# bryanboateng/animating-gaussian-splats

Hardware: AMD Instinct MI355X
Metric: Msplats/sec fwd+bwd @1080p (1M gauss) (higher is better)
Workload: dtype f32; 1 GPU; C3: 1000000 Gaussians, SH3, 1920x1080, 27-camera rig, 5 view(s)/GPU/step, fwd+bwd; gaussians=1000000, image=1920x1080, sh_degree=3, parallelism=camera-dp1, streams_per_gpu=3, submission=one host thread per stream, means2D=one fresh zero leaf per render (shared.py:38-41)

## Files before the change

animating-gaussian-splats_amd/csrc/gsr_api.hip:

```cpp
#include <hip/hip_runtime.h>

#include <atomic>
#include <cstdarg>
#include <cstdio>
#include <cstdlib>
#include <cmath>
#include <cstring>
#include <chrono>
#include <condition_variable>
#include <thread>
#include <map>
#include <memory>
#include <unordered_map>
#include <mutex>
#include <string>
#include <vector>

#include "../../include/gsr.h"
#include "gsr_common.h"
#include "gsr_internal.h"
#include "gsr_host.h"

using namespace gsr;

// ... 21 lines not shown
}

int gsr::fail(int code, const char *fmt, ...) {
    char buf[512];
    va_list ap;
    va_start(ap, fmt);
    vsnprintf(buf, sizeof(buf), fmt, ap);
    va_end(ap);
    g_err = buf;
    return code;
}

gsr::Phase::Phase(hipStream_t s_, const char *n, bool on) : s(s_), name(n) {
    if (!on || !g_prof_on) return;
    std::lock_guard<std::mutex> lk(g_prof_mu);
    if (!g_prof_sel.empty() && g_prof_sel.find("," + std::string(n) + ",") == std::string::npos) return;
    a = ev_get(); b = ev_get();
    if (a) (void)hipEventRecord(a, s);
}
gsr::Phase::~Phase() {
    if (!a || !b) return;
    (void)hipEventRecord(b, s);
    std::lock_guard<std::mutex> lk(g_prof_mu);
    g_prof.push_back({name, a, b});
}

gsr::HostPhase::HostPhase(const char *n) : name(n), t0(hclock::now()), on(g_prof_on) {}
gsr::HostPhase::~HostPhase() {
    if (!on) return;
    const double ms = std::chrono::duration<double, std::milli>(hclock::now() - t0).count();
    std::lock_guard<std::mutex> lk(g_prof_mu);
    g_host_ms[name] += ms;
    g_host_n[name] += 1;
}

namespace {

std::vector<hipEvent_t> g_gw_evpool;
struct GradEvent {
    hipEvent_t ev = nullptr;
    ~GradEvent() { if (ev) g_gw_evpool.push_back(ev); }
};
struct GradWriter { hipStream_t s = nullptr; std::shared_ptr<GradEvent> ev; };
std::mutex g_gw_mu;
std::unordered_map<const void *, GradWriter> g_gw;
constexpr size_t kGradPruneAt = 1024;

hipError_t no_launch() { return hipSuccess; }

template <typename Launch>
hipError_t ordered_grad_write(const void *const *keys, int nkeys, hipStream_t s, Launch launch) {
    std::lock_guard<std::mutex> lk(g_gw_mu);
    const GradEvent *waited[16];
    int nw = 0;
    for (int k = 0; k < nkeys; ++k) {
        if (!keys[k]) continue;
        auto it = g_gw.find(keys[k]);
        if (it == g_gw.end() || it->second.s == s) continue;
        const GradEvent *e = it->second.ev.get();
        bool seen = false;
        for (int j = 0; j < nw; ++j) seen = seen || waited[j] == e;
        if (seen) continue;
        const hipError_t r = hipStreamWaitEvent(s, e->ev, 0);
        if (r != hipSuccess) return r;
        if (nw < 16) waited[nw++] = e;
    }
    auto ev = std::make_shared<GradEvent>();
    hipError_t r = hipSuccess;
    if (!g_gw_evpool.empty()) { ev->ev = g_gw_evpool.back(); g_gw_evpool.pop_back(); }
    else r = hipEventCreateWithFlags(&ev->ev, hipEventDisableTiming);
    if (r != hipSuccess) { ev->ev = nullptr; return r; }
    r = launch();
    if (r != hipSuccess) return r;
    r = hipEventRecord(ev->ev, s);
    if (r != hipSuccess) return r;
    for (int k = 0; k < nkeys; ++k)
        if (keys[k]) g_gw[keys[k]] = GradWriter{s, ev};
    if (g_gw.size() > kGradPruneAt) {
        for (auto it = g_gw.begin(); it != g_gw.end();)
            it = hipEventQuery(it->second.ev->ev) == hipSuccess ? g_gw.erase(it) : std::next(it);
    }
    return hipSuccess;
}

struct HostWord { uint32_t *h = nullptr; uint32_t *d = nullptr; };
HostWord pinned_word() {
    thread_local HostWord w;
    if (!w.h) {
        uint32_t *h = nullptr;
        if (hipHostMalloc((void **)&h, 4 * kHostWords, hipHostMallocMapped | hipHostMallocCoherent) != hipSuccess) return w;
        uint32_t *d = nullptr;
        if (hipHostGetDevicePointer((void **)&d, h, 0) != hipSuccess) { (void)hipHostFree(h); return w; }
        w.h = h; w.d = d;
    }
    return w;
}

constexpr uint32_t kNoValue = 0xFFFFFFFFu;

int check_common(const gsr_camera *cam, const gsr_gaussians *g, bool need_opacity) {
    if (!cam || !g) return fail(GSR_ERR_ARG, "null camera or gaussians");
    if (g->P < 0) return fail(GSR_ERR_ARG, "P must be >= 0");
    if (cam->image_width <= 0 || cam->image_height <= 0)
        return fail(GSR_ERR_ARG, "image size must be positive (got %dx%d)", cam->image_width, cam->image_height);
    const int gx = div_up(cam->image_width, kTileW), gy = div_up(cam->image_height, kTileH);
    if (gx > 65535 || gy > 65535) return fail(GSR_ERR_UNSUPPORTED, "tile grid too large");
    if (g->activations & ~(GSR_ACT_SIGMOID_OPACITY | GSR_ACT_EXP_SCALES | GSR_ACT_NORMALIZE_ROTATIONS))
        return fail(GSR_ERR_ARG, "unknown activation bits 0x%x", g->activations);
    if (g->P == 0) return GSR_OK;
    if (!g->means3D || (need_opacity && !g->opacities))
        return fail(GSR_ERR_ARG, "means3D and opacities are required");
    if ((g->shs == nullptr) == (g->colors_precomp == nullptr))
        return fail(GSR_ERR_ARG, "Please provide excatly one of either SHs or precomputed colors!");
    const bool sr = g->scales && g->rotations;
    if (sr == (g->cov3D_precomp != nullptr) || ((g->scales != nullptr) != (g->rotations != nullptr)))
        return fail(GSR_ERR_ARG, "Please provide exactly one of either scale/rotation pair or precomputed 3D covariance!");
    if (g->shs && (g->sh_coeffs <= 0 || (g->sh_degree + 1) * (g->sh_degree + 1) > g->sh_coeffs || g->sh_degree > 3 || g->sh_degree < 0))
        return fail(GSR_ERR_ARG, "invalid SH configuration: degree %d with %d coefficients", g->sh_degree, g->sh_coeffs);
    if (!cam->viewmatrix || !cam->projmatrix || !cam->bg || (g->shs && !cam->campos))
        return fail(GSR_ERR_ARG, "camera matrices / bg / campos missing");
    return GSR_OK;
}

std::atomic<int> g_exact{[] {
    const char *e = getenv("GSR_EXACT_THRESHOLDS");
    return (e && e[0] == '0') ? 0 : 1;
}()};

void fill_common(ViewIn &v, const gsr_camera *cam, const gsr_gaussians *g) {
    memset(&v, 0, sizeof(v));
    v.P = g->P; v.D = g->sh_degree; v.M = g->shs ? g->sh_coeffs : 0;
    v.W = cam->image_width; v.H = cam->image_height;
    v.gx = div_up(v.W, kTileW); v.gy = div_up(v.H, kTileH);
    v.scale_modifier = g->scale_modifier;
    v.act = g->activations;
    v.tan_fovx = cam->tan_fovx; v.tan_fovy = cam->tan_fovy;
    v.focal_y = v.H / (2.0f * v.tan_fovy);
    v.focal_x = v.W / (2.0f * v.tan_fovx);
    v.means3D = g->means3D; v.scales = g->scales; v.rotations = g->rotations; v.opacities = g->opacities;
    v.shs = g->shs; v.colors_precomp = g->colors_precomp; v.cov3D_precomp = g->cov3D_precomp;
    v.viewmatrix = cam->viewmatrix; v.projmatrix = cam->projmatrix; v.campos = cam->campos; v.bg = cam->bg;
    const bool vz = !cam->viewmatrix_stride[0] && !cam->viewmatrix_stride[1];
    const bool pz = !cam->projmatrix_stride[0] && !cam->projmatrix_stride[1];
    v.cs.v0 = vz ? 4 : cam->viewmatrix_stride[0]; v.cs.v1 = vz ? 1 : cam->viewmatrix_stride[1];
    v.cs.p0 = pz ? 4 : cam->projmatrix_stride[0]; v.cs.p1 = pz ? 1 : cam->projmatrix_stride[1];
    v.cs.c0 = cam->campos_stride ? cam->campos_stride : 1;
}

template <typename A>
void carve_saved(A &a, char *geom, char *img) {
    const GeomLayout G(a.v.P);
    a.rec = (float4 *)(geom + G.rec); a.rect = (uint2 *)(geom + G.rect);
    a.goff = (uint32_t *)(geom + G.goff); a.clampm = (uint8_t *)(geom + G.clampm);
    const ImageLayout L(a.v.W, a.v.H, a.v.P);
    a.ranges = (uint2 *)(img + L.ranges); a.pix_end = (float4 *)(img + L.pix_end);
    a.n_contrib = (uint32_t *)(img + L.n_contrib); a.tile_maxc = (uint32_t *)(img + L.tile_maxc);
    a.tile_flag = (uint32_t *)(img + L.tile_flag); a.near_rec = (float4 *)(img + L.near_rec);
    a.seg_off = (uint32_t *)(img + L.seg_off); a.meta = (uint32_t *)(img + L.meta);
    a.items_ws = (uint32_t *)(img + L.items_ws);
}
void carve_forward(FwdArgs &a, char *geom, char *img) {
    carve_saved(a, geom, img);
    const GeomLayout G(a.v.P);
    a.depth = (float *)(geom + G.depth); a.tiles = (uint32_t *)(geom + G.tiles);
    const ImageLayout L(a.v.W, a.v.H, a.v.P);
    a.tile_order_f = (uint32_t *)(img + L.tile_order_f); a.sort_lists = (uint32_t *)(img + L.sort_lists);
    a.tile_count = (uint32_t *)(img + L.tile_count); a.tile_cursor = (uint32_t *)(img + L.tile_cursor);
    a.block_sums = (uint32_t *)(img + L.block_sums); a.block_off = (uint32_t *)(img + L.block_off);
    a.chunk_off = (uint32_t *)(img + L.chunk_off); a.scan_ws = (uint32_t *)(img + L.scan_ws);
    a.tile_rank = (uint32_t *)(img + L.tile_rank); a.tsat_list = (uint32_t *)(img + L.tsat_list);
}
template <typename A>
void carve_binning(A &a, char *bin, const BinningLayout &L) {
    a.point_list = (uint32_t *)(bin + L.point_list); a.slot_emit = (uint32_t *)(bin + L.slot_emit);
    a.seg_state = (float4 *)(bin + L.seg_state);
}

struct BinRegions {
    BinningLayout arrays;
    size_t items, tmp, total;
    BinRegions(int K, int P, int T, bool with_items, bool with_merge) : arrays(K, P) {
        items = arrays.total;
        tmp = items + (with_items ? bwd_items_bytes(K, T) : 0);
        total = tmp + (with_merge ? sizeof(uint4) * (size_t)K : 0);
    }
};

int enqueue_post_scan(FwdArgs a, char *bin, int layout, uint32_t n_mid, uint32_t n_vlong, uint32_t max_n,
                      bool prepare_backward, int T, hipStream_t s, const uint32_t *spec_ok, bool phases) {
    const BinRegions R(layout, a.v.P, T, prepare_backward, n_vlong != 0);
    carve_binning(a, bin, R.arrays);
    a.pairs = (uint4 *)(bin + R.arrays.pairs);
    a.spec_ok = spec_ok;
    uint4 *tmp = n_vlong ? (uint4 *)(bin + R.tmp) : nullptr;
    uint2 *items = (uint2 *)(bin + R.items);
    { Phase ph(s, "bin_emit", phases); HIP_TRY(launch_bin_emit(a, spec_ok ? 0 : layout, s)); }
    { Phase ph(s, "tile_sort", phases); HIP_TRY(launch_tile_sort(a, n_mid, n_vlong, max_n, tmp, s)); }
    { Phase ph(s, "render_fwd", phases); HIP_TRY(launch_render_fwd(a, s)); }
    if (prepare_backward) {
        Phase ph(s, "bwd_items", phases);
        HIP_TRY(launch_bwd_items_raw(layout, T, a.v.P, a.ranges, a.tile_maxc, a.tile_flag, items, a.items_ws, s, spec_ok));
    }
    return GSR_OK;
}

enum class KWait { published, stream_error, drained };
KWait wait_published(const uint32_t *word, hipStream_t s, hipError_t *err) {
    auto last = hclock::now();
    while (__atomic_load_n(word, __ATOMIC_ACQUIRE) == kNoValue) {
        __builtin_ia32_pause();
        if (hclock::now() - last > std::chrono::microseconds(500)) {
            last = hclock::now();
            const hipError_t q = hipStreamQuery(s);
            if (q == hipErrorNotReady) continue;
            *err = q;
            if (q != hipSuccess) return KWait::stream_error;
            return __atomic_load_n(word, __ATOMIC_ACQUIRE) == kNoValue ? KWait::drained : KWait::published;
        }
    }
    return KWait::published;
}

}

extern "C" {

const char *gsr_last_error(void) { return g_err.c_str(); }

int gsr_set_exact_thresholds(int on) { return g_exact.exchange(on ? 1 : 0); }
int gsr_abi_version(void) { return GSR_ABI_VERSION; }

size_t gsr_geom_bytes(int P) { return GeomLayout(P < 0 ? 0 : P).total; }
size_t gsr_image_bytes(int W, int H, int P) { return ImageLayout(W, H, P < 0 ? 0 : P).total; }
size_t gsr_binning_bytes(int K, int P) { return BinningLayout(K, P).total; }
size_t gsr_backward_items_bytes(int K, int W, int H) {
    return bwd_items_bytes(K < 0 ? 0 : K, div_up(W < 0 ? 0 : W, kTileW) * div_up(H < 0 ? 0 : H, kTileH));
}
size_t gsr_sums_bytes(int P) { return align256(sizeof(float) * (kPartial * (size_t)(P < 0 ? 0 : P) + 1)); }
size_t gsr_scratch_bytes(int K, int W, int H) {
    return ScratchLayout(K, div_up(W < 0 ? 0 : W, kTileW) * div_up(H < 0 ? 0 : H, kTileH)).total;
}

void *gsr_prealloc_alloc(void *ctx, int which, size_t bytes) {
    gsr_prealloc *pa = (gsr_prealloc *)ctx;
    if (!pa) return nullptr;
    if (which >= 0 && which < 5 && pa->ptr[which] && pa->bytes[which] >= bytes && !(pa->used & (1 << which))) {
        pa->used |= 1 << which;
        return pa->ptr[which];
    }
    return pa->fallback ? pa->fallback(pa->fallback_ctx, which, bytes) : nullptr;
}

int gsr_buffer_offsets(int P, int W, int H, int K, size_t *out, int max_out) {
    const GeomLayout g(P);
    const ImageLayout im(W, H, P);
    const BinningLayout b(K, P);
    const size_t v[16] = {g.depth, g.rec, g.rect, g.tiles, g.goff,
                          im.ranges, im.pix_end, im.n_contrib, im.tile_maxc,
                          b.pairs, b.point_list, b.slot_emit, im.seg_off, b.seg_state, im.tile_flag,
                          im.items_ws + sizeof(uint32_t) * kTSatCtr};
    int n = 0;
    for (; n < 16 && n < max_out; ++n) out[n] = v[n];
    return n;
}

}

namespace {
struct SpecKey {
    int dev, P, W, H;
    bool operator==(const SpecKey &o) const { return dev == o.dev && P == o.P && W == o.W && H == o.H; }
};
struct SpecKeyHash {
    size_t operator()(const SpecKey &k) const {
        return ((size_t)k.dev * 1000003u) ^ ((size_t)k.P * 2654435761u) ^ ((size_t)k.W << 20) ^ (size_t)k.H;
    }
};
constexpr int kSpecWindow = 16;
constexpr size_t kSpecKeys = 64;
struct SpecStat {
    uint32_t recent[kSpecWindow] = {};
    uint32_t recent_mid[kSpecWindow] = {};
    int n = 0;
    bool long_lists = false;
    uint64_t used = 0;
    uint32_t window_max() const {
        uint32_t m = 0;
        for (int k = 0; k < std::min(n, kSpecWindow); ++k) m = std::max(m, recent[k]);
        return m;
    }
};
std::mutex g_spec_mu;
std::unordered_map<SpecKey, SpecStat, SpecKeyHash> g_spec;
uint64_t g_spec_clock = 0;
int g_spec_hits = 0, g_spec_misses = 0, g_async_calls = 0;

uint32_t spec_capacity(const SpecKey &key, uint32_t *sort_blocks = nullptr) {
    std::lock_guard<std::mutex> lk(g_spec_mu);
    auto it = g_spec.find(key);
    if (it == g_spec.end() || it->second.long_lists) return 0;
    it->second.used = ++g_spec_clock;
    const uint32_t mk = it->second.window_max();
    if (sort_blocks) {
        uint32_t mm = 0;
        for (int k = 0; k < std::min(it->second.n, kSpecWindow); ++k) mm = std::max(mm, it->second.recent_mid[k]);
        *sort_blocks = std::min<uint32_t>((uint32_t)kSpecSortBlocks, mm + mm / 4 + 16);
    }
    const uint64_t c = (uint64_t)mk + mk / 4 + 65536;
    return (uint32_t)std::min<uint64_t>((c + 4095) & ~uint64_t(4095), 0x7FFFFFFFu);
}
void spec_record(const SpecKey &key, uint32_t K, bool long_lists, int outcome, uint32_t n_mid) {
    std::lock_guard<std::mutex> lk(g_spec_mu);
    if (!g_spec.count(key) && g_spec.size() >= kSpecKeys) {
        auto lru = g_spec.begin();
        for (auto it = g_spec.begin(); it != g_spec.end(); ++it)
            if (it->second.used < lru->second.used) lru = it;
        g_spec.erase(lru);
    }
    SpecStat &st = g_spec[key];
    st.recent[st.n % kSpecWindow] = K;
    st.recent_mid[st.n % kSpecWindow] = n_mid;
    ++st.n;
    st.long_lists = long_lists;
    st.used = ++g_spec_clock;
    if (outcome > 0) ++g_spec_hits;
    if (outcome < 0) ++g_spec_misses;
}

constexpr int kAsyncSlots = 4096;
constexpr int kSlotWords = 16;
constexpr int kGateWord = 4, kGateErrWord = 5;
constexpr uint64_t kGateTimeoutTicks = 500000000ull;
std::atomic<uint64_t> g_gate_timeout{kGateTimeoutTicks};
std::atomic<int> g_hold_next_redo_ms{0};

struct AsyncFwd {
    uint64_t id = 0;
    int dev = 0, slot = -1, T = 0;
    hipStream_t s = nullptr;
    uint32_t seq = 0, cap = 0;
    bool prep = false, released = false, err_reported = false;
    SpecKey key{0, 0, 0, 0};
    FwdArgs a;
    void *spec_bin = nullptr;
    hipEvent_t ev_scan = nullptr;
    int state = 0;
    uint32_t K = 0;
    int layout = 0;
    void *bin = nullptr;
    void *own = nullptr;
    std::string err;
};

std::mutex g_as_mu;
std::condition_variable g_as_wake;
std::condition_variable g_as_done;
std::unordered_map<uint64_t, std::shared_ptr<AsyncFwd>> g_as;
uint64_t g_as_next_id = 1;
uint32_t g_as_seq = 0;
uint32_t *g_slot_h = nullptr, *g_slot_d = nullptr;
std::vector<uint8_t> g_slot_busy;
std::vector<hipEvent_t> g_as_evpool;
int g_slot_next = 0;
std::string g_async_err;
bool g_resolver_started = false, g_resolver_stop = false;
std::thread g_resolver;

uint32_t *slot_h(int k) { return g_slot_h + (size_t)k * kSlotWords; }
uint32_t *slot_d(int k) { return g_slot_d + (size_t)k * kSlotWords; }

void resolver_main();

std::map<int, hipStream_t> g_resolver_streams;
hipStream_t resolver_stream(int dev) {
    hipStream_t &h = g_resolver_streams[dev];
    if (h) return h;
    int lo = 0, hi = 0;
    if (hipDeviceGetStreamPriorityRange(&lo, &hi) != hipSuccess) hi = 0;
    if (hipStreamCreateWithPriority(&h, hipStreamNonBlocking, hi) != hipSuccess) h = nullptr;
    return h;
}

bool async_init() {
    if (!g_slot_h) {
        uint32_t *h = nullptr;
        const size_t bytes = sizeof(uint32_t) * ((size_t)kAsyncSlots * kSlotWords + 16);
        if (hipHostMalloc((void **)&h, bytes, hipHostMallocMapped | hipHostMallocCoherent | hipHostMallocPortable) != hipSuccess)
            return false;
        uint32_t *d = nullptr;
        if (hipHostGetDevicePointer((void **)&d, h, 0) != hipSuccess) { (void)hipHostFree(h); return false; }
        memset(h, 0, bytes);
        g_slot_h = h; g_slot_d = d;
        g_slot_busy.assign(kAsyncSlots, 0);
    }
    if (!g_resolver_started) {
        g_resolver_stop = false;
        g_resolver = std::thread(resolver_main);
        g_resolver_started = true;
    }
    return true;
}

int slot_acquire() {
    for (int k = 0; k < kAsyncSlots; ++k) {
        const int j = (g_slot_next + k) % kAsyncSlots;
        if (!g_slot_busy[j]) {
            g_slot_busy[j] = 1;
            g_slot_next = (j + 1) % kAsyncSlots;
            return j;
        }
    }
    return -1;
// ... 586 lines not shown
```

animating-gaussian-splats_amd/csrc/gsr_backward.hip:

```cpp
#include "gsr_common.h"
#include "gsr_internal.h"

#include <algorithm>

namespace gsr {

#ifdef GSR_TRACE
__device__ uint64_t *g_trace_bwd;
#endif

constexpr uint32_t kItemStartCost = 64;

constexpr int kItemsBlock = 256;
struct ItemBucket {
    uint32_t shift;
    __device__ explicit ItemBucket(int ks) {
        const uint32_t mx = (4u << ks) + kItemStartCost;
        shift = mx >= (uint32_t)kOrderBuckets ? 32 - __builtin_clz(mx / kOrderBuckets) : 0;
    }
    __device__ uint32_t operator()(uint32_t cost) const {
        return (uint32_t)kOrderBuckets - 1u - min(cost >> shift, (uint32_t)kOrderBuckets - 1u);
    }
};
template <typename F>
// ... 76 lines not shown
            items[base + atomicAdd(&items[0].y, 1u)] = make_uint2((uint32_t)t, code);
        });
    }
    const uint32_t n = ex ? 0u : rg.y - rg.x;
    for_tile_items(n, mq, ks, bk, [&](uint32_t, uint32_t b) { atomicAdd(&s_cur[b], 1u); });
    lds_barrier();
    for (int b = threadIdx.x; b < kOrderBuckets; b += blockDim.x) {
        const uint32_t h = s_cur[b];
        if (h) s_cur[b] = atomicAdd(&ws[kOrderBuckets + b], h);
    }
    lds_barrier();
    for_tile_items(n, mq, ks, bk, [&](uint32_t code, uint32_t b) {
        items[1 + atomicAdd(&s_cur[b], 1u)] = make_uint2((uint32_t)t, code);
    });
}

struct __attribute__((packed, aligned(4))) F3 { float x, y, z; };
__device__ inline void rec_store(float4 *part, uint32_t em, float r0, float r1, float r2, float r3, float r4,
                                 float r5, float r6, float r7, float r8) {
    F3 *d = reinterpret_cast<F3 *>(reinterpret_cast<float *>(part) + (size_t)kRecF * em);
    d[0] = F3{r0, r1, r2};
    d[1] = F3{r3, r4, r5};
    d[2] = F3{r6, r7, r8};
}

#define GSR_BWD_ATTR __attribute__((amdgpu_waves_per_eu(EXACT ? 4 : 7, 8)))
constexpr int kBwdWaves = 4;
#ifndef GSR_EXACT_BWD_BLOCKS
#define GSR_EXACT_BWD_BLOCKS 256
#endif
constexpr int kExactBwdBlocks = GSR_EXACT_BWD_BLOCKS;

__device__ inline void row_halves3(float &X, float &Y, float &Z) {
    asm("s_nop 1\n\t"
        "v_add_f32_dpp %0, %0, %0 row_ror:8 row_mask:0xf bank_mask:0xf bound_ctrl:1\n\t"
        "v_add_f32_dpp %1, %1, %1 row_ror:8 row_mask:0xf bank_mask:0xf bound_ctrl:1\n\t"
        "v_add_f32_dpp %2, %2, %2 row_ror:8 row_mask:0xf bank_mask:0xf bound_ctrl:1\n\t"
        "v_add_f32_dpp %0, %0, %0 row_ror:4 row_mask:0xf bank_mask:0xf bound_ctrl:1\n\t"
        "v_add_f32_dpp %1, %1, %1 row_ror:4 row_mask:0xf bank_mask:0xf bound_ctrl:1\n\t"
        "v_add_f32_dpp %2, %2, %2 row_ror:4 row_mask:0xf bank_mask:0xf bound_ctrl:1\n\t"
        "v_add_f32_dpp %0, %0, %0 row_ror:2 row_mask:0xf bank_mask:0xf bound_ctrl:1\n\t"
        "v_add_f32_dpp %1, %1, %1 row_ror:2 row_mask:0xf bank_mask:0xf bound_ctrl:1\n\t"
        "v_add_f32_dpp %2, %2, %2 row_ror:2 row_mask:0xf bank_mask:0xf bound_ctrl:1"
        : "+v"(X), "+v"(Y), "+v"(Z));
}
struct RowW { bool r0, r2; };
__device__ inline RowW row_weights(int row) { return RowW{row == 0, row == 2}; }
struct PairSums { float X, Y, Z; };
__device__ inline PairSums pair_sums(float S0, float S1, float S4, float cs0, float cs1, float cs2, float dx,
                                     const RowW &w) {
    const float pA = fold32(S0, S1), pB = fold32(S4, cs0), pC = fold32(cs1, cs2);
    const float rA = fold16(pA, pB);
    const float rC = fold16(0.f, pC);
    const float wx = w.r0 ? dx : 1.f;
    const float wy = w.r0 ? dx * dx : (w.r2 ? dx : 0.f);
    PairSums r{rA * wx, fmaf(rA, wy, rC), rA};
    row_halves3(r.X, r.Y, r.Z);
    return r;
}

struct PixState { float T, AR; f2v d01; float d2, fy; int lrel; };
struct LaneSums { float S0; f2v S14, c01; float c2; };

constexpr int kNearNone = 0, kNearLook = 1, kNearEval = 2;
struct NearRecs { const float4 *r; uint32_t n; int start; };
template <bool CLAMP, int NEAR>
__device__ __forceinline__ void eval_quarter(PixState &ps, LaneSums &s, bool &any, const PairX &x, float4 a,
                                             float C2, float o, float4 c, int j, int k, float pfx,
                                             const float4 *__restrict__ rec, const uint32_t *__restrict__ pl,
                                             const NearRecs &nrs) {
    const float dy = a.y - ps.fy;
    float p2 = pair_power(x, C2, dy);
    float G = __builtin_amdgcn_exp2f(p2);
    float alpha = CLAMP ? fminf(0.99f, o * G) : o * G;
    const bool live = j < ps.lrel;
    if constexpr (NEAR == kNearEval) {
        const bool nr = live && p2 <= 0.0f && near_threshold(alpha);
        if (nr) {
            const ExactBlend e = exact_blend(a.x, a.y, rec[(size_t)kRecF4 * pl[j] + 3], o, pfx, ps.fy);
            p2 = e.power; G = e.G; alpha = e.alpha;
        }
    } else if constexpr (NEAR == kNearLook) {
        const bool nr = live && p2 <= 0.0f && near_threshold(alpha);
        if (nr) {
            const uint32_t key = ((uint32_t)(nrs.start + j) << 8) | (uint32_t)((threadIdx.x & 63) + 64 * k);
            for (uint32_t i = 0; i < nrs.n; ++i) {
                const float4 r = nrs.r[i];
                const bool hit = __float_as_uint(r.x) == key;
                p2 = hit ? r.y : p2;
                G = hit ? r.z : G;
                alpha = hit ? r.w : alpha;
            }
        }
    }
    const bool ok = live && p2 <= 0.0f && alpha >= 1.0f / 255.0f;
    any = any || ok;
    const float al = ok ? alpha : 0.f;
    ps.T = ps.T * __builtin_amdgcn_rcpf(1.f - al);
    const float cd = fmaf(c.z, ps.d2, fmaf(c.y, ps.d01.y, c.x * ps.d01.x));
    const float diff = cd - ps.AR;
    ps.AR = fmaf(al, diff, ps.AR);
    const float w = al * ps.T;
    float gd;
    if constexpr (CLAMP) {
        const float tg = ps.T * diff;
        gd = ok ? (o * G) * tg : 0.f;
    } else {
        gd = w * diff;
    }
    const float u = gd * dy;
    s.S0 += gd;
    s.S14 = fma2(f2(gd, u), f2(dy, dy), s.S14);
    s.c01 = fma2(f2(w, w), ps.d01, s.c01);
    s.c2 = fmaf(w, ps.d2, s.c2);
}

template <bool CLAMP, int NEAR>
__device__ __forceinline__ void walk_batch(PixState (&ps)[4], uint64_t m, const float4 *s_a, float pfx,
                                           const RowW &rw, float *o_row, const float4 *__restrict__ rec,
                                           const uint32_t *__restrict__ pl, const NearRecs &nrs) {
    constexpr int kStage = 64 * kBwdWaves;
    while (m) {
        const int j = 63 - __builtin_clzll(m);
        m &= ~(1ull << j);
        const float4 a = s_a[j], b = s_a[kStage + j], c = s_a[2 * kStage + j];
        const uint32_t qm = __builtin_amdgcn_readfirstlane(__float_as_uint(c.w));
        const PairX x = pair_x(a, pfx);
        LaneSums s{-0.f, f2(-0.f, -0.f), f2(-0.f, -0.f), -0.f};
        bool any = false;
#pragma unroll
        for (int k = 0; k < 4; ++k) {
            if (!(qm & (1u << k))) continue;
            eval_quarter<CLAMP, NEAR>(ps[k], s, any, x, a, b.x, b.y, c, j, k, pfx, rec, pl, nrs);
        }
        if (__builtin_amdgcn_ballot_w64(any)) {
            const PairSums sm = pair_sums(s.S0, s.S14.x, s.S14.y, s.c01.x, s.c01.y, s.c2, x.dx, rw);
            if ((threadIdx.x & 14) == 0) {
                float *o = o_row + j * kPartial;
                lds_add(o, sm.X);
                lds_add(o + 4, sm.Y);
                if ((threadIdx.x & 63) < 2) lds_add(o + 8, sm.Z);
            }
        }
    }
}

template <bool EXACT>
__device__ __forceinline__ void bwd_item(
    uint2 it, uint32_t item, int W, int H, int gx, const uint2 *__restrict__ ranges,
    const uint32_t *__restrict__ point_list,
    const float4 *__restrict__ rec, const float *__restrict__ bg, const float4 *__restrict__ pix_end,
    const uint32_t *__restrict__ n_contrib, const uint32_t *__restrict__ tile_maxc,
    const uint32_t *__restrict__ seg_off, const float4 *__restrict__ seg_state,
    const uint32_t *__restrict__ slot_emit, const float *__restrict__ dL_dpixels,
    float4 *__restrict__ part, int ks, const uint32_t *__restrict__ tile_flag,
    const float4 *__restrict__ near_rec, float4 *s_a, float *s_out) {
    constexpr int kStage = 64 * kBwdWaves;
#ifdef GSR_TRACE
    const uint64_t t_start = __builtin_amdgcn_s_memrealtime();
#endif
    const int tile = (int)it.x;
    const uint32_t seg = it.y;
    const uint2 rg = ranges[tile];
    const int n = (int)(rg.y - rg.x);
    const int tx = tile % gx, ty = tile / gx;
    const int lane = threadIdx.x & 63;
    const int px = tx * kTileW + (lane & 15);
    const int py0 = ty * kTileH + (lane >> 4);
    const float pfx = (float)px;
    const float tx0 = (float)(tx * kTileW), ty0 = (float)(ty * kTileH);
    const float tx1 = tx0 + (kTileW - 1);
    const uint4 mq = reinterpret_cast<const uint4 *>(tile_maxc)[tile];
    const int maxc = min((int)max(max(mq.x, mq.y), max(mq.z, mq.w)), n);
    if (seg & kZeroItem) {
        const int z0 = maxc + (int)kZeroChunk * (int)((seg & ~kZeroItem) + 1);
        for (int p = z0 + lane; p < min(n, z0 + (int)kZeroChunk); p += 64) {
            rec_store(part, slot_emit[rg.x + p], 0.f, 0.f, 0.f, 0.f, 0.f, 0.f, 0.f, 0.f, 0.f);
        }
        return;
    }
    const int s0 = (int)seg << ks, s1f = s0 + (1 << ks);
    const int s1 = min(s1f, maxc);
    if (s1f >= maxc) {
        for (int p = maxc + lane; p < min(n, maxc + (int)kZeroChunk); p += 64) {
            rec_store(part, slot_emit[rg.x + p], 0.f, 0.f, 0.f, 0.f, 0.f, 0.f, 0.f, 0.f, 0.f);
        }
    }
    const float half_w = (float)(0.5 * W), half_h = (float)(0.5 * H);
    const float bg0 = bg[0], bg1 = bg[1], bg2 = bg[2];
    PixState ps[4];
    const uint32_t qmax[4] = {mq.x, mq.y, mq.z, mq.w};
    const bool has_bound = s1f < n;
    const size_t bidx = has_bound ? ((size_t)seg_off[tile] + seg) * kTilePix : 0;
#pragma unroll
    for (int k = 0; k < 4; ++k) {
        const int py = py0 + 4 * k;
        ps[k].fy = (float)py;
        const bool inside = px < W && py < H;
        const int pid = py * W + px;
        const float4 pe = inside ? pix_end[pid] : make_float4(0.f, 0.f, 0.f, 0.f);
        ps[k].lrel = (inside ? (int)n_contrib[pid] : 0) - s1;
        ps[k].d01 = f2(inside ? dL_dpixels[pid] : 0.f, inside ? dL_dpixels[H * W + pid] : 0.f);
        ps[k].d2 = inside ? dL_dpixels[2 * H * W + pid] : 0.f;
        float bd = 0;
        bd += bg0 * ps[k].d01.x; bd += bg1 * ps[k].d01.y; bd += bg2 * ps[k].d2;
        if (has_bound && qmax[k] >= (uint32_t)s1f) {
            const float4 st = seg_state[bidx + 64 * k + lane];
            ps[k].T = st.w;
            const float behind = ps[k].d01.x * (pe.x - st.x) + ps[k].d01.y * (pe.y - st.y) + ps[k].d2 * (pe.z - st.z);
            ps[k].AR = st.w > 0.f ? (behind + pe.w * bd) / st.w : bd;
        } else {
            ps[k].T = pe.w;
            ps[k].AR = bd;
        }
    }
    const RowW rw = row_weights(lane >> 4);
    float *o_row = s_out + (lane >> 4);
    NearRecs nrs{near_rec + (size_t)kNearCap * tile, EXACT ? 0u : tile_flag[tile], 0};
    uint32_t g_n = 0, em_n = 0;
    auto fetch = [&](int e) {
        const int st = e - 64 > s0 ? e - 64 : s0;
        if (lane < e - st) {
            g_n = point_list[rg.x + st + lane];
            em_n = slot_emit[rg.x + st + lane];
        }
    };
    if (s1 > s0) fetch(s1);
    for (int end = s1; end > s0; end -= 64) {
        const int start = end - 64 > s0 ? end - 64 : s0;
        const int cnt = end - start;
        float4 a = make_float4(0.f, 0.f, 0.f, 0.f), b = a, c = a, cj = a;
        float2 tl = make_float2(0.f, 0.f);
        if (lane < cnt) {
            const float4 *r = rec + (size_t)kRecF4 * g_n;
            a = r[0]; b = r[1]; c = r[2]; cj = r[3];
            tl = make_float2(cj.z, __uint_as_float(em_n));
        }
        if (end - 64 > s0) fetch(end - 64);
#pragma unroll
        for (int q = 0; q < kPartial; ++q) s_out[lane * kPartial + q] = 0.f;
#pragma unroll
        for (int k = 0; k < 4; ++k) ps[k].lrel += cnt;
        uint32_t qmask = 0;
        if (lane < cnt) {
            const uint32_t p = (uint32_t)(start + lane);
            s_a[lane] = a;
            s_a[kStage + lane] = make_float4(b.x, b.y, cj.x, cj.y);
#pragma unroll
            for (int k = 0; k < 4; ++k)
                if (p < qmax[k] &&
                    !tile_cull(a.x, a.y, -2.f * a.z, -a.w, -2.f * b.x, b.y, b.w, tx0, ty0 + 4 * k, tx1, ty0 + 4 * k + 3))
                    qmask |= 1u << k;
            if (qmask && b.y > 0.99f) qmask |= 16u;
            s_a[2 * kStage + lane] = make_float4(c.x, c.y, c.z, __uint_as_float(qmask));
        }
        uint64_t m = __ballot(qmask != 0);
        wave_lds_sync();
        const uint32_t *pl = point_list + rg.x + start;
        const bool clamp = __builtin_amdgcn_ballot_w64(qmask & 16u) != 0;
        if constexpr (EXACT) {
            if (clamp) walk_batch<true, kNearEval>(ps, m, s_a, pfx, rw, o_row, rec, pl, nrs);
            else walk_batch<false, kNearEval>(ps, m, s_a, pfx, rw, o_row, rec, pl, nrs);
        } else {
            nrs.start = start;
            if (nrs.n) {
                if (clamp) walk_batch<true, kNearLook>(ps, m, s_a, pfx, rw, o_row, rec, pl, nrs);
                else walk_batch<false, kNearLook>(ps, m, s_a, pfx, rw, o_row, rec, pl, nrs);
            } else {
                if (clamp) walk_batch<true, kNearNone>(ps, m, s_a, pfx, rw, o_row, rec, pl, nrs);
                else walk_batch<false, kNearNone>(ps, m, s_a, pfx, rw, o_row, rec, pl, nrs);
            }
        }
        wave_lds_sync();
        if (lane < cnt) {
            const float *s2 = s_out + lane * kPartial;
            float sm[kPartial];
#pragma unroll
            for (int q = 0; q < kPartial; ++q) sm[q] = s2[q];
            const float4 bj = s_a[kStage + lane];
            const float o = bj.y;
            const uint32_t em = __float_as_uint(tl.y);
            rec_store(part, em,
                      (-bj.z * sm[0] - bj.w * sm[2]) * half_w,
                      (-bj.w * sm[0] - tl.x * sm[2]) * half_h,
                      -0.5f * sm[4],
                      -0.5f * sm[6],
                      -0.5f * sm[1],
                      sm[8] != 0.f ? sm[8] / o : 0.f,
                      sm[3], sm[5], sm[7]);
        }
    }
#ifdef GSR_TRACE
    trace_wave(g_trace_bwd, item, t_start, 0);
#endif
}


template <bool EXACT>
__global__ __launch_bounds__(64 * kBwdWaves) GSR_BWD_ATTR void k_render_bwd(
    int W, int H, int gx, const uint2 *__restrict__ items, const uint2 *__restrict__ ranges,
    const uint32_t *__restrict__ point_list,
    const float4 *__restrict__ rec, const float *__restrict__ bg, const float4 *__restrict__ pix_end,
    const uint32_t *__restrict__ n_contrib, const uint32_t *__restrict__ tile_maxc,
    const uint32_t *__restrict__ seg_off, const float4 *__restrict__ seg_state,
    const uint32_t *__restrict__ slot_emit, const float *__restrict__ dL_dpixels,
    float4 *__restrict__ part, int ks, const uint32_t *__restrict__ spec_ok,
    const uint32_t *__restrict__ tile_flag, const float4 *__restrict__ near_rec) {
    constexpr int kStage = 64 * kBwdWaves;
    __shared__ float4 s_stage[3 * kStage];
    __shared__ float s_out_all[64 * kPartial * kBwdWaves];
    if (spec_ok && *spec_ok == 0u) return;
    const uint32_t wv = __builtin_amdgcn_readfirstlane(threadIdx.x >> 6);
    float4 *s_a = s_stage + 64 * wv;
    float *s_out = s_out_all + 64 * kPartial * wv;
    const uint2 hd = items[0];
    if constexpr (EXACT) {
        for (uint32_t i = blockIdx.x * kBwdWaves + wv; i < hd.y; i += gridDim.x * kBwdWaves)
            bwd_item<true>(items[1 + hd.x + i], hd.x + i, W, H, gx, ranges, point_list, rec, bg, pix_end, n_contrib, tile_maxc, seg_off, seg_state, slot_emit, dL_dpixels, part, ks, tile_flag, near_rec, s_a, s_out);
    } else {
        const uint32_t item = blockIdx.x * kBwdWaves + wv;
        if (item >= hd.x) return;
        bwd_item<false>(items[1 + item], item, W, H, gx, ranges, point_list, rec, bg, pix_end, n_contrib, tile_maxc, seg_off, seg_state, slot_emit, dL_dpixels, part, ks, tile_flag, near_rec, s_a, s_out);
    }
}

__device__ inline void gput(float *p, size_t idx, float v, bool acc) { p[idx] = acc ? p[idx] + v : v; }
template <int N>
__device__ inline void old_load(const float *p, size_t base, bool acc, float (&o)[N]) {
#pragma unroll
    for (int k = 0; k < N; ++k) o[k] = acc ? p[base + k] : 0.f;
}
__device__ inline void gput_old(float *p, size_t idx, float v, bool acc, float old) { p[idx] = acc ? old + v : v; }

__device__ inline float3 unit_vec_bwd(float3 v, float3 g) {
    const float n2 = v.x * v.x + v.y * v.y + v.z * v.z;
    const float inv_n3 = 1.0f / sqrtf(n2 * n2 * n2);
    return make_float3(((+n2 - v.x * v.x) * g.x - v.y * v.x * g.y - v.z * v.x * g.z) * inv_n3,
                       (-v.x * v.y * g.x + (n2 - v.y * v.y) * g.y - v.z * v.y * g.z) * inv_n3,
                       (-v.x * v.z * g.x - v.y * v.z * g.y + (n2 - v.z * v.z) * g.z) * inv_n3);
}

template <typename ShPtr>
__device__ inline float3 sh_dir_grad(int deg, float x, float y, float z, ShPtr sh, const float (&dRGB)[3]) {
    const float xx = x * x, yy = y * y, zz = z * z, xy = x * y, yz = y * z, xz = x * z;
    float dx[3] = {0, 0, 0}, dy[3] = {0, 0, 0}, dz[3] = {0, 0, 0};
#define SH(i, c) sh[(i) * 3 + (c)]
    if (deg > 0) {
#pragma unroll
        for (int c = 0; c < 3; ++c) {
            dx[c] = -GSR_SH_C1 * SH(3, c); dy[c] = -GSR_SH_C1 * SH(1, c); dz[c] = GSR_SH_C1 * SH(2, c);
        }
        if (deg > 1) {
#pragma unroll
            for (int c = 0; c < 3; ++c) {
                dx[c] += kSH_C2[0] * y * SH(4, c) + kSH_C2[2] * 2.f * -x * SH(6, c) + kSH_C2[3] * z * SH(7, c) +
                         kSH_C2[4] * 2.f * x * SH(8, c);
                dy[c] += kSH_C2[0] * x * SH(4, c) + kSH_C2[1] * z * SH(5, c) + kSH_C2[2] * 2.f * -y * SH(6, c) +
                         kSH_C2[4] * 2.f * -y * SH(8, c);
                dz[c] += kSH_C2[1] * y * SH(5, c) + kSH_C2[2] * 2.f * 2.f * z * SH(6, c) + kSH_C2[3] * x * SH(7, c);
            }
            if (deg > 2) {
#pragma unroll
                for (int c = 0; c < 3; ++c) {
                    dx[c] += (kSH_C3[0] * SH(9, c) * 3.f * 2.f * xy + kSH_C3[1] * SH(10, c) * yz +
                              kSH_C3[2] * SH(11, c) * -2.f * xy + kSH_C3[3] * SH(12, c) * -3.f * 2.f * xz +
                              kSH_C3[4] * SH(13, c) * (-3.f * xx + 4.f * zz - yy) +
                              kSH_C3[5] * SH(14, c) * 2.f * xz + kSH_C3[6] * SH(15, c) * 3.f * (xx - yy));
                    dy[c] += (kSH_C3[0] * SH(9, c) * 3.f * (xx - yy) + kSH_C3[1] * SH(10, c) * xz +
                              kSH_C3[2] * SH(11, c) * (-3.f * yy + 4.f * zz - xx) +
                              kSH_C3[3] * SH(12, c) * -3.f * 2.f * yz + kSH_C3[4] * SH(13, c) * -2.f * xy +
                              kSH_C3[5] * SH(14, c) * -2.f * yz + kSH_C3[6] * SH(15, c) * -3.f * 2.f * xy);
                    dz[c] += (kSH_C3[1] * SH(10, c) * xy + kSH_C3[2] * SH(11, c) * 4.f * 2.f * yz +
                              kSH_C3[3] * SH(12, c) * 3.f * (2.f * zz - xx - yy) +
                              kSH_C3[4] * SH(13, c) * 4.f * 2.f * xz + kSH_C3[5] * SH(14, c) * (xx - yy));
                }
            }
        }
    }
#undef SH
    return make_float3(dx[0] * dRGB[0] + dx[1] * dRGB[1] + dx[2] * dRGB[2],
                       dy[0] * dRGB[0] + dy[1] * dRGB[1] + dy[2] * dRGB[2],
                       dz[0] * dRGB[0] + dz[1] * dRGB[1] + dz[2] * dRGB[2]);
}

__device__ inline void sh_basis16(float x, float y, float z, float (&basis)[16]) {
    const float xx = x * x, yy = y * y, zz = z * z, xy = x * y, yz = y * z, xz = x * z;
    basis[0] = GSR_SH_C0;
    basis[1] = -GSR_SH_C1 * y; basis[2] = GSR_SH_C1 * z; basis[3] = -GSR_SH_C1 * x;
    basis[4] = kSH_C2[0] * xy; basis[5] = kSH_C2[1] * yz; basis[6] = kSH_C2[2] * (2.f * zz - xx - yy);
    basis[7] = kSH_C2[3] * xz; basis[8] = kSH_C2[4] * (xx - yy);
    basis[9] = kSH_C3[0] * y * (3.f * xx - yy);
    basis[10] = kSH_C3[1] * xy * z;
    basis[11] = kSH_C3[2] * y * (4.f * zz - xx - yy);
    basis[12] = kSH_C3[3] * z * (2.f * zz - 3.f * xx - 3.f * yy);
    basis[13] = kSH_C3[4] * x * (4.f * zz - xx - yy);
    basis[14] = kSH_C3[5] * z * (xx - yy);
    basis[15] = kSH_C3[6] * x * (xx - 3.f * yy);
}

template <typename ShPtr, typename OutPtr>
__device__ inline float3 sh_backward(int deg, int M, float3 mean, float3 campos, ShPtr sh,
                                     const bool *clamped, float3 dL_dcolor, OutPtr dL_dsh, bool acc = false) {
    const float3 d0 = make_float3(mean.x - campos.x, mean.y - campos.y, mean.z - campos.z);
    const float len = sqrtf(d0.x * d0.x + d0.y * d0.y + d0.z * d0.z);
    const float x = d0.x / len, y = d0.y / len, z = d0.z / len;
    const float dRGB[3] = {dL_dcolor.x * (clamped[0] ? 0.f : 1.f), dL_dcolor.y * (clamped[1] ? 0.f : 1.f),
                           dL_dcolor.z * (clamped[2] ? 0.f : 1.f)};
    const float3 dL_ddir = sh_dir_grad(deg, x, y, z, sh, dRGB);
    float basis[16];
    sh_basis16(x, y, z, basis);
    const int active = (deg + 1) * (deg + 1);
    if (dL_dsh) {
#pragma unroll
        for (int i = 0; i < 16; ++i) {
            if (i < M) {
#pragma unroll
                for (int c = 0; c < 3; ++c) {
                    const float v = i < active ? basis[i] * dRGB[c] : 0.f;
                    dL_dsh[i * 3 + c] = acc ? dL_dsh[i * 3 + c] + v : v;
                }
            }
        }
        for (int i = 16; i < M; ++i)
            for (int c = 0; c < 3; ++c) dL_dsh[i * 3 + c] = acc ? dL_dsh[i * 3 + c] : 0.f;
    }
    return unit_vec_bwd(d0, dL_ddir);
}

__device__ inline void cov3d_backward(float3 s3, float mod, float4 q, const float *dc, float3 &dscale,
                                      float4 &drot) {
    const float r = q.x, x = q.y, y = q.z, z = q.w;
    const m3 R = rot_from_quat(q);
    const float s[3] = {mod * s3.x, mod * s3.y, mod * s3.z};
    m3 S = {{0, 0, 0, 0, 0, 0, 0, 0, 0}};
    GM(S, 0, 0) = s[0]; GM(S, 1, 1) = s[1]; GM(S, 2, 2) = s[2];
    const m3 M = m3_mul(S, R);
    const m3 dSig = {{dc[0], 0.5f * dc[1], 0.5f * dc[2], 0.5f * dc[1], dc[3], 0.5f * dc[4], 0.5f * dc[2],
                      0.5f * dc[4], dc[5]}};
    m3 M2;
#pragma unroll
    for (int k = 0; k < 9; ++k) M2.m[k] = 2.0f * M.m[k];
    const m3 dM = m3_mul(M2, dSig);
    const m3 Rt = m3_T(R);
    m3 dMt = m3_T(dM);
    float ds[3];
#pragma unroll
    for (int i = 0; i < 3; ++i)
        ds[i] = GM(Rt, i, 0) * GM(dMt, i, 0) + GM(Rt, i, 1) * GM(dMt, i, 1) + GM(Rt, i, 2) * GM(dMt, i, 2);
    dscale = make_float3(ds[0], ds[1], ds[2]);
#pragma unroll
    for (int i = 0; i < 3; ++i)
#pragma unroll
        for (int rr = 0; rr < 3; ++rr) GM(dMt, i, rr) *= s[i];
#define G(c, rr) GM(dMt, c, rr)
    drot.x = 2 * z * (G(0, 1) - G(1, 0)) + 2 * y * (G(2, 0) - G(0, 2)) + 2 * x * (G(1, 2) - G(2, 1));
    drot.y = 2 * y * (G(1, 0) + G(0, 1)) + 2 * z * (G(2, 0) + G(0, 2)) + 2 * r * (G(1, 2) - G(2, 1)) -
             4 * x * (G(2, 2) + G(1, 1));
    drot.z = 2 * x * (G(1, 0) + G(0, 1)) + 2 * r * (G(2, 0) - G(0, 2)) + 2 * z * (G(1, 2) + G(2, 1)) -
             4 * y * (G(2, 2) + G(0, 0));
    drot.w = 2 * r * (G(0, 1) - G(1, 0)) + 2 * x * (G(2, 0) + G(0, 2)) + 2 * y * (G(1, 2) + G(2, 1)) -
             4 * z * (G(1, 1) + G(0, 0));
#undef G
}

template <int MC> constexpr int kRecChunk = 3 * 256 * 16 <= 64 * sh_row_stride(MC) * 4 ? 256 : 128;
template <int MC> constexpr int kRecStageF4 = 3 * kRecChunk<MC>;
__host__ __device__ constexpr int rec_chunk_f4(int C) { return (kRecF * C + 3 + 3) / 4; }
__device__ inline void add_chunk_records(const float *sf, uint32_t cb, uint32_t lo, uint32_t hi,
                                         float (&acc)[kPartial]) {
    for (uint32_t e = lo; e < hi; ++e) {
        const float *p = sf + kRecF * (e - cb);
#pragma unroll
        for (int k = 0; k < kPartial; ++k) acc[k] += p[k];
    }
}
// ... 440 lines not shown
        vis = true;
        gop += acc[5]; gc0 += acc[6]; gc1 += acc[7]; gc2 += acc[8];
        float vm[16], pj[16];
        load_mat16(V.viewmatrix, V.cs.v0, V.cs.v1, vm);
        load_mat16(V.projmatrix, V.cs.p0, V.cs.p1, pj);
        float dcov[6], dm0, dm1, dm2;
        view_chain(mean, c3, vm, pj, V.tan_fovx, V.tan_fovy, V.focal_x, V.focal_y, acc, dcov, dm0, dm1, dm2);
#pragma unroll
        for (int k = 0; k < 6; ++k) gcov[k] += dcov[k];
        if constexpr (MC > 0) {
            const float3 cp = load_campos(V.campos, V.cs.c0);
            bool cl[3];
            clamp_from_mask(V.clampm[i], cl);
            const float3 d0 = make_float3(mean.x - cp.x, mean.y - cp.y, mean.z - cp.z);
            const float len = sqrtf(d0.x * d0.x + d0.y * d0.y + d0.z * d0.z);
            const float x = d0.x / len, y = d0.y / len, z = d0.z / len;
            const float dRGB[3] = {acc[6] * (cl[0] ? 0.f : 1.f), acc[7] * (cl[1] ? 0.f : 1.f),
                                   acc[8] * (cl[2] ? 0.f : 1.f)};
            const float3 d = unit_vec_bwd(d0, sh_dir_grad(a.D, x, y, z, s_row, dRGB));
            dm0 += d.x; dm1 += d.y; dm2 += d.z;
        }
        gm0 += dm0; gm1 += dm1; gm2 += dm2;
    }
    if (live) {
        const int accm = a.accm;
        const bool ac = accm & GSR_GRAD_COLORS, ao = accm & GSR_GRAD_OPACITY, a3 = accm & GSR_GRAD_MEANS3D,
                   acv = accm & GSR_GRAD_COV3D, asc = accm & GSR_GRAD_SCALES, ar = accm & GSR_GRAD_ROTATIONS;
        if (!vis) {
#pragma unroll
            for (int k = 0; k < 3; ++k) {
                if (a.dL_dmeans3D && !a3) a.dL_dmeans3D[3 * i + k] = 0.f;
                if (a.dL_dcolors && !ac) a.dL_dcolors[3 * i + k] = 0.f;
                if (a.dL_dscales && !asc) a.dL_dscales[3 * i + k] = 0.f;
            }
            if (a.dL_dopacity && !ao) a.dL_dopacity[i] = 0.f;
            if (a.dL_dcov3D && !acv) {
#pragma unroll
                for (int k = 0; k < 6; ++k) a.dL_dcov3D[6 * i + k] = 0.f;
            }
            if (a.dL_drot && !ar) {
#pragma unroll
                for (int k = 0; k < 4; ++k) a.dL_drot[4 * i + k] = 0.f;
            }
        } else {
            float oo[1], oc[3], o3[3];
            old_load(a.dL_dopacity, (size_t)i, a.dL_dopacity && ao, oo);
            old_load(a.dL_dcolors, 3 * (size_t)i, a.dL_dcolors && ac, oc);
            old_load(a.dL_dmeans3D, 3 * (size_t)i, a.dL_dmeans3D && a3, o3);
            if (!a.dL_dopacity) {
            } else if (a.act & GSR_ACT_SIGMOID_OPACITY) {
                gput_old(a.dL_dopacity, i, gop * ((1.f - o_act) * o_act), ao, oo[0]);
            } else {
                gput_old(a.dL_dopacity, i, gop, ao, oo[0]);
            }
            if (a.dL_dcolors) {
                gput_old(a.dL_dcolors, 3 * i, gc0, ac, oc[0]); gput_old(a.dL_dcolors, 3 * i + 1, gc1, ac, oc[1]);
                gput_old(a.dL_dcolors, 3 * i + 2, gc2, ac, oc[2]);
            }
            if (a.dL_dmeans3D) {
                gput_old(a.dL_dmeans3D, 3 * i, gm0, a3, o3[0]); gput_old(a.dL_dmeans3D, 3 * i + 1, gm1, a3, o3[1]);
                gput_old(a.dL_dmeans3D, 3 * i + 2, gm2, a3, o3[2]);
            }
            if (a.dL_dcov3D) {
#pragma unroll
                for (int k = 0; k < 6; ++k) gput(a.dL_dcov3D, 6 * i + k, gcov[k], acv);
            }
            const bool has_sr = a.scales && !a.cov3D_precomp;
            if (has_sr) {
                float os[3], orr[4];
                old_load(a.dL_dscales, 3 * (size_t)i, a.dL_dscales && asc, os);
                old_load(a.dL_drot, 4 * (size_t)i, a.dL_drot && ar, orr);
                float3 ds; float4 dr;
                cov3d_backward(s3, a.scale_modifier, q, gcov, ds, dr);
                if (a.act & GSR_ACT_EXP_SCALES) { ds.x *= s3.x; ds.y *= s3.y; ds.z *= s3.z; }
                if (a.act & GSR_ACT_NORMALIZE_ROTATIONS) dr = act_normalize_bwd(q, qn, dr);
                if (a.dL_dscales) {
                    gput_old(a.dL_dscales, 3 * i, ds.x, asc, os[0]); gput_old(a.dL_dscales, 3 * i + 1, ds.y, asc, os[1]);
                    gput_old(a.dL_dscales, 3 * i + 2, ds.z, asc, os[2]);
                }
                if (a.dL_drot) {
                    gput_old(a.dL_drot, 4 * i, dr.x, ar, orr[0]); gput_old(a.dL_drot, 4 * i + 1, dr.y, ar, orr[1]);
                    gput_old(a.dL_drot, 4 * i + 2, dr.z, ar, orr[2]); gput_old(a.dL_drot, 4 * i + 3, dr.w, ar, orr[3]);
                }
            } else {
                if (a.dL_dscales && !asc) { a.dL_dscales[3 * i] = 0.f; a.dL_dscales[3 * i + 1] = 0.f; a.dL_dscales[3 * i + 2] = 0.f; }
                if (a.dL_drot && !ar) { a.dL_drot[4 * i] = 0.f; a.dL_drot[4 * i + 1] = 0.f; a.dL_drot[4 * i + 2] = 0.f; a.dL_drot[4 * i + 3] = 0.f; }
            }
        }
    }
    if constexpr (MC > 0) {
        if (!a.dL_dsh) return;
        if (live) {
#pragma unroll
            for (int k = 0; k < RL; ++k) s_row[k] = 0.f;
            const MultiView &V0 = a.v[vid(0)];
            int rv_n = V0.radii[i];
            uint8_t cm_n = V0.clampm[i];
            float g_n[3] = {V0.sums[(size_t)6 * P + i], V0.sums[(size_t)7 * P + i], V0.sums[(size_t)8 * P + i]};
            for (int t = 0; t < a.nv; ++t) {
                const MultiView &V = a.v[vid(t)];
                const int rv = rv_n;
                const uint8_t cm = cm_n;
                const float g[3] = {g_n[0], g_n[1], g_n[2]};
                if (t + 1 < a.nv) {
                    const MultiView &Vn = a.v[vid(t + 1)];
                    rv_n = Vn.radii[i];
                    cm_n = Vn.clampm[i];
#pragma unroll
                    for (int c = 0; c < 3; ++c) g_n[c] = Vn.sums[(size_t)(6 + c) * P + i];
                }
                if (!(rv > 0)) continue;
                const float3 cp = load_campos(V.campos, V.cs.c0);
                bool cl[3];
                clamp_from_mask(cm, cl);
                const float3 d0 = make_float3(mean.x - cp.x, mean.y - cp.y, mean.z - cp.z);
                const float len = sqrtf(d0.x * d0.x + d0.y * d0.y + d0.z * d0.z);
                const float x = d0.x / len, y = d0.y / len, z = d0.z / len;
                const float dRGB[3] = {g[0] * (cl[0] ? 0.f : 1.f), g[1] * (cl[1] ? 0.f : 1.f), g[2] * (cl[2] ? 0.f : 1.f)};
                float basis[16];
                sh_basis16(x, y, z, basis);
#pragma unroll
                for (int k = 0; k < MC; ++k)
                    if (k < active) {
#pragma unroll
                        for (int c = 0; c < 3; ++c) s_row[3 * k + c] += basis[k] * dRGB[c];
                    }
            }
        }
        __syncthreads();
        if (a.accm & GSR_GRAD_SH) sh_rows_from_lds<MC, true>(s_sh, nrow, a.dL_dsh + (size_t)i0 * RL);
        else sh_rows_from_lds<MC, false>(s_sh, nrow, a.dL_dsh + (size_t)i0 * RL);
    }
}


hipError_t launch_bwd_items_raw(int K, int T, int P, const uint2 *ranges, const uint32_t *tile_maxc,
                                const uint32_t *tile_flag, uint2 *items, uint32_t *ws, hipStream_t s,
                                const uint32_t *spec_ok) {
    if (K == 0) return hipSuccess;
    const int nb = div_up(T, kItemsBlock);
    k_items_count<<<nb, kItemsBlock, 0, s>>>(T, ranges, tile_maxc, tile_flag, items, ws, spec_ok, seg_log2(P));
    k_items_emit<<<nb, kItemsBlock, 0, s>>>(T, ranges, tile_maxc, tile_flag, items, ws, spec_ok, seg_log2(P));
    return hipGetLastError();
}
hipError_t launch_bwd_items(const BwdArgs &a, hipStream_t s) {
    return launch_bwd_items_raw(a.K, a.v.gx * a.v.gy, a.v.P, a.ranges, a.tile_maxc, a.tile_flag, a.items, a.items_ws, s);
}

hipError_t launch_render_bwd(const BwdArgs &a, hipStream_t s) {
    if (a.K == 0) return hipSuccess;
    const int ks = seg_log2(a.v.P);
    k_render_bwd<false><<<div_up((int)a.max_items, kBwdWaves), 64 * kBwdWaves, 0, s>>>(
        a.v.W, a.v.H, a.v.gx, a.items, a.ranges, a.point_list, a.rec, a.v.bg, a.pix_end, a.n_contrib, a.tile_maxc, a.seg_off,
        a.seg_state, a.slot_emit, a.dL_dcolor, a.part, ks, a.spec_ok, a.tile_flag, a.near_rec);
    k_render_bwd<true><<<std::min(div_up((int)a.max_items, kBwdWaves), kExactBwdBlocks), 64 * kBwdWaves, 0, s>>>(
        a.v.W, a.v.H, a.v.gx, a.items, a.ranges, a.point_list, a.rec, a.v.bg, a.pix_end, a.n_contrib, a.tile_maxc, a.seg_off,
        a.seg_state, a.slot_emit, a.dL_dcolor, a.part, ks, a.spec_ok, a.tile_flag, a.near_rec);
    return hipGetLastError();
}

template <int MC>
static void gauss_bwd_mc(const BwdArgs &a, hipStream_t s) {
    constexpr size_t lds = std::max(sizeof(float) * kShBlock * (MC ? sh_row_stride(MC) : 0),
                                    sizeof(float4) * kRecStageF4<MC> * (kShBlock / 64));
    k_gauss_bwd<MC><<<div_up(a.v.P, kShBlock), kShBlock, lds, s>>>(
        a.v.P, a.v.D, a.v.M, a.v.W, a.v.H, a.v.scale_modifier, a.v.tan_fovx, a.v.tan_fovy, a.v.focal_x, a.v.focal_y,
        a.v.means3D, a.v.scales, a.v.rotations, a.v.shs, a.v.cov3D_precomp, a.v.viewmatrix, a.v.projmatrix, a.v.campos, a.v.cs,
        a.radii, a.goff, a.part, a.dL_dmeans2D, a.dL_dcolors, a.dL_dopacity,
        a.dL_dmeans3D, a.dL_dcov3D, a.dL_dsh, a.dL_dscales, a.dL_drot, a.v.act, a.rec, a.accm, a.clampm);
}

hipError_t launch_gauss_bwd(const BwdArgs &a, hipStream_t s) {
    if (a.v.P == 0) return hipSuccess;
    switch (a.v.shs ? a.v.M : 0) {
        case 16: gauss_bwd_mc<16>(a, s); break;
        case 9: gauss_bwd_mc<9>(a, s); break;
        case 4: gauss_bwd_mc<4>(a, s); break;
        case 1: gauss_bwd_mc<1>(a, s); break;
        default: gauss_bwd_mc<0>(a, s); break;
    }
    return hipGetLastError();
}

template <int MC>
static void gauss_bwd_multi_mc(const MultiArgs &a, hipStream_t s) {
    k_gauss_bwd_multi<MC><<<div_up(a.P, kShBlock), kShBlock, multi_lds_bytes<MC>(), s>>>(a);
}

hipError_t launch_sum_records(int P, const uint32_t *goff, const float4 *part, float *sums, hipStream_t s,
                              const uint32_t *spec_ok, const float *viewmatrix, const float *projmatrix,
                              const float *campos, CamStrides cs, int W, int H) {
    if (P == 0) return hipSuccess;
    k_sum_records<<<div_up(P, 256), 256, 0, s>>>(P, goff, part, sums, spec_ok, viewmatrix, projmatrix, campos, cs,
                                                 W, H);
    return hipGetLastError();
}

hipError_t launch_gauss_bwd_multi(const MultiArgs &a, hipStream_t s) {
    if (a.P == 0 || a.nv == 0) return hipSuccess;
    switch (a.shs ? a.M : 0) {
        case 16: gauss_bwd_multi_mc<16>(a, s); break;
        case 9: gauss_bwd_multi_mc<9>(a, s); break;
        case 4: gauss_bwd_multi_mc<4>(a, s); break;
        case 1: gauss_bwd_multi_mc<1>(a, s); break;
        default: gauss_bwd_multi_mc<0>(a, s); break;
    }
    return hipGetLastError();
}

}

#ifdef GSR_TRACE
extern "C" int gsr_debug_trace_bwd(void *buf) {
    return hipMemcpyToSymbol(HIP_SYMBOL(gsr::g_trace_bwd), &buf, sizeof(buf)) == hipSuccess ? 0 : 2;
}
#endif
```

animating-gaussian-splats_amd/csrc/gsr_common.h:

```cpp
#pragma once
#include <hip/hip_runtime.h>
#include <stdint.h>

#include "../../include/gsr.h"

namespace gsr {

constexpr int kTileW = 16;
constexpr int kTileH = 16;
constexpr int kTilePix = kTileW * kTileH;
constexpr int kPartial = 9;
constexpr int kRecF = kPartial;
constexpr int kSortCap = 4096;
__host__ __device__ inline uint64_t pair_key(uint4 r) { return ((uint64_t)r.y << 32) | r.x; }
#ifndef GSR_FWD_SORT_CAP
#define GSR_FWD_SORT_CAP 1024
#endif
constexpr int kFwdSortCap = GSR_FWD_SORT_CAP;
constexpr int kHostWords = 4;

__host__ __device__ inline int div_up(int a, int b) { return (a + b - 1) / b; }
__host__ __device__ inline size_t align256(size_t x) { return (x + 255) & ~size_t(255); }

constexpr int kRecF4 = 4;
struct GeomLayout {
    size_t depth, rec, rect, tiles, goff, clampm, total;
    __host__ __device__ GeomLayout(int P) {
        size_t o = 0;
        depth = o;    o = align256(o + sizeof(float) * P);
        rec = o;      o = align256(o + sizeof(float4) * kRecF4 * (size_t)P);
        rect = o;     o = align256(o + sizeof(uint2) * P);
        tiles = o;    o = align256(o + sizeof(uint32_t) * P);
        goff = o;     o = align256(o + sizeof(uint32_t) * (P + 1));
        clampm = o;   o = align256(o + (size_t)P);
        total = o;
    }
};

constexpr int kBinThreads = 1024;
constexpr int kMaxLdsTiles = 16384;
struct BinGrid {
    int CH, NB;
    __host__ __device__ BinGrid(int P) {
        int c = div_up(P, 512);
        c = div_up(c, 256) * 256;
        CH = c < 1024 ? 1024 : c;
        NB = P > 0 ? div_up(P, CH) : 0;
    }
};

constexpr int kSeg = 256;
static_assert(kSeg >= 64 && (kSeg & (kSeg - 1)) == 0, "kSeg: a power of two, >= the forward's 64-entry batch");
constexpr int kSegLog2Max = __builtin_ctz(kSeg), kSegLog2Min = 6;
__host__ __device__ inline int seg_log2(int P) {
    int ks = kSegLog2Max;
    while (ks > kSegLog2Min && ((4 * (size_t)(P > 0 ? P : 0)) >> ks) < 8192) --ks;
    return ks;
}
__host__ __device__ inline uint32_t seg_bounds(uint32_t n, int ks) { return n > 0 ? (n - 1) >> ks : 0; }

__host__ __device__ inline uint32_t bwd_item_count(uint32_t n, uint4 mq, int ks) {
    const uint32_t maxc = min(max(max(mq.x, mq.y), max(mq.z, mq.w)), n);
    return n == 0 ? 0u : max(1u, (maxc + (1u << ks) - 1) >> ks);
}
__host__ __device__ inline uint32_t bwd_item_cost(uint32_t j, uint4 mq, int ks) {
    const uint32_t s0 = j << ks, s1 = s0 + (1u << ks);
    const uint32_t a = mq.x > s0 ? min(mq.x, s1) - s0 : 0u, b = mq.y > s0 ? min(mq.y, s1) - s0 : 0u;
    const uint32_t c = mq.z > s0 ? min(mq.z, s1) - s0 : 0u, d = mq.w > s0 ? min(mq.w, s1) - s0 : 0u;
    return a + b + c + d;
}
constexpr uint32_t kZeroChunk = 1024;
constexpr uint32_t kZeroItem = 0x80000000u;
__host__ __device__ inline uint32_t bwd_zero_items(uint32_t n, uint4 mq) {
    const uint32_t maxc = min(max(max(mq.x, mq.y), max(mq.z, mq.w)), n);
    return n - maxc > kZeroChunk ? (n - maxc - 1) / kZeroChunk : 0u;
}
__host__ __device__ inline size_t max_bwd_items(int K, int T) {
    const size_t k = (size_t)(K > 0 ? K : 0);
    return (k >> kSegLog2Min) + k / kZeroChunk + (k < (size_t)T ? k : (size_t)T) + 1;
}

constexpr int kOrderBuckets = 2048;
constexpr int kItemsWsWords = 2 * kOrderBuckets + 64;
constexpr int kTSatCtr = 2 * kOrderBuckets + 8;
__host__ __device__ constexpr uint32_t tsat_capacity(int npix) { return (uint32_t)(npix / 8 + 64); }

constexpr uint64_t kScanAgg = 1ull << 62, kScanInc = 2ull << 62;
constexpr int kScanBlocksMax = 512;
constexpr int kScanCtr = 16;
constexpr int kScanWsWords = 2 * kScanBlocksMax + kScanCtr + kOrderBuckets;
__host__ __device__ inline uint32_t lpt_bucket(uint32_t c) {
    uint32_t b = c;
    if (c >= 1024u) {
        const uint32_t e = 31u - (uint32_t)__builtin_clz(c);
        b = 1024u + ((e - 10u) << 5) + ((c >> (e - 5u)) & 31u);
    }
    return (uint32_t)kOrderBuckets - 1u - b;
}

constexpr uint32_t kNearCap = 16;
struct ImageLayout {
    size_t ranges, pix_end, n_contrib, tile_maxc, tile_order_f, seg_off, sort_lists,
        tile_count, tile_cursor, block_sums, block_off, meta, items_ws, scan_ws, tile_rank, tile_flag, tsat_list,
        near_rec, chunk_off, total;
    __host__ __device__ ImageLayout(int W, int H, int P) {
        const int T = div_up(W, kTileW) * div_up(H, kTileH);
        const int N = W * H;
        const int NB = BinGrid(P).NB;
        size_t o = 0;
        ranges = o;      o = align256(o + sizeof(uint2) * T);
        pix_end = o;     o = align256(o + sizeof(float4) * N);
        n_contrib = o;   o = align256(o + sizeof(uint32_t) * N);
        tile_maxc = o;   o = align256(o + sizeof(uint32_t) * 4 * T);
        tile_order_f = o; o = align256(o + sizeof(uint32_t) * T);
        seg_off = o;     o = align256(o + sizeof(uint32_t) * (T + 1));
        sort_lists = o;  o = align256(o + sizeof(uint32_t) * T);
        tile_count = o;  o = align256(o + sizeof(uint32_t) * T);
        tile_cursor = o; o = align256(o + sizeof(uint32_t) * T);
        block_sums = o;  o = align256(o + sizeof(uint32_t) * (NB + 1));
        block_off = o;   o = align256(o + sizeof(uint32_t) * (NB + 1));
        meta = o;        o = align256(o + sizeof(uint32_t) * 16);
        items_ws = o;    o = align256(o + sizeof(uint32_t) * kItemsWsWords);
        scan_ws = o;     o = align256(o + sizeof(uint32_t) * kScanWsWords);
        tile_rank = o;   o = align256(o + sizeof(uint32_t) * T);
        tile_flag = o;   o = align256(o + sizeof(uint32_t) * T);
        tsat_list = o;   o = align256(o + 32 * (size_t)tsat_capacity(N));
        near_rec = o;    o = align256(o + sizeof(float4) * kNearCap * T);
        chunk_off = o;   o = align256(o + (T <= kMaxLdsTiles ? sizeof(uint32_t) * (size_t)NB * T : 0));
        total = o;
    }
};

struct BinningLayout {
    size_t pairs, point_list, slot_emit, seg_state, total;
    __host__ __device__ BinningLayout(int K, int P) {
        size_t o = 0;
        pairs = o;      o = align256(o + sizeof(uint4) * (K > 0 ? K : 1));
        point_list = o; o = align256(o + sizeof(uint32_t) * (K > 0 ? K : 1));
        slot_emit = o;  o = align256(o + sizeof(uint32_t) * (K > 0 ? K : 1));
        seg_state = o;  o = align256(o + sizeof(float4) * kTilePix * (size_t)(((size_t)(K > 0 ? K : 0) >> seg_log2(P)) + 1));
        total = o;
    }
};

__host__ __device__ inline size_t bwd_items_bytes(int K, int T) { return align256(sizeof(uint2) * (max_bwd_items(K, T) + 1)); }

struct ScratchLayout {
    size_t part, items, total;
    __host__ __device__ ScratchLayout(int K, int T) {
        const size_t k = size_t(K > 0 ? K : 1);
        size_t o = 0;
        part = o;  o = align256(o + sizeof(float) * kRecF * k + 16);
        items = o; o += bwd_items_bytes(K, T);
        total = o;
    }
};

constexpr int kShBlock = 128;
__host__ __device__ constexpr int sh_row_stride(int MC) { return (3 * MC) | 1; }

template <int MC, int INFL = 16>
__device__ inline void sh_rows_to_lds(const float *__restrict__ src, int nrow, float *s) {
    constexpr int RL = 3 * MC, RS = sh_row_stride(MC);
    constexpr int IT = (kShBlock * RL / 4 + kShBlock - 1) / kShBlock;
    constexpr int B = IT < INFL ? IT : INFL;
    const int n = nrow * RL;
    if ((reinterpret_cast<uintptr_t>(src) & 15) == 0) {
        const int n4 = n >> 2;
        const float4 *s4 = reinterpret_cast<const float4 *>(src);
#pragma unroll
        for (int i0 = 0; i0 < IT; i0 += B) {
            float4 v[B];
#pragma unroll
            for (int it = 0; it < B; ++it) {
                const int q = threadIdx.x + (i0 + it) * kShBlock;
                if (i0 + it < IT && q < n4) v[it] = s4[q];
            }
#pragma unroll
            for (int it = 0; it < B; ++it) {
                const int q = threadIdx.x + (i0 + it) * kShBlock;
                if (i0 + it < IT && q < n4) {
                    const float f[4] = {v[it].x, v[it].y, v[it].z, v[it].w};
#pragma unroll
                    for (int j = 0; j < 4; ++j) {
                        const int e = 4 * q + j, r = e / RL;
                        s[r * RS + (e - r * RL)] = f[j];
                    }
                }
            }
        }
        for (int e = 4 * n4 + (int)threadIdx.x; e < n; e += kShBlock) {
            const int r = e / RL;
            s[r * RS + (e - r * RL)] = src[e];
        }
    } else {
        for (int e = threadIdx.x; e < n; e += kShBlock) {
            const int r = e / RL;
            s[r * RS + (e - r * RL)] = src[e];
        }
    }
}

template <int MC, bool ACC = false>
__device__ inline void sh_rows_from_lds(const float *s, int nrow, float *__restrict__ dst) {
    constexpr int RL = 3 * MC, RS = sh_row_stride(MC);
    const int n = nrow * RL;
    if ((reinterpret_cast<uintptr_t>(dst) & 15) == 0) {
        const int n4 = n >> 2;
        float4 *d4 = reinterpret_cast<float4 *>(dst);
        constexpr int IT = (kShBlock * RL / 4 + kShBlock - 1) / kShBlock;
        float4 o[IT];
        if (ACC) {
#pragma unroll
            for (int it = 0; it < IT; ++it) {
                const int q = threadIdx.x + it * kShBlock;
                o[it] = d4[q < n4 ? q : 0];
            }
        }
#pragma unroll
        for (int it = 0; it < IT; ++it) {
            const int q = threadIdx.x + it * kShBlock;
            if (q >= n4) break;
            float f[4];
#pragma unroll
            for (int j = 0; j < 4; ++j) {
                const int e = 4 * q + j, r = e / RL;
                f[j] = s[r * RS + (e - r * RL)];
            }
            float4 v = make_float4(f[0], f[1], f[2], f[3]);
            if (ACC) v = make_float4(o[it].x + v.x, o[it].y + v.y, o[it].z + v.z, o[it].w + v.w);
            d4[q] = v;
        }
        for (int e = 4 * n4 + (int)threadIdx.x; e < n; e += kShBlock) {
            const int r = e / RL;
            const float v = s[r * RS + (e - r * RL)];
            dst[e] = ACC ? dst[e] + v : v;
        }
    } else {
        for (int e = threadIdx.x; e < n; e += kShBlock) {
            const int r = e / RL;
            const float v = s[r * RS + (e - r * RL)];
            dst[e] = ACC ? dst[e] + v : v;
        }
    }
}

#define GSR_SH_C0 0.28209479177387814f
#define GSR_SH_C1 0.4886025119029199f
__device__ __constant__ const float kSH_C2[5] = {1.0925484305920792f, -1.0925484305920792f,
                                                 0.31539156525252005f, -1.0925484305920792f,
                                                 0.5462742152960396f};
__device__ __constant__ const float kSH_C3[7] = {-0.5900435899266435f, 2.890611442640554f,
                                                 -0.4570457994644658f, 0.3731763325901154f,
                                                 -0.4570457994644658f, 1.445305721320277f,
                                                 -0.5900435899266435f};

struct m3 { float m[9]; };
#define GM(A, c, r) ((A).m[(c) * 3 + (r)])

__device__ inline m3 m3_mul(const m3 &a, const m3 &b) {
    m3 o;
#pragma unroll
    for (int c = 0; c < 3; ++c)
#pragma unroll
        for (int r = 0; r < 3; ++r)
            o.m[c * 3 + r] = a.m[0 * 3 + r] * b.m[c * 3 + 0] + a.m[1 * 3 + r] * b.m[c * 3 + 1] +
                             a.m[2 * 3 + r] * b.m[c * 3 + 2];
    return o;
}
__device__ inline m3 m3_T(const m3 &a) {
    m3 o;
#pragma unroll
    for (int c = 0; c < 3; ++c)
#pragma unroll
        for (int r = 0; r < 3; ++r) o.m[c * 3 + r] = a.m[r * 3 + c];
    return o;
}

__device__ inline float ndc2pix(float v, int S) { return (float)(((v + 1.0) * S - 1.0) * 0.5); }

__device__ inline void get_rect(float px, float py, int max_radius, int gx, int gy, int &x0, int &y0,
                                int &x1, int &y1) {
    x0 = min(gx, max(0, (int)((px - max_radius) / kTileW)));
    y0 = min(gy, max(0, (int)((py - max_radius) / kTileH)));
    x1 = min(gx, max(0, (int)((px + max_radius + kTileW - 1) / kTileW)));
    y1 = min(gy, max(0, (int)((py + max_radius + kTileH - 1) / kTileH)));
}

__device__ inline float3 xform4x3(float3 p, const float *m) {
    return make_float3(m[0] * p.x + m[4] * p.y + m[8] * p.z + m[12],
                       m[1] * p.x + m[5] * p.y + m[9] * p.z + m[13],
                       m[2] * p.x + m[6] * p.y + m[10] * p.z + m[14]);
// ... 287 lines not shown
```

animating-gaussian-splats_amd/csrc/gsr_forward.hip:

```cpp
#include "gsr_common.h"
#include "gsr_internal.h"

#include <algorithm>
#include <type_traits>

namespace gsr {

#ifdef GSR_TRACE
__device__ uint64_t *g_trace_fwd;
#ifdef GSR_TRACE
__device__ inline uint64_t trace_fwd_work(uint64_t batches, uint64_t walk, uint64_t evals) {
    return (batches << 40) | ((walk < 0xFFFFFull ? walk : 0xFFFFFull) << 20) | (evals < 0xFFFFFull ? evals : 0xFFFFFull);
}
#endif
__device__ uint64_t *g_trace_emit;
#define GSR_EMIT_STAMP(k)                                                                        \
    do {                                                                                         \
        if (g_trace_emit && threadIdx.x == 0)                                                    \
            g_trace_emit[4 * blockIdx.x + (k)] = __builtin_amdgcn_s_memrealtime();               \
    } while (0)
#else
#define GSR_EMIT_STAMP(k) do {} while (0)
#endif

// ... 207 lines not shown
            const uint32_t ws_ = lane <= first ? (uint32_t)(w >> 32) & 0x3FFFFFFFu : 0u;
            ex_c += (uint32_t)__builtin_amdgcn_readlane((int)wave_incl_scan_u32(wc), 63);
            ex_s += (uint32_t)__builtin_amdgcn_readlane((int)wave_incl_scan_u32(ws_), 63);
            if (inc) break;
        }
        if (lane == 0 && blk > 0)
            __hip_atomic_store(&look[blk], kScanInc | ((uint64_t)(ex_s + agg_s) << 32) | (ex_c + agg_c),
                               __ATOMIC_RELAXED, __HIP_MEMORY_SCOPE_AGENT);
        const int tl = blk * kColW + lane;
        const uint32_t bkt = lpt_bucket(cnt);
        const bool mine = lane < kColW && tl < T;
        const uint32_t local = mine ? atomicAdd(&s_lpt[bkt], 1u) : 0u;
        wave_lds_sync();
        if (mine && local == 0) s_lpt[bkt] = atomicAdd(&lpt[bkt], s_lpt[bkt]);
        wave_lds_sync();
        if (mine) tile_rank[tl] = s_lpt[bkt] + local;
        if (mine) {
            const uint32_t ex = ex_c + ic - cnt;
            ranges[tl] = cnt ? make_uint2(ex, ex + cnt) : make_uint2(0, 0);
            tile_cursor[tl] = ex;
            seg_off[tl] = ex_s + is - sb;
            if (cnt > (uint32_t)kSortCap) {
                sort_lists[T - 1 - atomicAdd(&ctr[3], 1u)] = (uint32_t)tl;
                atomicMax(&ctr[4], cnt);
            } else if (cnt > (uint32_t)kFwdSortCap) {
                sort_lists[atomicAdd(&ctr[2], 1u)] = (uint32_t)tl;
            }
        }
    }
    drain_vmem();
    __builtin_amdgcn_fence(__ATOMIC_RELEASE, "workgroup");
    __syncthreads();
    if (threadIdx.x == 0) s_last = atomicAdd(&ctr[1], 1u) == gridDim.x - 1 ? 1u : 0u;
    __syncthreads();
    if (!s_last) return;
    const uint64_t fin = __hip_atomic_load(&look[gridDim.x - 1], __ATOMIC_RELAXED, __HIP_MEMORY_SCOPE_AGENT);
    const uint32_t K = (uint32_t)fin, n_seg = (uint32_t)(fin >> 32) & 0x3FFFFFFFu;
    {
        constexpr int kPer = kOrderBuckets / (kColW * kColG);
        uint32_t h[kPer], hs = 0;
#pragma unroll
        for (int i = 0; i < kPer; ++i) {
            h[i] = __hip_atomic_load(&lpt[threadIdx.x * kPer + i], __ATOMIC_RELAXED, __HIP_MEMORY_SCOPE_AGENT);
            hs += h[i];
        }
        uint32_t tt;
        uint32_t e = block_excl_scan_u32(hs, s_red, &tt);
#pragma unroll
        for (int i = 0; i < kPer; ++i) {
            lpt[threadIdx.x * kPer + i] = e;
            e += h[i];
        }
    }
    {
        const uint32_t bs = (int)threadIdx.x < NB ? block_sums[threadIdx.x] : 0u;
        uint32_t btot;
        const uint32_t bex = block_excl_scan_u32(bs, s_red, &btot);
        if ((int)threadIdx.x < NB) block_off[threadIdx.x] = bex;
    }
    if (threadIdx.x == 0) {
        const uint32_t n_mid = __hip_atomic_load(&ctr[2], __ATOMIC_RELAXED, __HIP_MEMORY_SCOPE_AGENT);
        const uint32_t n_long = __hip_atomic_load(&ctr[3], __ATOMIC_RELAXED, __HIP_MEMORY_SCOPE_AGENT);
        const uint32_t max_long = __hip_atomic_load(&ctr[4], __ATOMIC_RELAXED, __HIP_MEMORY_SCOPE_AGENT);
        seg_off[T] = n_seg;
        meta[0] = K;
        meta[1] = (cap && K <= cap && n_long == 0u) ? 1u : 0u;
        meta[2] = n_mid;
        if (host_words) {
            __hip_atomic_store(host_words + 1, n_mid, __ATOMIC_RELAXED, __HIP_MEMORY_SCOPE_SYSTEM);
            __hip_atomic_store(host_words + 2, n_long, __ATOMIC_RELAXED, __HIP_MEMORY_SCOPE_SYSTEM);
            __hip_atomic_store(host_words + 3, max_long, __ATOMIC_RELAXED, __HIP_MEMORY_SCOPE_SYSTEM);
            __hip_atomic_store(host_words, K, __ATOMIC_RELEASE, __HIP_MEMORY_SCOPE_SYSTEM);
        }
    }
}

__global__ __launch_bounds__(1024) void k_bin_scan(int T, int NB, const uint32_t *__restrict__ tile_count,
                                                   uint2 *__restrict__ ranges,
                                                   uint32_t *__restrict__ tile_cursor,
                                                   const uint32_t *__restrict__ block_sums,
                                                   uint32_t *__restrict__ block_off,
                                                   uint32_t *__restrict__ meta,
                                                   uint32_t *host_words,
                                                   uint32_t *__restrict__ tile_order,
                                                   uint32_t *__restrict__ sort_lists,
                                                   uint32_t *__restrict__ seg_off, uint32_t cap, int ks) {
    __shared__ uint32_t s_red[16];
    __shared__ uint32_t s_hist[kOrderBuckets];
    __shared__ uint32_t s_cls[3];
    if (threadIdx.x < 3) s_cls[threadIdx.x] = 0;
    uint32_t carry = 0;
    for (int base = 0; base < T; base += blockDim.x) {
        const int t = base + threadIdx.x;
        const uint32_t c = t < T ? tile_count[t] : 0;
        uint32_t tot;
        const uint32_t ex = block_excl_scan_u32(c, s_red, &tot) + carry;
        if (t < T) {
            ranges[t] = c ? make_uint2(ex, ex + c) : make_uint2(0, 0);
            tile_cursor[t] = ex;
        }
        carry += tot;
    }
    uint32_t carry3 = 0;
    for (int base = 0; base < T; base += blockDim.x) {
        const int t = base + threadIdx.x;
        const uint32_t nb = t < T ? seg_bounds(tile_count[t], ks) : 0;
        uint32_t tot;
        const uint32_t ex = block_excl_scan_u32(nb, s_red, &tot) + carry3;
        if (t < T) seg_off[t] = ex;
        carry3 += tot;
    }
    if (threadIdx.x == 0) seg_off[T] = carry3;
    uint32_t carry2 = 0;
    for (int base = 0; base < NB; base += blockDim.x) {
        const int b = base + threadIdx.x;
        const uint32_t c = b < NB ? block_sums[b] : 0;
        uint32_t tot;
        const uint32_t ex = block_excl_scan_u32(c, s_red, &tot) + carry2;
        if (b < NB) block_off[b] = ex;
        carry2 += tot;
    }
    __syncthreads();
    for (int t = threadIdx.x; t < T; t += blockDim.x) {
        const uint32_t n = tile_count[t];
        if (n == 0) continue;
        if (n > (uint32_t)kSortCap) {
            sort_lists[T - 1 - atomicAdd(&s_cls[1], 1u)] = (uint32_t)t;
            atomicMax(&s_cls[2], n);
        } else if (n > (uint32_t)kFwdSortCap) {
            sort_lists[atomicAdd(&s_cls[0], 1u)] = (uint32_t)t;
        }
    }
    lds_barrier();
    if (threadIdx.x == 0) {
        meta[0] = carry;
        meta[1] = (cap && carry <= cap && s_cls[1] == 0u) ? 1u : 0u;
        meta[2] = s_cls[0];
        if (host_words) {
            for (int c = 0; c < 3; ++c)
                __hip_atomic_store(host_words + 1 + c, s_cls[c], __ATOMIC_RELAXED, __HIP_MEMORY_SCOPE_SYSTEM);
            __hip_atomic_store(host_words, carry, __ATOMIC_RELEASE, __HIP_MEMORY_SCOPE_SYSTEM);
        }
    }
    lpt_order(T, [&](int t) { return tile_count[t]; }, tile_order, s_hist, s_red);
}

template <bool USE_LDS>
__global__ __launch_bounds__(kBinThreads) void k_bin_emit(int P, int CH, int T, int gx,
                                                  const uint2 *__restrict__ rects,
                                                  const uint32_t *__restrict__ tiles,
                                                  const float *__restrict__ depth,
                                                  const uint32_t *__restrict__ block_off,
                                                  uint32_t *__restrict__ tile_cursor,
                                                  uint32_t *__restrict__ goff,
                                                  uint4 *__restrict__ pairs, uint32_t K,
                                                  const uint32_t *__restrict__ chunk_off,
                                                  const uint32_t *__restrict__ spec_ok,
                                                  const uint32_t *__restrict__ tile_count,
                                                  const uint32_t *__restrict__ tile_rank,
                                                  const uint32_t *__restrict__ lpt_off,
                                                  uint32_t *__restrict__ tile_order) {
    extern __shared__ __attribute__((aligned(16))) uint32_t s_cur[];
    __shared__ uint32_t s_red[16];
    if (spec_ok && *spec_ok == 0u) return;
    const int b = blockIdx.x;
    const int g0 = b * CH, g1 = min(P, g0 + CH);
    if (tile_rank) {
        const int per = div_up(T, (int)gridDim.x), t1 = min(T, (b + 1) * per);
        for (int t = b * per + (int)threadIdx.x; t < t1; t += blockDim.x)
            tile_order[lpt_off[lpt_bucket(tile_count[t])] + tile_rank[t]] = (uint32_t)t;
    }
    GSR_EMIT_STAMP(0);
    if (USE_LDS) {
        const uint32_t *row = chunk_off + (size_t)b * T;
        for (int t = threadIdx.x; t < T; t += blockDim.x) s_cur[t] = tile_cursor[t] + row[t];
        __syncthreads();
        GSR_EMIT_STAMP(1);
        GSR_EMIT_STAMP(2);
    }
    uint32_t carry = block_off[b];
    for (int base = g0; base < g1; base += blockDim.x) {
        const int g = base + threadIdx.x;
        const uint32_t n = g < g1 ? tiles[g] : 0;
        uint32_t tot;
        const uint32_t ex = block_excl_scan_u32(n, s_red, &tot) + carry;
        carry += tot;
        if (g < g1) {
            goff[g] = ex;
            if (n) {
                const uint2 r = rects[g];
                const int x0 = r.x & 0xFFFF, y0 = r.x >> 16, x1 = r.y & 0xFFFF, y1 = r.y >> 16;
                const uint32_t dbits = __float_as_uint(depth[g]);
                uint32_t e = ex;
                for (int y = y0; y < y1; ++y)
                    for (int x = x0; x < x1; ++x, ++e) {
                        const int t = y * gx + x;
                        const uint32_t pos = USE_LDS ? atomicAdd(&s_cur[t], 1u) : atomicAdd(&tile_cursor[t], 1u);
                        pairs[pos] = make_uint4((uint32_t)g, dbits, e, 0u);
                    }
            }
        }
    }
    if (b == gridDim.x - 1 && threadIdx.x == 0) goff[P] = spec_ok ? spec_ok[-1] : K;
#ifdef GSR_TRACE
    __syncthreads();
    GSR_EMIT_STAMP(3);
#endif
}


template <int D>
__device__ inline uint32_t lane_xor(uint32_t x) {
    if constexpr (D == 1) return (uint32_t)__builtin_amdgcn_mov_dpp((int)x, 0xB1, 0xF, 0xF, false);
    else if constexpr (D == 2) return (uint32_t)__builtin_amdgcn_mov_dpp((int)x, 0x4E, 0xF, 0xF, false);
    else if constexpr (D == 4) {
        const int m = __builtin_amdgcn_mov_dpp((int)x, 0x141, 0xF, 0xF, false);
        return (uint32_t)__builtin_amdgcn_mov_dpp(m, 0x1B, 0xF, 0xF, false);
    } else if constexpr (D == 8) return (uint32_t)__builtin_amdgcn_mov_dpp((int)x, 0x128, 0xF, 0xF, false);
    else if constexpr (D == 16) {
        auto r = __builtin_amdgcn_permlane16_swap(x, x, false, false);
        return (threadIdx.x & 16) ? r[0] : r[1];
    } else {
        auto r = __builtin_amdgcn_permlane32_swap(x, x, false, false);
        return (threadIdx.x & 32) ? r[0] : r[1];
    }
}

template <int R, int D>
__device__ inline void bitonic_xlane(uint64_t (&k)[R], uint32_t (&v)[R], bool take_min) {
#pragma unroll
    for (int r = 0; r < R; ++r) {
        const uint32_t plo = lane_xor<D>((uint32_t)k[r]), phi = lane_xor<D>((uint32_t)(k[r] >> 32));
        const uint32_t pv = lane_xor<D>(v[r]);
        const uint64_t pk = ((uint64_t)phi << 32) | plo;
        const bool mine = (k[r] < pk) == take_min;
        k[r] = mine ? k[r] : pk;
        v[r] = mine ? v[r] : pv;
    }
}

template <int R, int J>
__device__ inline void wave_merge_stages(uint64_t (&k)[R], uint32_t (&v)[R], int lane, uint32_t gbase, uint32_t KK) {
    if constexpr (J > 0) {
        if constexpr (J < R) {
#pragma unroll
            for (int r = 0; r < R; ++r) {
                if (r & J) continue;
                const int r2 = r | J;
                const bool asc = ((gbase + lane * R + r) & KK) == 0;
                if ((k[r] > k[r2]) == asc) {
                    const uint64_t t = k[r]; k[r] = k[r2]; k[r2] = t;
                    const uint32_t u = v[r]; v[r] = v[r2]; v[r2] = u;
                }
            }
        } else {
            constexpr int D = J / R;
            const bool asc = ((gbase + lane * R) & KK) == 0;
            const bool take_min = ((lane & D) == 0) == asc;
            bitonic_xlane<R, D>(k, v, take_min);
        }
        wave_merge_stages<R, J / 2>(k, v, lane, gbase, KK);
    }
}

template <int R, int KK>
__device__ inline void wave_sort_stages(uint64_t (&k)[R], uint32_t (&v)[R], int lane, uint32_t gbase) {
    if constexpr (KK <= 64 * R) {
        wave_merge_stages<R, KK / 2>(k, v, lane, gbase, KK);
        wave_sort_stages<R, 2 * KK>(k, v, lane, gbase);
    }
}

__device__ inline uint32_t sort_slot(uint32_t i) { return i + (i >> 4); }
constexpr int sort_slots(int n) { return n + n / 16; }

template <int R>
__device__ inline void block_xchg_stage(uint64_t (&k)[R], uint32_t (&v)[R], uint32_t ibase, int kk, int j,
                                        uint64_t *s_key, uint32_t *s_val) {
    const uint32_t sb = sort_slot(ibase), qb = sort_slot(ibase ^ (uint32_t)j);
#pragma unroll
    for (int r = 0; r < R; ++r) { s_key[sb + r] = k[r]; s_val[sb + r] = v[r]; }
    __syncthreads();
#pragma unroll
    for (int r = 0; r < R; ++r) {
        const uint32_t i = ibase + r;
        const uint64_t pk = s_key[qb + r];
        const uint32_t pv = s_val[qb + r];
        const bool take_min = ((i & j) == 0) == ((i & kk) == 0);
        const bool mine = (k[r] < pk) == take_min;
        k[r] = mine ? k[r] : pk;
        v[r] = mine ? v[r] : pv;
    }
    __syncthreads();
}

template <int R, int NW>
__device__ inline void block_sort_tile(int n, uint32_t start, const uint4 *__restrict__ pairs, uint64_t *s_key,
                                       uint32_t *s_val) {
    constexpr int SEG = 64 * R;
    const int lane = threadIdx.x & 63, w = threadIdx.x >> 6;
    const uint32_t gbase = (uint32_t)(w * SEG), ibase = gbase + lane * R;
    uint64_t k[R];
    uint32_t v[R];
#pragma unroll
    for (int r = 0; r < R; ++r) {
        const int i = (int)ibase + r;
        const uint4 q = i < n ? pairs[start + i] : make_uint4(~0u, ~0u, 0u, 0u);
        k[r] = pair_key(q);
        v[r] = q.z;
    }
    wave_sort_stages<R, 2>(k, v, lane, gbase);
    for (uint32_t kk = 2 * SEG; kk <= (uint32_t)(NW * SEG); kk <<= 1) {
        for (uint32_t j = kk >> 1; j >= (uint32_t)SEG; j >>= 1) block_xchg_stage<R>(k, v, ibase, kk, j, s_key, s_val);
        wave_merge_stages<R, SEG / 2>(k, v, lane, gbase, kk);
    }
    const uint32_t sb = sort_slot(ibase);
#pragma unroll
    for (int r = 0; r < R; ++r) { s_key[sb + r] = k[r]; s_val[sb + r] = v[r]; }
    __syncthreads();
}

__global__ __launch_bounds__(512) void k_tile_sort(int gx, const uint32_t *__restrict__ tiles,
                                                    const uint2 *__restrict__ ranges,
                                                    uint4 *__restrict__ pairs,
                                                    uint32_t *__restrict__ point_list,
                                                    uint32_t *__restrict__ slot_emit, uint32_t nlist,
                                                    const uint32_t *__restrict__ spec_ok) {
    __shared__ uint64_t s_keys[sort_slots(kSortCap)];
    __shared__ uint32_t s_vals[sort_slots(kSortCap)];
    if (spec_ok) {
        if (*spec_ok == 0u) return;
        nlist = spec_ok[1];
    }
    static_assert(kSortCap == 8 * 64 * 8, "k_tile_sort: 8 waves x 64 lanes x 8 keys");
    for (uint32_t li = blockIdx.x; li < nlist; li += gridDim.x) {
        const int tile = (int)tiles[li];
        const uint2 rg = ranges[tile];
        const int n = (int)(rg.y - rg.x);
        if (n <= 4 * 64 * 8) block_sort_tile<4, 8>(n, rg.x, pairs, s_keys, s_vals);
        else block_sort_tile<8, 8>(n, rg.x, pairs, s_keys, s_vals);
        for (int i = threadIdx.x; i < n; i += blockDim.x) {
            const uint32_t sl = sort_slot((uint32_t)i);
            point_list[rg.x + i] = (uint32_t)s_keys[sl];
            slot_emit[rg.x + i] = s_vals[sl];
        }
        __syncthreads();
    }
}

__device__ inline uint4 key_record(uint64_t k, uint32_t emit) {
    return make_uint4((uint32_t)k, (uint32_t)(k >> 32), emit, 0u);
}

__global__ __launch_bounds__(512) void k_chunk_sort(int T, const uint32_t *__restrict__ lists,
                                                     const uint2 *__restrict__ ranges, uint4 *__restrict__ pairs) {
    __shared__ uint64_t s_keys[sort_slots(kSortCap)];
    __shared__ uint32_t s_vals[sort_slots(kSortCap)];
    const int tile = (int)lists[T - 1 - (int)blockIdx.y];
    const uint2 rg = ranges[tile];
    const int n = (int)(rg.y - rg.x);
    const int c0 = (int)blockIdx.x * kSortCap;
    if (c0 >= n) return;
    const int m = min(kSortCap, n - c0);
    block_sort_tile<8, 8>(m, rg.x + c0, pairs, s_keys, s_vals);
    for (int i = threadIdx.x; i < m; i += blockDim.x) {
        const uint32_t sl = sort_slot((uint32_t)i);
        pairs[rg.x + c0 + i] = key_record(s_keys[sl], s_vals[sl]);
    }
}

__device__ inline uint32_t merge_split(const uint4 *__restrict__ a, uint32_t la, const uint4 *__restrict__ b,
                                       uint32_t lb, uint32_t d) {
    const int lane = threadIdx.x & 63;
    uint32_t lo = d > lb ? d - lb : 0u, hi = min(d, la);
    while (lo < hi) {
        const uint32_t span = hi - lo, step = (span + 63) / 64;
        const uint32_t x = lo + (uint32_t)lane * step;
        const bool p = x < hi && pair_key(a[x]) < pair_key(b[d - 1 - x]);
        const uint32_t c = (uint32_t)__popcll(__ballot(p));
        const uint32_t nlo = c ? lo + (c - 1) * step + 1 : lo;
        const uint32_t nhi = min(hi, lo + c * step);
        lo = nlo;
        hi = max(nlo, nhi);
    }
    return lo;
}

__global__ __launch_bounds__(512) void k_merge_pass(int T, const uint32_t *__restrict__ lists,
                                                     const uint2 *__restrict__ ranges, uint32_t L,
                                                     const uint4 *__restrict__ src, uint4 *__restrict__ dst,
                                                     int final_pass, uint32_t *__restrict__ point_list,
                                                     uint32_t *__restrict__ slot_emit) {
    __shared__ uint64_t s_ka[kSortCap], s_kb[kSortCap];
    __shared__ uint32_t s_va[kSortCap], s_vb[kSortCap];
    __shared__ uint32_t s_split[2];
    const int tile = (int)lists[T - 1 - (int)blockIdx.y];
    const uint2 rg = ranges[tile];
    const uint32_t n = rg.y - rg.x;
    const uint32_t o0 = blockIdx.x * (uint32_t)kSortCap;
    if (o0 >= n) return;
    const uint32_t pb = o0 / (2 * L) * (2 * L);
    const uint32_t la = min(L, n - pb), lb = n - pb > L ? min(L, n - pb - L) : 0u;
    const uint4 *a = src + rg.x + pb, *b = a + la;
    const uint32_t d0 = o0 - pb, d1 = min(d0 + (uint32_t)kSortCap, la + lb);
    const int wv = threadIdx.x >> 6;
    if (wv < 2) {
        const uint32_t sp = merge_split(a, la, b, lb, wv == 0 ? d0 : d1);
        if ((threadIdx.x & 63) == 0) s_split[wv] = sp;
    }
    __syncthreads();
    const uint32_t i0 = s_split[0], i1 = s_split[1], j0 = d0 - i0, j1 = d1 - i1;
    const uint32_t na = i1 - i0, nb = j1 - j0;
    for (uint32_t i = threadIdx.x; i < na; i += blockDim.x) { const uint4 q = a[i0 + i]; s_ka[i] = pair_key(q); s_va[i] = q.z; }
    for (uint32_t i = threadIdx.x; i < nb; i += blockDim.x) { const uint4 q = b[j0 + i]; s_kb[i] = pair_key(q); s_vb[i] = q.z; }
    __syncthreads();
    constexpr uint32_t kPer = kSortCap / 512;
    const uint32_t dl = threadIdx.x * kPer;
    if (dl >= na + nb) return;
    uint32_t lo = dl > nb ? dl - nb : 0u, hi = min(dl, na);
    while (lo < hi) {
        const uint32_t mid = (lo + hi) >> 1;
        if (s_ka[mid] < s_kb[dl - 1 - mid]) lo = mid + 1; else hi = mid;
    }
    uint32_t ia = lo, ib = dl - lo;
    const uint32_t e = min(dl + kPer, na + nb);
    for (uint32_t o = dl; o < e; ++o) {
        const bool take_a = ib >= nb || (ia < na && s_ka[ia] < s_kb[ib]);
        const uint64_t k = take_a ? s_ka[ia] : s_kb[ib];
        const uint32_t v = take_a ? s_va[ia] : s_vb[ib];
        ia += take_a; ib += !take_a;
        const size_t slot = (size_t)rg.x + pb + d0 + o;
        if (final_pass) { point_list[slot] = (uint32_t)k; slot_emit[slot] = v; }
        else dst[slot] = key_record(k, v);
    }
}

__device__ inline void gate_wait(const uint32_t *gate, uint32_t seq, uint32_t *err, uint64_t timeout) {
    const uint64_t t0 = __builtin_amdgcn_s_memrealtime();
    while ((int32_t)(__hip_atomic_load(gate, __ATOMIC_ACQUIRE, __HIP_MEMORY_SCOPE_SYSTEM) - seq) < 0) {
        __builtin_amdgcn_s_sleep(100);
        if (__builtin_amdgcn_s_memrealtime() - t0 > timeout) {
            if (threadIdx.x == 0 &&
                (int32_t)(__hip_atomic_load(gate, __ATOMIC_ACQUIRE, __HIP_MEMORY_SCOPE_SYSTEM) - seq) < 0)
                __hip_atomic_store(err, seq, __ATOMIC_RELAXED, __HIP_MEMORY_SCOPE_SYSTEM);
            return;
        }
    }
}

#ifndef GSR_TSAT_THREADS
#define GSR_TSAT_THREADS 64
#endif
constexpr int kTSatThreads = GSR_TSAT_THREADS;
__device__ inline bool tsat_flagged(float T, uint32_t last) { return T < kTSat * (1.0f + t_window(last)); }
struct TSatRec { float4 r0, r1, r3; };
__device__ inline TSatRec tsat_load(const float4 *__restrict__ rec, uint32_t g, bool v) {
    TSatRec t;
    const float4 z = make_float4(0.f, 0.f, 0.f, 0.f);
    const float4 *r = rec + (size_t)kRecF4 * g;
    t.r0 = v ? r[0] : z; t.r1 = v ? r[1] : z; t.r3 = v ? r[3] : z;
    return t;
}
__device__ inline void tsat_chain(int nf, const uint32_t *__restrict__ plist, float pfx, float pfy,
                                  const float4 *__restrict__ rec, uint32_t *s_rc, float *s_q, float *s_a,
                                  uint32_t *s_pos, float &T, uint32_t &nex, float4 &E) {
    constexpr int NT = kTSatThreads, NW = NT / 64;
    const int t = threadIdx.x, lane = t & 63, wv = t >> 6;
    float Tc = 0.f;
    bool stopped = false;
    uint32_t g_next = t < nf ? plist[t] : 0u;
    TSatRec cur = tsat_load(rec, g_next, t < nf);
    g_next = NT + t < nf ? plist[NT + t] : 0u;
    for (int base = 0; base < nf; base += NT) {
        const int e = base + t;
        const TSatRec r = cur;
        cur = tsat_load(rec, g_next, e + NT < nf);
        g_next = e + 2 * NT < nf ? plist[e + 2 * NT] : 0u;
        bool take = false;
        float al = 0.f;
        if (e < nf) {
            const Blend eb = blend_eval<true>(r.r0, r.r1, pfx, pfy);
            if (eb.p2 <= 0.0f && eb.alpha >= kNearLo) {
                const ExactBlend x = exact_blend(r.r0.x, r.r0.y, r.r3, r.r1.y, pfx, pfy);
                take = eb.alpha >= kNearHi || (x.power <= 0.0f && x.alpha >= 1.0f / 255.0f);
                al = x.alpha;
            }
        }
        const uint64_t m = __ballot(take);
        if (lane == 0) s_rc[wv] = (uint32_t)__builtin_popcountll(m);
        __syncthreads();
        uint32_t off = 0, nc = 0;
#pragma unroll
        for (int w = 0; w < NW; ++w) {
            off += w < wv ? s_rc[w] : 0u;
            nc += s_rc[w];
        }
        if (take) {
            const uint32_t rk = off + __builtin_amdgcn_mbcnt_hi((uint32_t)(m >> 32), __builtin_amdgcn_mbcnt_lo((uint32_t)m, 0u));
            s_q[rk] = 1.0f - al;
            s_a[rk] = al;
            s_pos[rk] = (uint32_t)e;
        }
        if (t < 4) s_q[nc + t] = 1.0f;
        __syncthreads();
        if (wv == 0) {
            const float4 *q4 = reinterpret_cast<const float4 *>(s_q);
            for (uint32_t k = 0; k < nc; k += 4) {
                uint32_t j = 0;
                const uint32_t v = min(4u, nc - k);
                if (!stopped) {
                    const float4 q = q4[k >> 2];
                    const float t1 = T * q.x, t2 = t1 * q.y, t3 = t2 * q.z, t4 = t3 * q.w;
                    if (t4 >= kTSat) {
                        T = t4;
                        nex = s_pos[k + v - 1] + 1u;
                        continue;
                    }
                    const float tv[4] = {t1, t2, t3, t4};
                    while (tv[j] >= kTSat) ++j;
                    if (j > 0) {
                        T = tv[j - 1];
                        nex = s_pos[k + j - 1] + 1u;
                    }
                    stopped = true;
                    Tc = T;
                }
                for (; j < v; ++j) {
                    const float a = s_a[k + j];
                    const float4 c = rec[(size_t)kRecF4 * plist[s_pos[k + j]] + 2];
                    const float w = a * Tc;
                    E.x += c.x * w; E.y += c.y * w; E.z += c.z * w; E.w += c.w * w;
                    Tc = Tc * (1.0f - a);
                }
            }
        }
        __syncthreads();
    }
}
__device__ inline void tsat_store(int px, int py, int W, int H, int n, float4 pe, float dfast, float T, uint32_t nex,
                                  float4 E, const float *__restrict__ bg, float *__restrict__ out_color,
                                  float *__restrict__ out_depth, float4 *__restrict__ pix_end,
                                  uint32_t *__restrict__ n_contrib, size_t sb, float4 *__restrict__ seg_state, int ks,
                                  uint32_t *s_nex) {
    const int t = threadIdx.x;
    const int pid = py * W + px;
    const float4 fin = make_float4(pe.x - E.x, pe.y - E.y, pe.z - E.z, T);
    if (t == 0) {
        pix_end[pid] = fin;
        n_contrib[pid] = nex;
        out_color[pid] = fin.x + T * bg[0];
        out_color[H * W + pid] = fin.y + T * bg[1];
        out_color[2 * H * W + pid] = fin.z + T * bg[2];
        out_depth[pid] = dfast - E.w;
    }
    const uint32_t b0 = (nex + (1u << ks) - 1u) >> ks;
    const int lx = px % kTileW, ly = py % kTileH;
    const int bslot = 64 * (ly >> 2) + 16 * (ly & 3) + lx;
    const uint32_t nb = n > 0 ? (uint32_t)(n - 1) >> ks : 0u;
    for (uint32_t q = max(b0, 1u) + (uint32_t)t; q <= nb; q += kTSatThreads)
        seg_state[(sb + q - 1u) * kTilePix + bslot] = fin;
    (void)s_nex;
}
#define GSR_FWD_ATTR __attribute__((amdgpu_waves_per_eu(8, 8)))
template <bool EXACT>
__global__ __launch_bounds__(256) GSR_FWD_ATTR void k_render_fwd(
    int W, int H, int gx, int T, const uint32_t *__restrict__ tile_order, const uint2 *__restrict__ ranges,
    const uint4 *__restrict__ pairs,
    uint32_t *__restrict__ point_list, uint32_t *__restrict__ slot_emit, const float4 *__restrict__ rec,
    const float *__restrict__ bg, float *__restrict__ out_color, float *__restrict__ out_depth,
    float4 *__restrict__ pix_end, uint32_t *__restrict__ n_contrib, uint32_t *__restrict__ tile_maxc,
    const uint32_t *__restrict__ seg_off, float4 *__restrict__ seg_state, const uint32_t *__restrict__ spec_ok,
    int ks, const uint32_t *gate, uint32_t gate_seq, uint32_t *gate_err, uint64_t gate_timeout,
    uint32_t *__restrict__ tile_flag, float4 *__restrict__ near_rec, uint32_t *__restrict__ tsat_n,
    uint32_t *__restrict__ tsat_list, uint32_t tsat_cap) {
    __shared__ uint64_t s_key[sort_slots(kFwdSortCap > 0 ? kFwdSortCap : 1)];
    __shared__ union {
        uint32_t val[sort_slots(kFwdSortCap > 0 ? kFwdSortCap : 1)];
        struct {
            float4 rec[3][66];
            uint32_t q[64];
        } st;
    } s_u;
    __shared__ uint32_t s_live;
    __shared__ uint32_t s_near;
#ifdef GSR_TRACE
    const uint64_t t_start = __builtin_amdgcn_s_memrealtime();
#endif
    if (spec_ok && *spec_ok == 0u) {
        if (gate && blockIdx.x == 0 && threadIdx.x < 64) gate_wait(gate, gate_seq, gate_err, gate_timeout);
        return;
    }
    const int tile = (int)tile_order[blockIdx.x];
    const uint2 rg = ranges[tile];
    const int n = (int)(rg.y - rg.x);
    const bool sorted_here = n <= kFwdSortCap;
    if (threadIdx.x == 0) s_near = 0;
    if (n > 0 && sorted_here) {
        if (n <= 256) block_sort_tile<1, 4>(n, rg.x, pairs, s_key, s_u.val);
        else if (n <= 512) block_sort_tile<2, 4>(n, rg.x, pairs, s_key, s_u.val);
        else block_sort_tile<4, 4>(n, rg.x, pairs, s_key, s_u.val);
        for (int i = threadIdx.x; i < n; i += 256) {
            const uint32_t sl = sort_slot((uint32_t)i);
            point_list[rg.x + i] = (uint32_t)s_key[sl];
            slot_emit[rg.x + i] = s_u.val[sl];
        }
    }
    const int wv = threadIdx.x >> 6, lane = threadIdx.x & 63;
    const int tx = tile % gx, ty = tile / gx;
    const int lx = 8 * (wv & 1) + (lane & 7), ly = 8 * (wv >> 1) + (lane >> 3);
    const int px = tx * kTileW + lx;
    const int py = ty * kTileH + ly;
    const float pfx = (float)px, pfy = (float)py;
    const int bslot = 64 * (ly >> 2) + 16 * (ly & 3) + lx;
    const int se = threadIdx.x >> 2, sq = threadIdx.x & 3;
    const float qx0 = (float)(tx * kTileW + 8 * (sq & 1)), qy0 = (float)(ty * kTileH + 8 * (sq >> 1));
    constexpr int kQW = 8, kQH = 8;
    const bool inside = px < W && py < H;
    constexpr float kThrDone = 2.0f;
    constexpr float kThrLive = EXACT ? kNearLo : 1.0f / 255.0f;
    float thr = inside ? kThrLive : kThrDone;
    const uint32_t pix_key = (uint32_t)(16 * ly + lx);
    if (threadIdx.x == 0) s_live = 0;
    __syncthreads();
#ifdef GSR_TRACE
    const uint64_t tr_sorted = __builtin_amdgcn_s_memrealtime();
#endif
    if (__ballot(thr < kThrDone) && lane == 0) atomicOr(&s_live, 1u << wv);
    float Tt = 1.0f;
    f2v C01 = f2(0.f, 0.f), C2D = f2(0.f, 0.f);
    uint32_t last = 0;
    float4 pa = make_float4(0.f, 0.f, 0.f, 0.f), pb = pa, pr = pa;
    bool pv = false;
#define FETCH_BATCH(bse)                                                                           \
    do {                                                                                           \
        const int idx_ = (bse) + se;                                                               \
        pv = idx_ < n;                                                                             \
        if (pv) {                                                                                  \
            const uint32_t g_ = sorted_here ? (uint32_t)s_key[sort_slot(idx_)] : point_list[rg.x + idx_]; \
            const float4 *r_ = rec + (size_t)kRecF4 * g_;                                          \
            pa = r_[0];                                                                            \
            pb = r_[1];                                                                            \
            pr = r_[sq < 3 ? sq : 2];                                                              \
        }                                                                                          \
    } while (0)
    FETCH_BATCH(0);
#ifdef GSR_TRACE
    uint64_t tr_batches = 0, tr_walk = 0, tr_entries = 0;
#endif
    for (int base = 0; base < n; base += 64) {
        lds_barrier();
        const uint32_t live = s_live;
        if (!live) break;
        if (base > 0 && (base & ((1 << ks) - 1)) == 0) {
            const size_t b = (size_t)seg_off[tile] + ((uint32_t)base >> ks) - 1u;
            seg_state[b * kTilePix + bslot] = make_float4(C01.x, C01.y, C2D.x, Tt);
        }
        bool hit = false, opaque = false;
        {
            const float4 a = pa, b = pb;
            opaque = pv && b.y > 0.99f;
            if (pv) {
                if (sq < 3) s_u.st.rec[sq][se] = pr;
                hit = ((live >> sq) & 1u) &&
                      !tile_cull(a.x, a.y, -2.f * a.z, -a.w, -2.f * b.x, b.y, b.w, qx0, qy0, qx0 + (kQW - 1), qy0 + (kQH - 1));
            }
            FETCH_BATCH(base + 64);
        }
        uint32_t bits = hit ? (1u << sq) : 0u;
        bits |= (uint32_t)__builtin_amdgcn_mov_dpp((int)bits, 0xB1, 0xF, 0xF, false);
        bits |= (uint32_t)__builtin_amdgcn_mov_dpp((int)bits, 0x4E, 0xF, 0xF, false);
        if (sq == 0) s_u.st.q[se] = bits | ((bits && opaque) ? 16u : 0u);
        __syncthreads();
        const uint32_t qw = s_u.st.q[lane];
        uint64_t m = __ballot((qw >> wv) & 1u);
        if (!((live >> wv) & 1u)) m = 0;
        const bool clamp = __builtin_amdgcn_ballot_w64((qw & 16u) != 0u) != 0;
        const float t_stop = EXACT ? kTSat * (1.0f - t_window((uint32_t)base + 64u)) : kTSat;
        auto take = [&](const Blend &e, bool ok, float4 b, float4 c, int j) {
            const float test_T = fmaf(-e.alpha, Tt, Tt);
            const bool use = ok && test_T >= t_stop;
            thr = (ok && !use) ? kThrDone : thr;
            if (use) {
                const float w = e.alpha * Tt;
                C01 = fma2(f2(c.x, c.y), f2(w, w), C01);
                C2D = fma2(f2(c.z, c.w), f2(w, w), C2D);
                Tt = test_T;
                last = (uint32_t)(base + j + 1);
            }
        };
        auto walk = [&](auto clamp_c) {
            constexpr bool CL = decltype(clamp_c)::value;
            while (m) {
                const int j = __builtin_ctzll(m);
                m &= ~(1ull << j);
                const float4 a = s_u.st.rec[0][j], b = s_u.st.rec[1][j], c = s_u.st.rec[2][j];
                Blend e = blend_eval<CL>(a, b, pfx, pfy);
                bool ok = e.p2 <= 0.0f && e.alpha >= thr;
                if constexpr (EXACT) {
                    const bool nr = ok && e.alpha < kNearHi;
                    if (nr) {
                        const int idx = base + j;
                        const uint32_t g = sorted_here ? (uint32_t)s_key[sort_slot(idx)] : point_list[rg.x + idx];
                        const ExactBlend x = exact_blend(a.x, a.y, rec[(size_t)kRecF4 * g + 3], b.y, pfx, pfy);
                        e.p2 = x.power; e.G = x.G; e.alpha = x.alpha;
                        ok = x.power <= 0.0f && x.alpha >= 1.0f / 255.0f;
                        const uint32_t slot = atomicAdd(&s_near, 1u);
                        if (slot < kNearCap)
                            near_rec[(size_t)kNearCap * tile + slot] =
                                make_float4(__uint_as_float(((uint32_t)idx << 8) | pix_key), x.power, x.G, x.alpha);
                    }
                }
                take(e, ok, b, c, j);
            }
        };
#ifdef GSR_TRACE
        const uint64_t tr_w0 = __builtin_amdgcn_s_memrealtime();
        tr_batches += 1;
        tr_entries += (uint64_t)__builtin_popcountll(m);
#endif
        if (clamp) walk(std::true_type{});
        else walk(std::false_type{});
#ifdef GSR_TRACE
        tr_walk += __builtin_amdgcn_s_memrealtime() - tr_w0;
#endif
        if (((live >> wv) & 1u) && !__ballot(thr < kThrDone) && lane == 0) atomicAnd(&s_live, ~(1u << wv));
    }
    if (EXACT && inside && tsat_flagged(Tt, last)) {
        const uint32_t slot = atomicAdd(tsat_n, 1u);
        if (slot < tsat_cap) {
            uint4 *r = reinterpret_cast<uint4 *>(tsat_list) + 2 * (size_t)slot;
            r[0] = make_uint4((uint32_t)(py * W + px), rg.x, (uint32_t)n, last);
            r[1] = make_uint4(__float_as_uint(C01.x), __float_as_uint(C01.y), __float_as_uint(C2D.x), __float_as_uint(C2D.y));
        }
    }
    if (inside) {
        const int pid = py * W + px;
        pix_end[pid] = make_float4(C01.x, C01.y, C2D.x, Tt);
        n_contrib[pid] = last;
        out_color[pid] = C01.x + Tt * bg[0];
        out_color[H * W + pid] = C01.y + Tt * bg[1];
        out_color[2 * H * W + pid] = C2D.x + Tt * bg[2];
        out_depth[pid] = C2D.y;
    }
    uint32_t mx = last;
#pragma unroll
    for (int d = 16; d > 0; d >>= 1) mx = max(mx, (uint32_t)__shfl_xor((int)mx, d, 64));
    __syncthreads();
    if (threadIdx.x < 4) s_u.st.q[threadIdx.x] = 0;
    __syncthreads();
    if ((lane & 31) == 0) atomicMax(&s_u.st.q[2 * (wv >> 1) + (lane >> 5)], mx);
    lds_barrier();
    if (threadIdx.x < 4) tile_maxc[4 * tile + threadIdx.x] = s_u.st.q[threadIdx.x];
    if (threadIdx.x == 0) tile_flag[tile] = EXACT ? s_near : 0u;
#ifdef GSR_TRACE
    trace_wave(g_trace_fwd, 4 * blockIdx.x + wv, t_start, trace_fwd_work(tr_batches, tr_walk, tr_entries));
    if (g_trace_fwd && lane == 0)
        g_trace_fwd[4 * (4 * blockIdx.x + wv) + 2] |= (tr_sorted - t_start) << 40;
#endif
}

#ifndef GSR_TSAT_BLOCKS
#define GSR_TSAT_BLOCKS 4096
#endif
constexpr int kTSatBlocks = GSR_TSAT_BLOCKS;
__global__ __launch_bounds__(kTSatThreads) void k_render_tsat(
    int W, int H, const uint32_t *__restrict__ point_list, const float4 *__restrict__ rec,
    const float *__restrict__ bg, float *__restrict__ out_color, float *__restrict__ out_depth,
    float4 *__restrict__ pix_end, uint32_t *__restrict__ n_contrib, const uint32_t *__restrict__ seg_off,
    float4 *__restrict__ seg_state, const uint32_t *__restrict__ tsat_n, const uint32_t *__restrict__ tsat_list,
    uint32_t tsat_cap, const uint32_t *__restrict__ spec_ok, int ks, int gx, const uint2 *__restrict__ ranges) {
    constexpr int NT = kTSatThreads;
    __shared__ float4 s_buf[(3 * NT + 4 + 3) / 4];
    __shared__ uint32_t s_rc[4];
    if (spec_ok && *spec_ok == 0u) return;
    const uint32_t flagged = *tsat_n;
    const uint32_t cnt = flagged > tsat_cap ? 0u : flagged;
#ifdef GSR_TRACE
    const uint64_t tr_b = __builtin_amdgcn_s_memrealtime();
#endif
    float *s_q = reinterpret_cast<float *>(s_buf), *s_a = s_q + NT + 4;
    uint32_t *s_pos = reinterpret_cast<uint32_t *>(s_a + NT);
    for (uint32_t i = blockIdx.x; i < cnt; i += gridDim.x) {
#ifdef GSR_TRACE
        const uint64_t tr_i = __builtin_amdgcn_s_memrealtime();
#endif
        const uint4 *rp = reinterpret_cast<const uint4 *>(tsat_list) + 2 * (size_t)i;
        const uint4 r0 = rp[0], r1 = rp[1];
        const uint32_t pid = r0.x, start = r0.y;
        const int n = (int)r0.z, nf = (int)r0.w;
        const int px = (int)(pid % (uint32_t)W), py = (int)(pid / (uint32_t)W);
        const int tile = (py / kTileH) * gx + px / kTileW;
        float T = 1.0f;
        uint32_t nex = 0;
        float4 E = make_float4(0.f, 0.f, 0.f, 0.f);
        tsat_chain(nf, point_list + start, (float)px, (float)py, rec, s_rc, s_q, s_a, s_pos, T, nex, E);
#ifdef GSR_TRACE
        const uint64_t tr_c = __builtin_amdgcn_s_memrealtime();
#endif
        if (threadIdx.x == 0) {
            s_rc[0] = nex;
            s_rc[1] = __float_as_uint(T);
            s_q[0] = E.x; s_q[1] = E.y; s_q[2] = E.z; s_q[3] = E.w;
        }
        __syncthreads();
        tsat_store(px, py, W, H, n,
                   make_float4(__uint_as_float(r1.x), __uint_as_float(r1.y), __uint_as_float(r1.z), 0.f),
                   __uint_as_float(r1.w), __uint_as_float(s_rc[1]), s_rc[0],
                   make_float4(s_q[0], s_q[1], s_q[2], s_q[3]), bg, out_color, out_depth, pix_end, n_contrib,
                   seg_off[tile], seg_state, ks, nullptr);
        __syncthreads();
#ifdef GSR_TRACE
        const uint32_t ntile = (uint32_t)gx * (uint32_t)((H + kTileH - 1) / kTileH);
        if (g_trace_fwd && threadIdx.x == 0 && i < 4u * ntile) {
            uint64_t *o = g_trace_fwd + 16 * (size_t)ntile + 4 * (size_t)i;
            o[0] = tr_i;
            o[1] = __builtin_amdgcn_s_memrealtime();
            o[2] = (uint64_t)(uint32_t)nf | ((uint64_t)(uint32_t)n << 32);
            o[3] = (tr_c - tr_i) | ((tr_i - tr_b) << 32);
        }
#endif
    }
    if (__builtin_expect(flagged > tsat_cap, 0)) {
        const uint32_t npix = (uint32_t)W * (uint32_t)H;
        for (uint32_t base = blockIdx.x * 64u; base < npix; base += gridDim.x * 64u) {
            const uint32_t p = base + (threadIdx.x & 63u);
            uint64_t fm = __ballot(p < npix && tsat_flagged(pix_end[p].w, n_contrib[p]));
            __syncthreads();
            while (fm) {
                const uint32_t pid = base + (uint32_t)__builtin_ctzll(fm);
                fm &= fm - 1;
                const int px = (int)(pid % (uint32_t)W), py = (int)(pid / (uint32_t)W);
                const int tile = (py / kTileH) * gx + px / kTileW;
                const uint2 rg = ranges[tile];
                const float4 pe = pix_end[pid];
                const int nf = (int)n_contrib[pid];
                const float dfast = out_depth[pid];
                float T = 1.0f;
                uint32_t nex = 0;
                float4 E = make_float4(0.f, 0.f, 0.f, 0.f);
                tsat_chain(nf, point_list + rg.x, (float)px, (float)py, rec, s_rc, s_q, s_a, s_pos, T, nex, E);
                if (threadIdx.x == 0) {
                    s_rc[0] = nex;
                    s_rc[1] = __float_as_uint(T);
                    s_q[0] = E.x; s_q[1] = E.y; s_q[2] = E.z; s_q[3] = E.w;
                }
                __syncthreads();
                tsat_store(px, py, W, H, (int)(rg.y - rg.x), make_float4(pe.x, pe.y, pe.z, 0.f), dfast,
                           __uint_as_float(s_rc[1]), s_rc[0], make_float4(s_q[0], s_q[1], s_q[2], s_q[3]), bg,
                           out_color, out_depth, pix_end, n_contrib, seg_off[tile], seg_state, ks, nullptr);
                __syncthreads();
            }
        }
    }
}

__global__ void k_zero_f32(float *p, size_t n) {
    const size_t i = (size_t)blockIdx.x * blockDim.x + threadIdx.x;
    if (i < n) p[i] = 0.f;
}

__global__ void k_mark_visible(int P, const float *__restrict__ means3D,
                               const float *__restrict__ viewmatrix, uint8_t *__restrict__ present) {
    const int i = blockIdx.x * blockDim.x + threadIdx.x;
    if (i >= P) return;
    float vm[16];
#pragma unroll
    for (int k = 0; k < 16; ++k) vm[k] = viewmatrix[k];
    const float3 pv = xform4x3(make_float3(means3D[3 * i], means3D[3 * i + 1], means3D[3 * i + 2]), vm);
    present[i] = !(pv.z <= 0.2f);
}

template <int MC>
static void preprocess_mc(const FwdArgs &a, hipStream_t s) {
    k_preprocess<MC><<<div_up(a.v.P, kShBlock), kShBlock, sizeof(float) * kShBlock * (MC ? sh_row_stride(MC) : 0), s>>>(
        a.v.P, a.v.D, a.v.M, a.v.means3D, a.v.scales, a.v.scale_modifier, a.v.rotations, a.v.opacities, a.v.shs,
        a.v.colors_precomp, a.v.cov3D_precomp, a.v.viewmatrix, a.v.projmatrix, a.v.campos, a.v.W, a.v.H, a.v.tan_fovx,
        a.v.tan_fovy, a.v.focal_x, a.v.focal_y, a.v.gx, a.v.gy, a.radii, a.depth, a.rec, a.rect, a.tiles, a.v.act, a.v.cs,
        a.tile_count, a.v.gx * a.v.gy, a.clampm);
}

hipError_t launch_preprocess(const FwdArgs &a, hipStream_t s) {
    if (a.v.P == 0) return hipSuccess;
    const int mc = a.v.shs ? a.v.M : 0;
    switch (mc) {
        case 16: preprocess_mc<16>(a, s); break;
        case 9: preprocess_mc<9>(a, s); break;
        case 4: preprocess_mc<4>(a, s); break;
        case 1: preprocess_mc<1>(a, s); break;
        default: preprocess_mc<0>(a, s); break;
    }
    return hipGetLastError();
}

hipError_t launch_bin_count(const FwdArgs &a, hipStream_t s) {
    const BinGrid bg(a.v.P);
    const int T = a.v.gx * a.v.gy;
    if (bg.NB == 0) return hipSuccess;
    if (T <= kMaxLdsTiles)
        k_bin_count<true><<<bg.NB, kBinThreads, sizeof(uint32_t) * T, s>>>(a.v.P, bg.CH, T, a.v.gx, a.rect, a.tiles, a.tile_count, a.block_sums, a.chunk_off, a.items_ws, a.scan_ws);
    else
        k_bin_count<false><<<bg.NB, kBinThreads, 0, s>>>(a.v.P, bg.CH, T, a.v.gx, a.rect, a.tiles, a.tile_count, a.block_sums, nullptr, a.items_ws, nullptr);
    return hipGetLastError();
}

hipError_t launch_bin_scan(const FwdArgs &a, uint32_t *host_words, hipStream_t s) {
    const BinGrid bg(a.v.P);
    const int T = a.v.gx * a.v.gy;
    if (T <= kMaxLdsTiles && bg.NB > 0)
        k_bin_colscan<<<div_up(T, kColW), kColW * kColG, 0, s>>>(T, bg.NB, a.chunk_off, a.tile_count, a.ranges,
                                                                a.tile_cursor, a.seg_off, a.sort_lists, a.tile_rank,
                                                                a.scan_ws, a.block_sums, a.block_off, a.meta,
                                                                host_words, a.spec_cap, seg_log2(a.v.P));
    else
        k_bin_scan<<<1, 1024, 0, s>>>(T, bg.NB, a.tile_count, a.ranges, a.tile_cursor,
                                      a.block_sums, a.block_off, a.meta, host_words, a.tile_order_f,
                                      a.sort_lists, a.seg_off, a.spec_cap, seg_log2(a.v.P));
    return hipGetLastError();
}

hipError_t launch_bin_emit(const FwdArgs &a, int K, hipStream_t s) {
    const BinGrid bg(a.v.P);
    const int T = a.v.gx * a.v.gy;
    if (bg.NB == 0) return hipSuccess;
    if (T <= kMaxLdsTiles)
        k_bin_emit<true><<<bg.NB, kBinThreads, sizeof(uint32_t) * T, s>>>(a.v.P, bg.CH, T, a.v.gx, a.rect, a.tiles, a.depth, a.block_off, a.tile_cursor, a.goff, a.pairs, (uint32_t)K, a.chunk_off, a.spec_ok,
                                                                           a.tile_count, a.tile_rank, a.scan_ws + 2 * kScanBlocksMax + kScanCtr, a.tile_order_f);
    else
        k_bin_emit<false><<<bg.NB, kBinThreads, 0, s>>>(a.v.P, bg.CH, T, a.v.gx, a.rect, a.tiles, a.depth, a.block_off, a.tile_cursor, a.goff, a.pairs, (uint32_t)K, a.chunk_off, a.spec_ok,
                                                        nullptr, nullptr, nullptr, nullptr);
    return hipGetLastError();
}

hipError_t launch_tile_sort(const FwdArgs &a, uint32_t n_mid, uint32_t n_vlong, uint32_t max_n, uint4 *tmp,
                            hipStream_t s) {
    const int T = a.v.gx * a.v.gy;
    if (a.spec_ok) {
        const int nb = a.spec_sort_blocks ? (int)a.spec_sort_blocks : kSpecSortBlocks;
        k_tile_sort<<<std::min(T, nb), 512, 0, s>>>(a.v.gx, a.sort_lists, a.ranges, a.pairs, a.point_list,
                                                                 a.slot_emit, 0u, a.spec_ok);
        return hipGetLastError();
    }
    if (n_mid) k_tile_sort<<<n_mid, 512, 0, s>>>(a.v.gx, a.sort_lists, a.ranges, a.pairs, a.point_list, a.slot_emit,
                                                 n_mid, nullptr);
    if (n_vlong) {
        const dim3 grid((unsigned)div_up((int)max_n, kSortCap), n_vlong);
        k_chunk_sort<<<grid, 512, 0, s>>>(T, a.sort_lists, a.ranges, a.pairs);
        const uint4 *src = a.pairs;
        uint4 *dst = tmp;
        for (uint32_t L = kSortCap; L < max_n; L *= 2) {
            const int final_pass = 2 * (size_t)L >= max_n;
            k_merge_pass<<<grid, 512, 0, s>>>(T, a.sort_lists, a.ranges, L, src, dst, final_pass, a.point_list,
                                              a.slot_emit);
            const uint4 *t = dst;
            dst = const_cast<uint4 *>(src);
            src = t;
        }
    }
    return hipGetLastError();
}

hipError_t launch_render_fwd(const FwdArgs &a, hipStream_t s) {
    const int T = a.v.gx * a.v.gy;
    auto k = a.exact ? k_render_fwd<true> : k_render_fwd<false>;
    k<<<T, 256, 0, s>>>(a.v.W, a.v.H, a.v.gx, T, a.tile_order_f, a.ranges, a.pairs,
                        a.point_list, a.slot_emit, a.rec, a.v.bg, a.out_color, a.out_depth, a.pix_end, a.n_contrib,
                        a.tile_maxc, a.seg_off, a.seg_state, a.spec_ok, seg_log2(a.v.P), a.gate, a.gate_seq,
                        a.gate_err, a.gate_timeout, a.tile_flag, a.near_rec, a.items_ws + kTSatCtr, a.tsat_list,
                        tsat_capacity(a.v.W * a.v.H));
    if (a.exact)
        k_render_tsat<<<kTSatBlocks, kTSatThreads, 0, s>>>(a.v.W, a.v.H, a.point_list, a.rec, a.v.bg, a.out_color, a.out_depth,
                                                 a.pix_end, a.n_contrib, a.seg_off, a.seg_state, a.items_ws + kTSatCtr,
                                                 a.tsat_list, tsat_capacity(a.v.W * a.v.H), a.spec_ok, seg_log2(a.v.P),
                                                 a.v.gx, a.ranges);
    return hipGetLastError();
}

hipError_t launch_zero(float *p, size_t n, hipStream_t s) {
    if (n == 0) return hipSuccess;
    k_zero_f32<<<(unsigned)((n + 255) / 256), 256, 0, s>>>(p, n);
    return hipGetLastError();
}

hipError_t launch_mark_visible(int P, const float *means3D, const float *viewmatrix, uint8_t *present,
                               hipStream_t s) {
    if (P == 0) return hipSuccess;
    k_mark_visible<<<div_up(P, 256), 256, 0, s>>>(P, means3D, viewmatrix, present);
    return hipGetLastError();
}

}

#ifdef GSR_TRACE
extern "C" int gsr_debug_trace_fwd(void *buf) {
    return hipMemcpyToSymbol(HIP_SYMBOL(gsr::g_trace_fwd), &buf, sizeof(buf)) == hipSuccess ? 0 : 2;
}
extern "C" int gsr_debug_trace_emit(void *buf) {
    return hipMemcpyToSymbol(HIP_SYMBOL(gsr::g_trace_emit), &buf, sizeof(buf)) == hipSuccess ? 0 : 2;
}
#endif
```

animating-gaussian-splats_amd/csrc/gsr_internal.h:

```cpp
#pragma once
#include <hip/hip_runtime.h>
#include <stdint.h>

namespace gsr {

struct ViewIn {
    int P, D, M, W, H, gx, gy, act;
    float scale_modifier, tan_fovx, tan_fovy, focal_x, focal_y;
    const float *means3D, *scales, *rotations, *opacities, *shs, *colors_precomp, *cov3D_precomp;
    const float *viewmatrix, *projmatrix, *campos, *bg;
    CamStrides cs;
};

struct FwdArgs {
    ViewIn v;
    float *depth; float4 *rec; uint2 *rect; uint32_t *tiles; uint32_t *goff; uint8_t *clampm;
    uint2 *ranges; float4 *pix_end; uint32_t *n_contrib; uint32_t *tile_maxc;
    uint32_t *tile_order_f; uint32_t *seg_off; uint32_t *sort_lists; uint32_t *tile_count;
    uint32_t *tile_cursor; uint32_t *block_sums; uint32_t *block_off; uint32_t *meta; uint32_t *chunk_off;
    uint32_t *items_ws; uint32_t *scan_ws; uint32_t *tile_rank;
    uint32_t *tile_flag; float4 *near_rec;
    uint32_t *tsat_list;
    uint4 *pairs; uint32_t *point_list; uint32_t *slot_emit; float4 *seg_state;
    int *radii; float *out_color; float *out_depth;
    uint32_t spec_cap; const uint32_t *spec_ok;
    uint32_t spec_sort_blocks;
    const uint32_t *gate; uint32_t gate_seq; uint32_t *gate_err; uint64_t gate_timeout;
    int exact;
};
constexpr int kSpecSortBlocks = 512;

struct BwdArgs {
    ViewIn v;
    int K;
    const int *radii;
    const float4 *rec; const uint2 *rect; const uint8_t *clampm;
    const uint32_t *goff; const uint2 *ranges; const float4 *pix_end; const uint32_t *n_contrib;
    const uint32_t *tile_maxc; const uint32_t *tile_flag; const float4 *near_rec; const uint32_t *seg_off; const uint32_t *meta; uint32_t *items_ws;
    const uint32_t *point_list; const uint32_t *slot_emit; const float4 *seg_state;
    uint2 *items; uint32_t max_items;
    float4 *part;
    const float *dL_dcolor;
    float *dL_dmeans2D, *dL_dcolors, *dL_dopacity, *dL_dmeans3D, *dL_dcov3D, *dL_dsh, *dL_dscales,
        *dL_drot;
    int accm;
    const uint32_t *spec_ok;
};

hipError_t launch_preprocess(const FwdArgs &a, hipStream_t s);
hipError_t launch_bin_count(const FwdArgs &a, hipStream_t s);
hipError_t launch_bin_scan(const FwdArgs &a, uint32_t *host_words, hipStream_t s);
hipError_t launch_bin_emit(const FwdArgs &a, int K, hipStream_t s);
hipError_t launch_tile_sort(const FwdArgs &a, uint32_t n_mid, uint32_t n_vlong, uint32_t max_n, uint4 *tmp,
                            hipStream_t s);
hipError_t launch_render_fwd(const FwdArgs &a, hipStream_t s);
hipError_t launch_zero(float *p, size_t n, hipStream_t s);
hipError_t launch_mark_visible(int P, const float *means3D, const float *viewmatrix, uint8_t *present,
                               hipStream_t s);

hipError_t launch_bwd_items(const BwdArgs &a, hipStream_t s);
hipError_t launch_bwd_items_raw(int K, int T, int P, const uint2 *ranges, const uint32_t *tile_maxc,
                                const uint32_t *tile_flag, uint2 *items, uint32_t *ws, hipStream_t s,
                                const uint32_t *spec_ok = nullptr);
hipError_t launch_render_bwd(const BwdArgs &a, hipStream_t s);
hipError_t launch_gauss_bwd(const BwdArgs &a, hipStream_t s);
hipError_t launch_sum_records(int P, const uint32_t *goff, const float4 *part, float *sums, hipStream_t s,
                              const uint32_t *spec_ok, const float *viewmatrix, const float *projmatrix,
                              const float *campos, CamStrides cs, int W, int H);

constexpr int kMultiViews = 8;
struct MultiView {
    const float *viewmatrix, *projmatrix, *campos;
    CamStrides cs;
    float tan_fovx, tan_fovy, focal_x, focal_y;
    const int *radii;
    const float4 *rec;
    const uint8_t *clampm;
    const float *sums;
    float *dL_dmeans2D;
    int acc2;
};
struct MultiArgs {
    int P, D, M, nv, act, accm;
    float scale_modifier;
    const float *means3D, *scales, *rotations, *shs, *cov3D_precomp;
    float *dL_dcolors, *dL_dopacity, *dL_dmeans3D, *dL_dcov3D, *dL_dsh, *dL_dscales, *dL_drot;
    MultiView v[kMultiViews];
};
hipError_t launch_gauss_bwd_multi(const MultiArgs &a, hipStream_t s);

struct SsimWindow { float w[11]; };
size_t ssim_partials(int planes, int H, int W);
hipError_t launch_ssim_fwd(int planes, int H, int W, const float *img1, const float *img2, const SsimWindow &w,
                           float *maps, float2 *partial, float *out_l1, float *out_ssim, hipStream_t s);
hipError_t launch_ssim_bwd(int planes, int H, int W, const float *img1, const float *img2, const SsimWindow &w,
                           const float *maps, const float *g_l1, const float *g_ssim, float *dimg1,
                           hipStream_t s);

hipError_t launch_knn(int n, const float *pts, int k, int *out_idx, double *out_d2, hipStream_t s);
int rigid_blocks(int F);
hipError_t launch_rigid_fwd(int F, int k, const float *means, const float *quats, const int *fg_rows,
                            const int *nbr_rows, const float *weights, const float *prev_off, const float *prev_inv,
                            double *partial, float *save_u, float *save_m, float *save_q, float *out_loss,
                            hipStream_t s);
hipError_t launch_rigid_bwd(int P, int F, int k, const int *row_to_fg, const int *rev_off, const int *rev_edge,
                            const float *save_u, const float *save_m, const float *save_q, const float *g_loss,
                            float *dmeans, float *dquats, hipStream_t s);

constexpr int kDeformAutoBlocks = 256;
constexpr int kPosencRangeBlocks = 256;
hipError_t launch_posenc_ranges(int P, const float *means, const float *quats, float *partial, float *ranges,
                                hipStream_t s);
hipError_t launch_posenc(int P, const float *means, const float *quats, const float *ranges, float *out, hipStream_t s);
hipError_t launch_deform_in_fwd(int P, int H, const float *im, const float *iq, const float *ir, const float *pm,
                                const float *pq, const float *pr, float progress, const float *W, const float *bias,
                                float *Y, hipStream_t s);
int deform_in_blocks(int P, int max_blocks);
size_t deform_in_partial_floats(int P, int H, int max_blocks);
hipError_t launch_deform_in_bwd(int P, int H, const float *im, const float *iq, const float *ir, const float *pm,
                                const float *pq, const float *pr, float progress, const float *dY, float *partial,
                                int max_blocks, float *dW, float *db, hipStream_t s);

struct DensArgs {
    int P, prune_big;
    float grad_threshold, small_scale, big_scale, remove_opacity, inv_split_div;
    const float *grad_accum, *vis_count, *log_scales, *opacity_logits, *rotations;
};
struct DensColumn {
    int width, role;
    const float *src, *m_src, *v_src;
    float *dst, *m_dst, *v_dst;
};
constexpr int kDensMaxColumns = 8;
struct DensColumns { int n; DensColumn c[kDensMaxColumns]; };
struct DensWorkspace {
    int NB;
    size_t flags, bsum, boff, totals, total;
    explicit DensWorkspace(int P);
};
hipError_t launch_dens_radii(int P, const int *radii, float *max_radii, uint8_t *visible, hipStream_t s);
hipError_t launch_dens_grads(int P, const uint8_t *visible, const float *m2grad, float *grad_accum,
                             float *vis_count, hipStream_t s);
hipError_t launch_dens_plan(const DensArgs &a, char *ws, hipStream_t s);
hipError_t launch_dens_stds(const DensArgs &a, const char *ws, float *stds, hipStream_t s);
hipError_t launch_dens_apply(const DensArgs &a, const char *ws, const float *samples, const DensColumns &cols,
                             hipStream_t s);

struct AdamTensor {
    float *param; const float *grad; float *exp_avg; float *exp_avg_sq;
    long long n; float step_size, bc2_sqrt; int vec4;
};
constexpr int kAdamMaxTensors = 16;
struct AdamTable {
    int n; float w1, b2, omb2, eps;
    AdamTensor t[kAdamMaxTensors];
    int block_start[kAdamMaxTensors + 1];
};
int adam_blocks(long long n);
hipError_t launch_adam(const AdamTable &tab, hipStream_t s);

hipError_t launch_views_pack(int frames, int HW, const uint8_t *rgb, const uint8_t *seg, float *img, float *msk,
                             hipStream_t s);

}
```

animating-gaussian-splats_amd/diff_gaussian_rasterization/_C.py:

```python
from __future__ import annotations

import ctypes
import os
import threading

import torch

_HERE = os.path.dirname(os.path.abspath(__file__))
LIB_PATH = os.environ.get("GSR_LIB", os.path.join(_HERE, "libgsr.so"))

GSR_BUF_GEOM, GSR_BUF_BINNING, GSR_BUF_IMAGE, GSR_BUF_SCRATCH, GSR_BUF_SUMS = 0, 1, 2, 3, 4
EXPORTED_SYMBOLS = (
    "gsr_forward", "gsr_backward", "gsr_mark_visible", "gsr_geom_bytes", "gsr_image_bytes",
    "gsr_binning_bytes", "gsr_scratch_bytes", "gsr_last_error", "gsr_abi_version",
    "gsr_profile_enable", "gsr_profile_select", "gsr_profile_reset", "gsr_profile_read", "gsr_buffer_offsets",
    "gsr_ssim_scratch_bytes", "gsr_l1_ssim_forward", "gsr_l1_ssim_backward",
    "gsr_densify_update_radii", "gsr_densify_accumulate_grads", "gsr_densify_workspace_bytes",
    "gsr_densify_plan", "gsr_densify_split_stds", "gsr_densify_apply", "gsr_adam_step", "gsr_views_pack",
    "gsr_grad_fence", "gsr_backward_render", "gsr_backward_gaussians", "gsr_backward_items_bytes",
    "gsr_forward_info_call", "gsr_spec_stats", "gsr_sums_bytes", "gsr_prealloc_alloc", "gsr_spec_binning_bytes",
    "gsr_forward_async", "gsr_forward_resolve", "gsr_forward_release", "gsr_forward_query", "gsr_async_stats",
    "gsr_spec_keys", "gsr_async_shutdown", "gsr_debug_async_fault", "gsr_set_exact_thresholds",
    "gsr_knn", "gsr_rigidity_scratch_bytes", "gsr_rigidity_forward", "gsr_rigidity_backward",
    "gsr_posenc_ranges", "gsr_posenc_forward", "gsr_deform_in_forward", "gsr_deform_in_workspace_bytes",
# ... 608 lines not shown
                     float(tan_fovy), dL_dout_color, e if sh is None else sh, int(degree),
                     e if campos is None else campos, _bp(geomBuffer), int(R), binning_ptr or _bp(binningBuffer),
                     _bp(imageBuffer), int(activations), bool(prepare_backward), int(binning_layout or 0),
                     list(out), int(acc_bits), _PREALLOC_ON)
        return out
    keep = []
    g, P, M = _gaussians(means3D, sh, degree, colors, torch.empty(0, device=means3D.device), scales,
                         rotations, scale_modifier, cov3D_precomp, keep, activations, prepare_backward,
                         binning_layout)
    H, W = dL_dout_color.shape[-2], dL_dout_color.shape[-1]
    cam = _camera(viewmatrix, projmatrix, tan_fovx, tan_fovy, H, W, campos, background, False, keep)
    dev = means3D.device
    skip = tuple(k for k in range(8) if needed is not None and not needed[k])
    out, acc_bits = _grad_outputs(P, M, dev, colors, cov3D_precomp, scales, rotations, skip_unused,
                                  accumulate_into, skip=skip)
    if P == 0:
        return out
    dpix = dL_dout_color.contiguous().float()
    keep.append(dpix)
    grads = _Grads(*[t.data_ptr() if t is not None and t.numel() else None for t in out], acc_bits)
    alloc = _PreAllocator(dev, [[(GSR_BUF_SCRATCH, L.gsr_scratch_bytes(int(R), W, H))]])
    with _device_guard(dev), alloc:
        _check(L.gsr_backward(ctypes.byref(cam), ctypes.byref(g), radii.data_ptr(), int(R),
                              _bp(geomBuffer), binning_ptr or _bp(binningBuffer), _bp(imageBuffer),
                              dpix.data_ptr(), None, alloc.cb, alloc.ctx, ctypes.byref(grads), _stream_ptr(dev)))
    return out


def rasterize_gaussians_backward_render(background, means3D, radii, colors, scales, rotations,
                                        scale_modifier, cov3D_precomp, viewmatrix, projmatrix, tan_fovx,
                                        tan_fovy, dL_dout_color, sh, degree, campos, geomBuffer, R,
                                        binningBuffer, imageBuffer, activations=0, prepare_backward=False,
                                        binning_layout=0, binning_ptr=None):
    L = load_library()
    nat = _native() if _NATIVE_PARTS & 2 else None
    if nat is not None:
        e = _EMPTY
        sums, _ = nat.backward_render(
            background, means3D, radii, e if colors is None else colors, e if scales is None else scales,
            e if rotations is None else rotations, float(scale_modifier), e if cov3D_precomp is None else cov3D_precomp,
            viewmatrix, projmatrix, float(tan_fovx), float(tan_fovy), dL_dout_color, e if sh is None else sh,
            int(degree), e if campos is None else campos, _bp(geomBuffer), int(R),
            binning_ptr or _bp(binningBuffer), _bp(imageBuffer), int(activations), bool(prepare_backward),
            int(binning_layout or 0), _PREALLOC_ON)
        return sums
    keep = []
    g, P, _ = _gaussians(means3D, sh, degree, colors, torch.empty(0, device=means3D.device), scales,
                         rotations, scale_modifier, cov3D_precomp, keep, activations, prepare_backward,
                         binning_layout)
    H, W = dL_dout_color.shape[-2], dL_dout_color.shape[-1]
    cam = _camera(viewmatrix, projmatrix, tan_fovx, tan_fovy, H, W, campos, background, False, keep)
    dev = means3D.device
    if P == 0:
        return torch.empty(1, dtype=torch.uint8, device=dev)
    dpix = dL_dout_color.contiguous().float()
    keep.append(dpix)
    alloc = _PreAllocator(dev, [[(GSR_BUF_SCRATCH, L.gsr_scratch_bytes(int(R) if R >= 0 else int(binning_layout), W, H))],
                                [(GSR_BUF_SUMS, L.gsr_sums_bytes(P))]])
    with _device_guard(dev), alloc:
        _check(L.gsr_backward_render(ctypes.byref(cam), ctypes.byref(g), radii.data_ptr(), int(R),
                                     _bp(geomBuffer), binning_ptr or _bp(binningBuffer), _bp(imageBuffer),
                                     dpix.data_ptr(), alloc.cb, alloc.ctx, _stream_ptr(dev)))
    return alloc.buffers[GSR_BUF_SUMS]


def rasterize_gaussians_backward_views(views, means3D, colors, scales, rotations, scale_modifier,
                                       cov3D_precomp, sh, degree, activations=0, skip_unused=True,
                                       accumulate_into=None, overwrite=(), needed=None):
    L = load_library()
    keep = []
    dev = means3D.device
    g, P, M = _gaussians(means3D, sh, degree, colors, torch.empty(0, device=dev), scales, rotations,
                         scale_modifier, cov3D_precomp, keep, activations)
    skip = (0,) + tuple(k for k in range(1, 8) if needed is not None and not needed[k])
    out, acc_bits = _grad_outputs(P, M, dev, colors, cov3D_precomp, scales, rotations, skip_unused,
                                  accumulate_into, skip=skip, overwrite=overwrite)
    if P == 0 or not views:
        return out
    nat = _native() if _NATIVE_PARTS & 4 else None
    if nat is not None:
        e = _EMPTY
        nat.backward_views(list(views), means3D, e if colors is None else colors, e if scales is None else scales,
                           e if rotations is None else rotations, float(scale_modifier),
                           e if cov3D_precomp is None else cov3D_precomp, e if sh is None else sh, int(degree),
                           int(activations), list(out), int(acc_bits))
        return out
    cams = []
    vg = (_ViewGrad * len(views))()
    cs = torch.cuda.current_stream(dev)
    for k, v in enumerate(views):
        cam = _camera(v["viewmatrix"], v["projmatrix"], v["tanfovx"], v["tanfovy"], v["image_height"],
                      v["image_width"], v["campos"], v["bg"], False, keep)
        cams.append(cam)
        m2 = v.get("means2D_grad")
        if m2 is not None:
            if tuple(m2.shape) != (P, 3) or m2.dtype != torch.float32 or not m2.is_contiguous() or m2.device != dev:
                raise RuntimeError(f"views[{k}]['means2D_grad']: expected a contiguous float32 ({P}, 3) tensor on {dev}")
            m2.record_stream(cs)
        for t in (v["radii"], v["scratch"], *v.get("keep", ()),
                  *((v["geomBuffer"],) if isinstance(v["geomBuffer"], torch.Tensor) else ())):
            t.record_stream(cs)
        vg[k] = _ViewGrad(ctypes.pointer(cam), v["radii"].data_ptr(), _bp(v["geomBuffer"]),
                          v["scratch"].data_ptr(), int(v["num_rendered"]),
                          m2.data_ptr() if m2 is not None else None, int(bool(v.get("accumulate_means2D"))))
    grads = _Grads(*[t.data_ptr() if t is not None and t.numel() else None for t in out], acc_bits)
    with _device_guard(dev):
        _check(L.gsr_backward_gaussians(len(views), vg, ctypes.byref(g), ctypes.byref(grads), _stream_ptr(dev)))
    return out


def grad_fence(*grads):
    grads = [g for g in grads if g is not None and g.numel()]
    if not grads:
        return
    dev = grads[0].device
    arr = (ctypes.c_void_p * len(grads))(*[g.data_ptr() for g in grads])
    with _device_guard(dev):
        _check(load_library().gsr_grad_fence(arr, len(grads), _stream_ptr(dev)))


def mark_visible(means3D, viewmatrix, projmatrix):
    L = load_library()
    P = means3D.size(0)
    present = torch.zeros((P,), dtype=torch.bool, device=means3D.device)
    if P == 0:
        return present
    m = means3D.contiguous().float()
    vm, pm = viewmatrix.contiguous().float(), projmatrix.contiguous().float()
    with _device_guard(means3D.device):
        _check(L.gsr_mark_visible(P, _ptr(m), _ptr(vm), _ptr(pm), present.data_ptr(),
                                  _stream_ptr(means3D.device)))
    return present


def profile_enable(on=True):
    _check(load_library().gsr_profile_enable(int(bool(on))))


def profile_select(phases=None):
    _check(load_library().gsr_profile_select(",".join(phases).encode() if phases else None))


def profile_reset():
    _check(load_library().gsr_profile_reset())


def profile_read(phase=None):
    L = load_library()
    tot, cnt = ctypes.c_double(0), ctypes.c_int(0)
    _check(L.gsr_profile_read(phase.encode() if phase else None, ctypes.byref(tot), ctypes.byref(cnt)))
    return tot.value, cnt.value


def decode_buffers(P, W, H, num_rendered, geomBuffer, binningBuffer, imgBuffer, binning_layout=0):
    L = load_library()
    offs = (ctypes.c_size_t * 16)()
    L.gsr_buffer_offsets(int(P), int(W), int(H), int(binning_layout or num_rendered), offs, 16)
    o = list(offs)
    T = ((W + 15) // 16) * ((H + 15) // 16)
    K = int(num_rendered)

    def view(buf, off, n, dtype, shape):
        nbytes = n * torch.tensor([], dtype=dtype).element_size()
        return buf[off:off + nbytes].view(dtype).reshape(shape)

    f32, i32, i64 = torch.float32, torch.int32, torch.int64
    rec = view(geomBuffer, o[1], 16 * P, f32, (P, 16))
    return {
        "depth": view(geomBuffer, o[0], P, f32, (P,)),
        "rec": rec,
        "xy": rec[:, 0:2],
        "conic_opacity": torch.stack([rec[:, 12], rec[:, 13], rec[:, 14], rec[:, 5]], 1),
        "rgbd": torch.cat([rec[:, 8:11], rec[:, 6:7]], 1),
        "tau2": rec[:, 7],
        "rect": view(geomBuffer, o[2], 2 * P, i32, (P, 2)),
        "tiles_touched": view(geomBuffer, o[3], P, i32, (P,)),
        "goff": view(geomBuffer, o[4], P + 1, i32, (P + 1,)),
        "ranges": view(imgBuffer, o[5], 2 * T, i32, (T, 2)),
        "pix_end": view(imgBuffer, o[6], 4 * W * H, f32, (H, W, 4)),
        "final_T": view(imgBuffer, o[6], 4 * W * H, f32, (H, W, 4))[..., 3],
        "seg_off": view(imgBuffer, o[12], T + 1, i32, (T + 1,)),
        "n_contrib": view(imgBuffer, o[7], W * H, i32, (H, W)),
        "tile_maxc": view(imgBuffer, o[8], 4 * T, i32, (T, 4)),
        "tile_flag": view(imgBuffer, o[14], T, i32, (T,)),
        "tsat_count": view(imgBuffer, o[15], 1, i32, (1,)),
        "pairs": view(binningBuffer, o[9], 4 * K, i32, (K, 4)),
        "keys": view(binningBuffer, o[9], 2 * K, i64, (K, 2))[:, 0],
        "point_list": view(binningBuffer, o[10], K, i32, (K,)),
        "slot_emit": view(binningBuffer, o[11], K, i32, (K,)),
    }
```

Before: 1418 Msplats/s.

## Replace per-pair slot_emit array with per-Gaussian emit map to shrink sort pairs

Sort pairs shrink from uint4 to uint2 by dropping the emit slot value, and the per-pair slot_emit array is removed. A per-Gaussian emap (base offset and rect width) is written at emit time, and backward recomputes each slot from the tile coordinates. This cuts memory traffic in emit, sort, merge and the forward render, and removes value shuffles from the bitonic sort. The cost is an extra gather of emap in the backward pass and in its zeroing loops.

```diff
diff --git a/animating-gaussian-splats_amd/csrc/gsr_api.hip b/animating-gaussian-splats_amd/csrc/gsr_api.hip
--- a/animating-gaussian-splats_amd/csrc/gsr_api.hip
+++ b/animating-gaussian-splats_amd/csrc/gsr_api.hip
@@ -197,6 +197,7 @@
     const GeomLayout G(a.v.P);
     a.rec = (float4 *)(geom + G.rec); a.rect = (uint2 *)(geom + G.rect);
     a.goff = (uint32_t *)(geom + G.goff); a.clampm = (uint8_t *)(geom + G.clampm);
+    a.emap = (uint2 *)(geom + G.emap);
     const ImageLayout L(a.v.W, a.v.H, a.v.P);
     a.ranges = (uint2 *)(img + L.ranges); a.pix_end = (float4 *)(img + L.pix_end);
     a.n_contrib = (uint32_t *)(img + L.n_contrib); a.tile_maxc = (uint32_t *)(img + L.tile_maxc);
@@ -217,7 +218,7 @@
 }
 template <typename A>
 void carve_binning(A &a, char *bin, const BinningLayout &L) {
-    a.point_list = (uint32_t *)(bin + L.point_list); a.slot_emit = (uint32_t *)(bin + L.slot_emit);
+    a.point_list = (uint32_t *)(bin + L.point_list);
     a.seg_state = (float4 *)(bin + L.seg_state);
 }
 
@@ -227,7 +228,7 @@
     BinRegions(int K, int P, int T, bool with_items, bool with_merge) : arrays(K, P) {
         items = arrays.total;
         tmp = items + (with_items ? bwd_items_bytes(K, T) : 0);
-        total = tmp + (with_merge ? sizeof(uint4) * (size_t)K : 0);
+        total = tmp + (with_merge ? sizeof(uint2) * (size_t)K : 0);
     }
 };
 
@@ -235,9 +236,9 @@
                       bool prepare_backward, int T, hipStream_t s, const uint32_t *spec_ok, bool phases) {
     const BinRegions R(layout, a.v.P, T, prepare_backward, n_vlong != 0);
     carve_binning(a, bin, R.arrays);
-    a.pairs = (uint4 *)(bin + R.arrays.pairs);
+    a.pairs = (uint2 *)(bin + R.arrays.pairs);
     a.spec_ok = spec_ok;
-    uint4 *tmp = n_vlong ? (uint4 *)(bin + R.tmp) : nullptr;
+    uint2 *tmp = n_vlong ? (uint2 *)(bin + R.tmp) : nullptr;
     uint2 *items = (uint2 *)(bin + R.items);
     { Phase ph(s, "bin_emit", phases); HIP_TRY(launch_bin_emit(a, spec_ok ? 0 : layout, s)); }
     { Phase ph(s, "tile_sort", phases); HIP_TRY(launch_tile_sort(a, n_mid, n_vlong, max_n, tmp, s)); }
@@ -302,7 +303,7 @@
     const BinningLayout b(K, P);
     const size_t v[16] = {g.depth, g.rec, g.rect, g.tiles, g.goff,
                           im.ranges, im.pix_end, im.n_contrib, im.tile_maxc,
-                          b.pairs, b.point_list, b.slot_emit, im.seg_off, b.seg_state, im.tile_flag,
+                          b.pairs, b.point_list, b.reserved, im.seg_off, b.seg_state, im.tile_flag,
                           im.items_ws + sizeof(uint32_t) * kTSatCtr};
     int n = 0;
     for (; n < 16 && n < max_out; ++n) out[n] = v[n];
diff --git a/animating-gaussian-splats_amd/csrc/gsr_backward.hip b/animating-gaussian-splats_amd/csrc/gsr_backward.hip
--- a/animating-gaussian-splats_amd/csrc/gsr_backward.hip
+++ b/animating-gaussian-splats_amd/csrc/gsr_backward.hip
@@ -252,7 +252,7 @@
     const float4 *__restrict__ rec, const float *__restrict__ bg, const float4 *__restrict__ pix_end,
     const uint32_t *__restrict__ n_contrib, const uint32_t *__restrict__ tile_maxc,
     const uint32_t *__restrict__ seg_off, const float4 *__restrict__ seg_state,
-    const uint32_t *__restrict__ slot_emit, const float *__restrict__ dL_dpixels,
+    const uint2 *__restrict__ emap, const float *__restrict__ dL_dpixels,
     float4 *__restrict__ part, int ks, const uint32_t *__restrict__ tile_flag,
     const float4 *__restrict__ near_rec, float4 *s_a, float *s_out) {
     constexpr int kStage = 64 * kBwdWaves;
@@ -272,20 +272,31 @@
     const float tx1 = tx0 + (kTileW - 1);
     const uint4 mq = reinterpret_cast<const uint4 *>(tile_maxc)[tile];
     const int maxc = min((int)max(max(mq.x, mq.y), max(mq.z, mq.w)), n);
+    auto zero_slots = [&](int z0, int z1) {
+        constexpr int kZeroAhead = 4;
+        for (int p0 = z0 + lane; p0 < z1; p0 += 64 * kZeroAhead) {
+            uint32_t g[kZeroAhead];
+#pragma unroll
+            for (int u = 0; u < kZeroAhead; ++u) g[u] = p0 + 64 * u < z1 ? point_list[rg.x + p0 + 64 * u] : 0u;
+            uint2 em[kZeroAhead] = {};
+#pragma unroll
+            for (int u = 0; u < kZeroAhead; ++u)
+                if (p0 + 64 * u < z1) em[u] = emap[g[u]];
+#pragma unroll
+            for (int u = 0; u < kZeroAhead; ++u)
+                if (p0 + 64 * u < z1)
+                    rec_store(part, em[u].x + (uint32_t)ty * em[u].y + (uint32_t)tx, 0.f, 0.f, 0.f, 0.f, 0.f, 0.f, 0.f, 0.f, 0.f);
+        }
+    };
     if (seg & kZeroItem) {
         const int z0 = maxc + (int)kZeroChunk * (int)((seg & ~kZeroItem) + 1);
-        for (int p = z0 + lane; p < min(n, z0 + (int)kZeroChunk); p += 64) {
-            rec_store(part, slot_emit[rg.x + p], 0.f, 0.f, 0.f, 0.f, 0.f, 0.f, 0.f, 0.f, 0.f);
-        }
+        zero_slots(z0, min(n, z0 + (int)kZeroChunk));
         return;
     }
     const int s0 = (int)seg << ks, s1f = s0 + (1 << ks);
     const int s1 = min(s1f, maxc);
-    if (s1f >= maxc) {
-        for (int p = maxc + lane; p < min(n, maxc + (int)kZeroChunk); p += 64) {
-            rec_store(part, slot_emit[rg.x + p], 0.f, 0.f, 0.f, 0.f, 0.f, 0.f, 0.f, 0.f, 0.f);
-        }
-    }
+    if (s1f >= maxc)
+        zero_slots(maxc, min(n, maxc + (int)kZeroChunk));
     const float half_w = (float)(0.5 * W), half_h = (float)(0.5 * H);
     const float bg0 = bg[0], bg1 = bg[1], bg2 = bg[2];
     PixState ps[4];
@@ -317,13 +328,10 @@
     const RowW rw = row_weights(lane >> 4);
     float *o_row = s_out + (lane >> 4);
     NearRecs nrs{near_rec + (size_t)kNearCap * tile, EXACT ? 0u : tile_flag[tile], 0};
-    uint32_t g_n = 0, em_n = 0;
+    uint32_t g_n = 0;
     auto fetch = [&](int e) {
         const int st = e - 64 > s0 ? e - 64 : s0;
-        if (lane < e - st) {
-            g_n = point_list[rg.x + st + lane];
-            em_n = slot_emit[rg.x + st + lane];
-        }
+        if (lane < e - st) g_n = point_list[rg.x + st + lane];
     };
     if (s1 > s0) fetch(s1);
     for (int end = s1; end > s0; end -= 64) {
@@ -333,8 +341,9 @@
         float2 tl = make_float2(0.f, 0.f);
         if (lane < cnt) {
             const float4 *r = rec + (size_t)kRecF4 * g_n;
+            const uint2 em = emap[g_n];
             a = r[0]; b = r[1]; c = r[2]; cj = r[3];
-            tl = make_float2(cj.z, __uint_as_float(em_n));
+            tl = make_float2(cj.z, __uint_as_float(em.x + (uint32_t)ty * em.y + (uint32_t)tx));
         }
         if (end - 64 > s0) fetch(end - 64);
 #pragma unroll
@@ -403,7 +412,7 @@
     const float4 *__restrict__ rec, const float *__restrict__ bg, const float4 *__restrict__ pix_end,
     const uint32_t *__restrict__ n_contrib, const uint32_t *__restrict__ tile_maxc,
     const uint32_t *__restrict__ seg_off, const float4 *__restrict__ seg_state,
-    const uint32_t *__restrict__ slot_emit, const float *__restrict__ dL_dpixels,
+    const uint2 *__restrict__ emap, const float *__restrict__ dL_dpixels,
     float4 *__restrict__ part, int ks, const uint32_t *__restrict__ spec_ok,
     const uint32_t *__restrict__ tile_flag, const float4 *__restrict__ near_rec) {
     constexpr int kStage = 64 * kBwdWaves;
@@ -416,11 +425,11 @@
     const uint2 hd = items[0];
     if constexpr (EXACT) {
         for (uint32_t i = blockIdx.x * kBwdWaves + wv; i < hd.y; i += gridDim.x * kBwdWaves)
-            bwd_item<true>(items[1 + hd.x + i], hd.x + i, W, H, gx, ranges, point_list, rec, bg, pix_end, n_contrib, tile_maxc, seg_off, seg_state, slot_emit, dL_dpixels, part, ks, tile_flag, near_rec, s_a, s_out);
+            bwd_item<true>(items[1 + hd.x + i], hd.x + i, W, H, gx, ranges, point_list, rec, bg, pix_end, n_contrib, tile_maxc, seg_off, seg_state, emap, dL_dpixels, part, ks, tile_flag, near_rec, s_a, s_out);
     } else {
         const uint32_t item = blockIdx.x * kBwdWaves + wv;
         if (item >= hd.x) return;
-        bwd_item<false>(items[1 + item], item, W, H, gx, ranges, point_list, rec, bg, pix_end, n_contrib, tile_maxc, seg_off, seg_state, slot_emit, dL_dpixels, part, ks, tile_flag, near_rec, s_a, s_out);
+        bwd_item<false>(items[1 + item], item, W, H, gx, ranges, point_list, rec, bg, pix_end, n_contrib, tile_maxc, seg_off, seg_state, emap, dL_dpixels, part, ks, tile_flag, near_rec, s_a, s_out);
     }
 }
 
@@ -1167,10 +1176,10 @@
     const int ks = seg_log2(a.v.P);
     k_render_bwd<false><<<div_up((int)a.max_items, kBwdWaves), 64 * kBwdWaves, 0, s>>>(
         a.v.W, a.v.H, a.v.gx, a.items, a.ranges, a.point_list, a.rec, a.v.bg, a.pix_end, a.n_contrib, a.tile_maxc, a.seg_off,
-        a.seg_state, a.slot_emit, a.dL_dcolor, a.part, ks, a.spec_ok, a.tile_flag, a.near_rec);
+        a.seg_state, a.emap, a.dL_dcolor, a.part, ks, a.spec_ok, a.tile_flag, a.near_rec);
     k_render_bwd<true><<<std::min(div_up((int)a.max_items, kBwdWaves), kExactBwdBlocks), 64 * kBwdWaves, 0, s>>>(
         a.v.W, a.v.H, a.v.gx, a.items, a.ranges, a.point_list, a.rec, a.v.bg, a.pix_end, a.n_contrib, a.tile_maxc, a.seg_off,
-        a.seg_state, a.slot_emit, a.dL_dcolor, a.part, ks, a.spec_ok, a.tile_flag, a.near_rec);
+        a.seg_state, a.emap, a.dL_dcolor, a.part, ks, a.spec_ok, a.tile_flag, a.near_rec);
     return hipGetLastError();
 }
 
diff --git a/animating-gaussian-splats_amd/csrc/gsr_common.h b/animating-gaussian-splats_amd/csrc/gsr_common.h
--- a/animating-gaussian-splats_amd/csrc/gsr_common.h
+++ b/animating-gaussian-splats_amd/csrc/gsr_common.h
@@ -12,7 +12,7 @@
 constexpr int kPartial = 9;
 constexpr int kRecF = kPartial;
 constexpr int kSortCap = 4096;
-__host__ __device__ inline uint64_t pair_key(uint4 r) { return ((uint64_t)r.y << 32) | r.x; }
+__host__ __device__ inline uint64_t pair_key(uint2 r) { return ((uint64_t)r.y << 32) | r.x; }
 #ifndef GSR_FWD_SORT_CAP
 #define GSR_FWD_SORT_CAP 1024
 #endif
@@ -24,7 +24,7 @@
 
 constexpr int kRecF4 = 4;
 struct GeomLayout {
-    size_t depth, rec, rect, tiles, goff, clampm, total;
+    size_t depth, rec, rect, tiles, goff, clampm, emap, total;
     __host__ __device__ GeomLayout(int P) {
         size_t o = 0;
         depth = o;    o = align256(o + sizeof(float) * P);
@@ -33,6 +33,7 @@
         tiles = o;    o = align256(o + sizeof(uint32_t) * P);
         goff = o;     o = align256(o + sizeof(uint32_t) * (P + 1));
         clampm = o;   o = align256(o + (size_t)P);
+        emap = o;     o = align256(o + sizeof(uint2) * P);
         total = o;
     }
 };
@@ -132,12 +133,12 @@
 };
 
 struct BinningLayout {
-    size_t pairs, point_list, slot_emit, seg_state, total;
+    size_t pairs, point_list, reserved, seg_state, total;
     __host__ __device__ BinningLayout(int K, int P) {
         size_t o = 0;
-        pairs = o;      o = align256(o + sizeof(uint4) * (K > 0 ? K : 1));
+        pairs = o;      o = align256(o + sizeof(uint2) * (K > 0 ? K : 1));
         point_list = o; o = align256(o + sizeof(uint32_t) * (K > 0 ? K : 1));
-        slot_emit = o;  o = align256(o + sizeof(uint32_t) * (K > 0 ? K : 1));
+        reserved = o;
         seg_state = o;  o = align256(o + sizeof(float4) * kTilePix * (size_t)(((size_t)(K > 0 ? K : 0) >> seg_log2(P)) + 1));
         total = o;
     }
diff --git a/animating-gaussian-splats_amd/csrc/gsr_forward.hip b/animating-gaussian-splats_amd/csrc/gsr_forward.hip
--- a/animating-gaussian-splats_amd/csrc/gsr_forward.hip
+++ b/animating-gaussian-splats_amd/csrc/gsr_forward.hip
@@ -383,8 +383,8 @@
                                                   const float *__restrict__ depth,
                                                   const uint32_t *__restrict__ block_off,
                                                   uint32_t *__restrict__ tile_cursor,
-                                                  uint32_t *__restrict__ goff,
-                                                  uint4 *__restrict__ pairs, uint32_t K,
+                                                  uint32_t *__restrict__ goff, uint2 *__restrict__ emap,
+                                                  uint2 *__restrict__ pairs, uint32_t K,
                                                   const uint32_t *__restrict__ chunk_off,
                                                   const uint32_t *__restrict__ spec_ok,
                                                   const uint32_t *__restrict__ tile_count,
@@ -418,18 +418,21 @@
         carry += tot;
         if (g < g1) {
             goff[g] = ex;
+            uint2 em = make_uint2(ex, 0u);
             if (n) {
                 const uint2 r = rects[g];
                 const int x0 = r.x & 0xFFFF, y0 = r.x >> 16, x1 = r.y & 0xFFFF, y1 = r.y >> 16;
                 const uint32_t dbits = __float_as_uint(depth[g]);
-                uint32_t e = ex;
+                const uint32_t w = (uint32_t)(x1 - x0);
+                em = make_uint2(ex - ((uint32_t)y0 * w + (uint32_t)x0), w);
                 for (int y = y0; y < y1; ++y)
-                    for (int x = x0; x < x1; ++x, ++e) {
+                    for (int x = x0; x < x1; ++x) {
                         const int t = y * gx + x;
                         const uint32_t pos = USE_LDS ? atomicAdd(&s_cur[t], 1u) : atomicAdd(&tile_cursor[t], 1u);
-                        pairs[pos] = make_uint4((uint32_t)g, dbits, e, 0u);
+                        pairs[pos] = make_uint2((uint32_t)g, dbits);
                     }
             }
+            emap[g] = em;
         }
     }
     if (b == gridDim.x - 1 && threadIdx.x == 0) goff[P] = spec_ok ? spec_ok[-1] : K;
@@ -458,20 +461,18 @@
 }
 
 template <int R, int D>
-__device__ inline void bitonic_xlane(uint64_t (&k)[R], uint32_t (&v)[R], bool take_min) {
+__device__ inline void bitonic_xlane(uint64_t (&k)[R], bool take_min) {
 #pragma unroll
     for (int r = 0; r < R; ++r) {
         const uint32_t plo = lane_xor<D>((uint32_t)k[r]), phi = lane_xor<D>((uint32_t)(k[r] >> 32));
-        const uint32_t pv = lane_xor<D>(v[r]);
         const uint64_t pk = ((uint64_t)phi << 32) | plo;
         const bool mine = (k[r] < pk) == take_min;
         k[r] = mine ? k[r] : pk;
-        v[r] = mine ? v[r] : pv;
     }
 }
 
 template <int R, int J>
-__device__ inline void wave_merge_stages(uint64_t (&k)[R], uint32_t (&v)[R], int lane, uint32_t gbase, uint32_t KK) {
+__device__ inline void wave_merge_stages(uint64_t (&k)[R], int lane, uint32_t gbase, uint32_t KK) {
     if constexpr (J > 0) {
         if constexpr (J < R) {
 #pragma unroll
@@ -479,26 +480,23 @@
                 if (r & J) continue;
                 const int r2 = r | J;
                 const bool asc = ((gbase + lane * R + r) & KK) == 0;
-                if ((k[r] > k[r2]) == asc) {
-                    const uint64_t t = k[r]; k[r] = k[r2]; k[r2] = t;
-                    const uint32_t u = v[r]; v[r] = v[r2]; v[r2] = u;
-                }
+                if ((k[r] > k[r2]) == asc) { const uint64_t t = k[r]; k[r] = k[r2]; k[r2] = t; }
             }
         } else {
             constexpr int D = J / R;
             const bool asc = ((gbase + lane * R) & KK) == 0;
             const bool take_min = ((lane & D) == 0) == asc;
-            bitonic_xlane<R, D>(k, v, take_min);
-        }
-        wave_merge_stages<R, J / 2>(k, v, lane, gbase, KK);
+            bitonic_xlane<R, D>(k, take_min);
+        }
+        wave_merge_stages<R, J / 2>(k, lane, gbase, KK);
     }
 }
 
 template <int R, int KK>
-__device__ inline void wave_sort_stages(uint64_t (&k)[R], uint32_t (&v)[R], int lane, uint32_t gbase) {
+__device__ inline void wave_sort_stages(uint64_t (&k)[R], int lane, uint32_t gbase) {
     if constexpr (KK <= 64 * R) {
-        wave_merge_stages<R, KK / 2>(k, v, lane, gbase, KK);
-        wave_sort_stages<R, 2 * KK>(k, v, lane, gbase);
+        wave_merge_stages<R, KK / 2>(k, lane, gbase, KK);
+        wave_sort_stages<R, 2 * KK>(k, lane, gbase);
     }
 }
 
@@ -506,59 +504,50 @@
 constexpr int sort_slots(int n) { return n + n / 16; }
 
 template <int R>
-__device__ inline void block_xchg_stage(uint64_t (&k)[R], uint32_t (&v)[R], uint32_t ibase, int kk, int j,
-                                        uint64_t *s_key, uint32_t *s_val) {
+__device__ inline void block_xchg_stage(uint64_t (&k)[R], uint32_t ibase, int kk, int j, uint64_t *s_key) {
     const uint32_t sb = sort_slot(ibase), qb = sort_slot(ibase ^ (uint32_t)j);
 #pragma unroll
-    for (int r = 0; r < R; ++r) { s_key[sb + r] = k[r]; s_val[sb + r] = v[r]; }
+    for (int r = 0; r < R; ++r) s_key[sb + r] = k[r];
     __syncthreads();
 #pragma unroll
     for (int r = 0; r < R; ++r) {
         const uint32_t i = ibase + r;
         const uint64_t pk = s_key[qb + r];
-        const uint32_t pv = s_val[qb + r];
         const bool take_min = ((i & j) == 0) == ((i & kk) == 0);
         const bool mine = (k[r] < pk) == take_min;
         k[r] = mine ? k[r] : pk;
-        v[r] = mine ? v[r] : pv;
     }
     __syncthreads();
 }
 
 template <int R, int NW>
-__device__ inline void block_sort_tile(int n, uint32_t start, const uint4 *__restrict__ pairs, uint64_t *s_key,
-                                       uint32_t *s_val) {
+__device__ inline void block_sort_tile(int n, uint32_t start, const uint2 *__restrict__ pairs, uint64_t *s_key) {
     constexpr int SEG = 64 * R;
     const int lane = threadIdx.x & 63, w = threadIdx.x >> 6;
     const uint32_t gbase = (uint32_t)(w * SEG), ibase = gbase + lane * R;
     uint64_t k[R];
-    uint32_t v[R];
 #pragma unroll
     for (int r = 0; r < R; ++r) {
         const int i = (int)ibase + r;
-        const uint4 q = i < n ? pairs[start + i] : make_uint4(~0u, ~0u, 0u, 0u);
-        k[r] = pair_key(q);
-        v[r] = q.z;
-    }
-    wave_sort_stages<R, 2>(k, v, lane, gbase);
+        k[r] = i < n ? pair_key(pairs[start + i]) : ~0ull;
+    }
+    wave_sort_stages<R, 2>(k, lane, gbase);
     for (uint32_t kk = 2 * SEG; kk <= (uint32_t)(NW * SEG); kk <<= 1) {
-        for (uint32_t j = kk >> 1; j >= (uint32_t)SEG; j >>= 1) block_xchg_stage<R>(k, v, ibase, kk, j, s_key, s_val);
-        wave_merge_stages<R, SEG / 2>(k, v, lane, gbase, kk);
+        for (uint32_t j = kk >> 1; j >= (uint32_t)SEG; j >>= 1) block_xchg_stage<R>(k, ibase, kk, j, s_key);
+        wave_merge_stages<R, SEG / 2>(k, lane, gbase, kk);
     }
     const uint32_t sb = sort_slot(ibase);
 #pragma unroll
-    for (int r = 0; r < R; ++r) { s_key[sb + r] = k[r]; s_val[sb + r] = v[r]; }
+    for (int r = 0; r < R; ++r) s_key[sb + r] = k[r];
     __syncthreads();
 }
 
 __global__ __launch_bounds__(512) void k_tile_sort(int gx, const uint32_t *__restrict__ tiles,
                                                     const uint2 *__restrict__ ranges,
-                                                    uint4 *__restrict__ pairs,
-                                                    uint32_t *__restrict__ point_list,
-                                                    uint32_t *__restrict__ slot_emit, uint32_t nlist,
+                                                    const uint2 *__restrict__ pairs,
+                                                    uint32_t *__restrict__ point_list, uint32_t nlist,
                                                     const uint32_t *__restrict__ spec_ok) {
     __shared__ uint64_t s_keys[sort_slots(kSortCap)];
-    __shared__ uint32_t s_vals[sort_slots(kSortCap)];
     if (spec_ok) {
         if (*spec_ok == 0u) return;
         nlist = spec_ok[1];
@@ -568,39 +557,29 @@
         const int tile = (int)tiles[li];
         const uint2 rg = ranges[tile];
         const int n = (int)(rg.y - rg.x);
-        if (n <= 4 * 64 * 8) block_sort_tile<4, 8>(n, rg.x, pairs, s_keys, s_vals);
-        else block_sort_tile<8, 8>(n, rg.x, pairs, s_keys, s_vals);
-        for (int i = threadIdx.x; i < n; i += blockDim.x) {
-            const uint32_t sl = sort_slot((uint32_t)i);
-            point_list[rg.x + i] = (uint32_t)s_keys[sl];
-            slot_emit[rg.x + i] = s_vals[sl];
-        }
+        if (n <= 4 * 64 * 8) block_sort_tile<4, 8>(n, rg.x, pairs, s_keys);
+        else block_sort_tile<8, 8>(n, rg.x, pairs, s_keys);
+        for (int i = threadIdx.x; i < n; i += blockDim.x) point_list[rg.x + i] = (uint32_t)s_keys[sort_slot((uint32_t)i)];
         __syncthreads();
     }
 }
 
-__device__ inline uint4 key_record(uint64_t k, uint32_t emit) {
-    return make_uint4((uint32_t)k, (uint32_t)(k >> 32), emit, 0u);
-}
+__device__ inline uint2 key_record(uint64_t k) { return make_uint2((uint32_t)k, (uint32_t)(k >> 32)); }
 
 __global__ __launch_bounds__(512) void k_chunk_sort(int T, const uint32_t *__restrict__ lists,
-                                                     const uint2 *__restrict__ ranges, uint4 *__restrict__ pairs) {
+                                                     const uint2 *__restrict__ ranges, uint2 *__restrict__ pairs) {
     __shared__ uint64_t s_keys[sort_slots(kSortCap)];
-    __shared__ uint32_t s_vals[sort_slots(kSortCap)];
     const int tile = (int)lists[T - 1 - (int)blockIdx.y];
     const uint2 rg = ranges[tile];
     const int n = (int)(rg.y - rg.x);
     const int c0 = (int)blockIdx.x * kSortCap;
     if (c0 >= n) return;
     const int m = min(kSortCap, n - c0);
-    block_sort_tile<8, 8>(m, rg.x + c0, pairs, s_keys, s_vals);
-    for (int i = threadIdx.x; i < m; i += blockDim.x) {
-        const uint32_t sl = sort_slot((uint32_t)i);
-        pairs[rg.x + c0 + i] = key_record(s_keys[sl], s_vals[sl]);
-    }
-}
-
-__device__ inline uint32_t merge_split(const uint4 *__restrict__ a, uint32_t la, const uint4 *__restrict__ b,
+    block_sort_tile<8, 8>(m, rg.x + c0, pairs, s_keys);
+    for (int i = threadIdx.x; i < m; i += blockDim.x) pairs[rg.x + c0 + i] = key_record(s_keys[sort_slot((uint32_t)i)]);
+}
+
+__device__ inline uint32_t merge_split(const uint2 *__restrict__ a, uint32_t la, const uint2 *__restrict__ b,
                                        uint32_t lb, uint32_t d) {
     const int lane = threadIdx.x & 63;
     uint32_t lo = d > lb ? d - lb : 0u, hi = min(d, la);
@@ -619,11 +598,9 @@
 
 __global__ __launch_bounds__(512) void k_merge_pass(int T, const uint32_t *__restrict__ lists,
                                                      const uint2 *__restrict__ ranges, uint32_t L,
-                                                     const uint4 *__restrict__ src, uint4 *__restrict__ dst,
-                                                     int final_pass, uint32_t *__restrict__ point_list,
-                                                     uint32_t *__restrict__ slot_emit) {
+                                                     const uint2 *__restrict__ src, uint2 *__restrict__ dst,
+                                                     int final_pass, uint32_t *__restrict__ point_list) {
     __shared__ uint64_t s_ka[kSortCap], s_kb[kSortCap];
-    __shared__ uint32_t s_va[kSortCap], s_vb[kSortCap];
     __shared__ uint32_t s_split[2];
     const int tile = (int)lists[T - 1 - (int)blockIdx.y];
     const uint2 rg = ranges[tile];
@@ -632,7 +609,7 @@
     if (o0 >= n) return;
     const uint32_t pb = o0 / (2 * L) * (2 * L);
     const uint32_t la = min(L, n - pb), lb = n - pb > L ? min(L, n - pb - L) : 0u;
-    const uint4 *a = src + rg.x + pb, *b = a + la;
+    const uint2 *a = src + rg.x + pb, *b = a + la;
     const uint32_t d0 = o0 - pb, d1 = min(d0 + (uint32_t)kSortCap, la + lb);
     const int wv = threadIdx.x >> 6;
     if (wv < 2) {
@@ -642,8 +619,8 @@
     __syncthreads();
     const uint32_t i0 = s_split[0], i1 = s_split[1], j0 = d0 - i0, j1 = d1 - i1;
     const uint32_t na = i1 - i0, nb = j1 - j0;
-    for (uint32_t i = threadIdx.x; i < na; i += blockDim.x) { const uint4 q = a[i0 + i]; s_ka[i] = pair_key(q); s_va[i] = q.z; }
-    for (uint32_t i = threadIdx.x; i < nb; i += blockDim.x) { const uint4 q = b[j0 + i]; s_kb[i] = pair_key(q); s_vb[i] = q.z; }
+    for (uint32_t i = threadIdx.x; i < na; i += blockDim.x) s_ka[i] = pair_key(a[i0 + i]);
+    for (uint32_t i = threadIdx.x; i < nb; i += blockDim.x) s_kb[i] = pair_key(b[j0 + i]);
     __syncthreads();
     constexpr uint32_t kPer = kSortCap / 512;
     const uint32_t dl = threadIdx.x * kPer;
@@ -658,11 +635,10 @@
     for (uint32_t o = dl; o < e; ++o) {
         const bool take_a = ib >= nb || (ia < na && s_ka[ia] < s_kb[ib]);
         const uint64_t k = take_a ? s_ka[ia] : s_kb[ib];
-        const uint32_t v = take_a ? s_va[ia] : s_vb[ib];
         ia += take_a; ib += !take_a;
         const size_t slot = (size_t)rg.x + pb + d0 + o;
-        if (final_pass) { point_list[slot] = (uint32_t)k; slot_emit[slot] = v; }
-        else dst[slot] = key_record(k, v);
+        if (final_pass) point_list[slot] = (uint32_t)k;
+        else dst[slot] = key_record(k);
     }
 }
 
@@ -796,8 +772,8 @@
 template <bool EXACT>
 __global__ __launch_bounds__(256) GSR_FWD_ATTR void k_render_fwd(
     int W, int H, int gx, int T, const uint32_t *__restrict__ tile_order, const uint2 *__restrict__ ranges,
-    const uint4 *__restrict__ pairs,
-    uint32_t *__restrict__ point_list, uint32_t *__restrict__ slot_emit, const float4 *__restrict__ rec,
+    const uint2 *__restrict__ pairs,
+    uint32_t *__restrict__ point_list, const float4 *__restrict__ rec,
     const float *__restrict__ bg, float *__restrict__ out_color, float *__restrict__ out_depth,
     float4 *__restrict__ pix_end, uint32_t *__restrict__ n_contrib, uint32_t *__restrict__ tile_maxc,
     const uint32_t *__restrict__ seg_off, float4 *__restrict__ seg_state, const uint32_t *__restrict__ spec_ok,
@@ -806,7 +782,6 @@
     uint32_t *__restrict__ tsat_list, uint32_t tsat_cap) {
     __shared__ uint64_t s_key[sort_slots(kFwdSortCap > 0 ? kFwdSortCap : 1)];
     __shared__ union {
-        uint32_t val[sort_slots(kFwdSortCap > 0 ? kFwdSortCap : 1)];
         struct {
             float4 rec[3][66];
             uint32_t q[64];
@@ -827,14 +802,10 @@
     const bool sorted_here = n <= kFwdSortCap;
     if (threadIdx.x == 0) s_near = 0;
     if (n > 0 && sorted_here) {
-        if (n <= 256) block_sort_tile<1, 4>(n, rg.x, pairs, s_key, s_u.val);
-        else if (n <= 512) block_sort_tile<2, 4>(n, rg.x, pairs, s_key, s_u.val);
-        else block_sort_tile<4, 4>(n, rg.x, pairs, s_key, s_u.val);
-        for (int i = threadIdx.x; i < n; i += 256) {
-            const uint32_t sl = sort_slot((uint32_t)i);
-            point_list[rg.x + i] = (uint32_t)s_key[sl];
-            slot_emit[rg.x + i] = s_u.val[sl];
-        }
+        if (n <= 256) block_sort_tile<1, 4>(n, rg.x, pairs, s_key);
+        else if (n <= 512) block_sort_tile<2, 4>(n, rg.x, pairs, s_key);
+        else block_sort_tile<4, 4>(n, rg.x, pairs, s_key);
+        for (int i = threadIdx.x; i < n; i += 256) point_list[rg.x + i] = (uint32_t)s_key[sort_slot((uint32_t)i)];
     }
     const int wv = threadIdx.x >> 6, lane = threadIdx.x & 63;
     const int tx = tile % gx, ty = tile / gx;
@@ -871,7 +842,7 @@
             const float4 *r_ = rec + (size_t)kRecF4 * g_;                                          \
             pa = r_[0];                                                                            \
             pb = r_[1];                                                                            \
-            pr = r_[sq < 3 ? sq : 2];                                                              \
+            if (sq < 3) pr = r_[sq];                                                               \
         }                                                                                          \
     } while (0)
     FETCH_BATCH(0);
@@ -1154,36 +1125,35 @@
     const int T = a.v.gx * a.v.gy;
     if (bg.NB == 0) return hipSuccess;
     if (T <= kMaxLdsTiles)
-        k_bin_emit<true><<<bg.NB, kBinThreads, sizeof(uint32_t) * T, s>>>(a.v.P, bg.CH, T, a.v.gx, a.rect, a.tiles, a.depth, a.block_off, a.tile_cursor, a.goff, a.pairs, (uint32_t)K, a.chunk_off, a.spec_ok,
+        k_bin_emit<true><<<bg.NB, kBinThreads, sizeof(uint32_t) * T, s>>>(a.v.P, bg.CH, T, a.v.gx, a.rect, a.tiles, a.depth, a.block_off, a.tile_cursor, a.goff, a.emap, a.pairs, (uint32_t)K, a.chunk_off, a.spec_ok,
                                                                            a.tile_count, a.tile_rank, a.scan_ws + 2 * kScanBlocksMax + kScanCtr, a.tile_order_f);
     else
-        k_bin_emit<false><<<bg.NB, kBinThreads, 0, s>>>(a.v.P, bg.CH, T, a.v.gx, a.rect, a.tiles, a.depth, a.block_off, a.tile_cursor, a.goff, a.pairs, (uint32_t)K, a.chunk_off, a.spec_ok,
+        k_bin_emit<false><<<bg.NB, kBinThreads, 0, s>>>(a.v.P, bg.CH, T, a.v.gx, a.rect, a.tiles, a.depth, a.block_off, a.tile_cursor, a.goff, a.emap, a.pairs, (uint32_t)K, a.chunk_off, a.spec_ok,
                                                         nullptr, nullptr, nullptr, nullptr);
     return hipGetLastError();
 }
 
-hipError_t launch_tile_sort(const FwdArgs &a, uint32_t n_mid, uint32_t n_vlong, uint32_t max_n, uint4 *tmp,
+hipError_t launch_tile_sort(const FwdArgs &a, uint32_t n_mid, uint32_t n_vlong, uint32_t max_n, uint2 *tmp,
                             hipStream_t s) {
     const int T = a.v.gx * a.v.gy;
     if (a.spec_ok) {
         const int nb = a.spec_sort_blocks ? (int)a.spec_sort_blocks : kSpecSortBlocks;
         k_tile_sort<<<std::min(T, nb), 512, 0, s>>>(a.v.gx, a.sort_lists, a.ranges, a.pairs, a.point_list,
-                                                                 a.slot_emit, 0u, a.spec_ok);
+                                                                 0u, a.spec_ok);
         return hipGetLastError();
     }
-    if (n_mid) k_tile_sort<<<n_mid, 512, 0, s>>>(a.v.gx, a.sort_lists, a.ranges, a.pairs, a.point_list, a.slot_emit,
+    if (n_mid) k_tile_sort<<<n_mid, 512, 0, s>>>(a.v.gx, a.sort_lists, a.ranges, a.pairs, a.point_list,
                                                  n_mid, nullptr);
     if (n_vlong) {
         const dim3 grid((unsigned)div_up((int)max_n, kSortCap), n_vlong);
         k_chunk_sort<<<grid, 512, 0, s>>>(T, a.sort_lists, a.ranges, a.pairs);
-        const uint4 *src = a.pairs;
-        uint4 *dst = tmp;
+        const uint2 *src = a.pairs;
+        uint2 *dst = tmp;
         for (uint32_t L = kSortCap; L < max_n; L *= 2) {
             const int final_pass = 2 * (size_t)L >= max_n;
-            k_merge_pass<<<grid, 512, 0, s>>>(T, a.sort_lists, a.ranges, L, src, dst, final_pass, a.point_list,
-                                              a.slot_emit);
-            const uint4 *t = dst;
-            dst = const_cast<uint4 *>(src);
+            k_merge_pass<<<grid, 512, 0, s>>>(T, a.sort_lists, a.ranges, L, src, dst, final_pass, a.point_list);
+            const uint2 *t = dst;
+            dst = const_cast<uint2 *>(src);
             src = t;
         }
     }
@@ -1194,7 +1164,7 @@
     const int T = a.v.gx * a.v.gy;
     auto k = a.exact ? k_render_fwd<true> : k_render_fwd<false>;
     k<<<T, 256, 0, s>>>(a.v.W, a.v.H, a.v.gx, T, a.tile_order_f, a.ranges, a.pairs,
-                        a.point_list, a.slot_emit, a.rec, a.v.bg, a.out_color, a.out_depth, a.pix_end, a.n_contrib,
+                        a.point_list, a.rec, a.v.bg, a.out_color, a.out_depth, a.pix_end, a.n_contrib,
                         a.tile_maxc, a.seg_off, a.seg_state, a.spec_ok, seg_log2(a.v.P), a.gate, a.gate_seq,
                         a.gate_err, a.gate_timeout, a.tile_flag, a.near_rec, a.items_ws + kTSatCtr, a.tsat_list,
                         tsat_capacity(a.v.W * a.v.H));
diff --git a/animating-gaussian-splats_amd/csrc/gsr_internal.h b/animating-gaussian-splats_amd/csrc/gsr_internal.h
--- a/animating-gaussian-splats_amd/csrc/gsr_internal.h
+++ b/animating-gaussian-splats_amd/csrc/gsr_internal.h
@@ -14,14 +14,14 @@
 
 struct FwdArgs {
     ViewIn v;
-    float *depth; float4 *rec; uint2 *rect; uint32_t *tiles; uint32_t *goff; uint8_t *clampm;
+    float *depth; float4 *rec; uint2 *rect; uint32_t *tiles; uint32_t *goff; uint8_t *clampm; uint2 *emap;
     uint2 *ranges; float4 *pix_end; uint32_t *n_contrib; uint32_t *tile_maxc;
     uint32_t *tile_order_f; uint32_t *seg_off; uint32_t *sort_lists; uint32_t *tile_count;
     uint32_t *tile_cursor; uint32_t *block_sums; uint32_t *block_off; uint32_t *meta; uint32_t *chunk_off;
     uint32_t *items_ws; uint32_t *scan_ws; uint32_t *tile_rank;
     uint32_t *tile_flag; float4 *near_rec;
     uint32_t *tsat_list;
-    uint4 *pairs; uint32_t *point_list; uint32_t *slot_emit; float4 *seg_state;
+    uint2 *pairs; uint32_t *point_list; float4 *seg_state;
     int *radii; float *out_color; float *out_depth;
     uint32_t spec_cap; const uint32_t *spec_ok;
     uint32_t spec_sort_blocks;
@@ -35,9 +35,9 @@
     int K;
     const int *radii;
     const float4 *rec; const uint2 *rect; const uint8_t *clampm;
-    const uint32_t *goff; const uint2 *ranges; const float4 *pix_end; const uint32_t *n_contrib;
+    const uint32_t *goff; const uint2 *emap; const uint2 *ranges; const float4 *pix_end; const uint32_t *n_contrib;
     const uint32_t *tile_maxc; const uint32_t *tile_flag; const float4 *near_rec; const uint32_t *seg_off; const uint32_t *meta; uint32_t *items_ws;
-    const uint32_t *point_list; const uint32_t *slot_emit; const float4 *seg_state;
+    const uint32_t *point_list; const float4 *seg_state;
     uint2 *items; uint32_t max_items;
     float4 *part;
     const float *dL_dcolor;
@@ -51,7 +51,7 @@
 hipError_t launch_bin_count(const FwdArgs &a, hipStream_t s);
 hipError_t launch_bin_scan(const FwdArgs &a, uint32_t *host_words, hipStream_t s);
 hipError_t launch_bin_emit(const FwdArgs &a, int K, hipStream_t s);
-hipError_t launch_tile_sort(const FwdArgs &a, uint32_t n_mid, uint32_t n_vlong, uint32_t max_n, uint4 *tmp,
+hipError_t launch_tile_sort(const FwdArgs &a, uint32_t n_mid, uint32_t n_vlong, uint32_t max_n, uint2 *tmp,
                             hipStream_t s);
 hipError_t launch_render_fwd(const FwdArgs &a, hipStream_t s);
 hipError_t launch_zero(float *p, size_t n, hipStream_t s);
diff --git a/animating-gaussian-splats_amd/diff_gaussian_rasterization/_C.py b/animating-gaussian-splats_amd/diff_gaussian_rasterization/_C.py
--- a/animating-gaussian-splats_amd/diff_gaussian_rasterization/_C.py
+++ b/animating-gaussian-splats_amd/diff_gaussian_rasterization/_C.py
@@ -784,6 +784,19 @@
     return tot.value, cnt.value
 
 
+class _Decoded(dict):
+
+    def __init__(self, slot_emit, views):
+        super().__init__(views)
+        self._slot_emit = slot_emit
+
+    def __missing__(self, key):
+        if key != "slot_emit":
+            raise KeyError(key)
+        self[key] = self._slot_emit()
+        return self[key]
+
+
 def decode_buffers(P, W, H, num_rendered, geomBuffer, binningBuffer, imgBuffer, binning_layout=0):
     L = load_library()
     offs = (ctypes.c_size_t * 16)()
@@ -798,17 +811,30 @@
 
     f32, i32, i64 = torch.float32, torch.int32, torch.int64
     rec = view(geomBuffer, o[1], 16 * P, f32, (P, 16))
-    return {
+    rect = view(geomBuffer, o[2], 2 * P, i32, (P, 2))
+    goff = view(geomBuffer, o[4], P + 1, i32, (P + 1,))
+    ranges = view(imgBuffer, o[5], 2 * T, i32, (T, 2))
+    point_list = view(binningBuffer, o[10], K, i32, (K,))
+
+    def slot_emit():
+        gx = (W + 15) // 16
+        tile = torch.repeat_interleave(torch.arange(T, device=ranges.device), (ranges[:, 1] - ranges[:, 0]).long())
+        g = point_list.long().clamp_(0, max(P - 1, 0))
+        r0, r1 = rect[g, 0].long(), rect[g, 1].long()
+        x0, y0, x1 = r0 & 0xFFFF, r0 >> 16, r1 & 0xFFFF
+        return (goff[g].long() + (tile // gx - y0) * (x1 - x0) + (tile % gx - x0)).to(i32)
+
+    return _Decoded(slot_emit, {
         "depth": view(geomBuffer, o[0], P, f32, (P,)),
         "rec": rec,
         "xy": rec[:, 0:2],
         "conic_opacity": torch.stack([rec[:, 12], rec[:, 13], rec[:, 14], rec[:, 5]], 1),
         "rgbd": torch.cat([rec[:, 8:11], rec[:, 6:7]], 1),
         "tau2": rec[:, 7],
-        "rect": view(geomBuffer, o[2], 2 * P, i32, (P, 2)),
+        "rect": rect,
         "tiles_touched": view(geomBuffer, o[3], P, i32, (P,)),
-        "goff": view(geomBuffer, o[4], P + 1, i32, (P + 1,)),
-        "ranges": view(imgBuffer, o[5], 2 * T, i32, (T, 2)),
+        "goff": goff,
+        "ranges": ranges,
         "pix_end": view(imgBuffer, o[6], 4 * W * H, f32, (H, W, 4)),
         "final_T": view(imgBuffer, o[6], 4 * W * H, f32, (H, W, 4))[..., 3],
         "seg_off": view(imgBuffer, o[12], T + 1, i32, (T + 1,)),
@@ -816,8 +842,7 @@
         "tile_maxc": view(imgBuffer, o[8], 4 * T, i32, (T, 4)),
         "tile_flag": view(imgBuffer, o[14], T, i32, (T,)),
         "tsat_count": view(imgBuffer, o[15], 1, i32, (1,)),
-        "pairs": view(binningBuffer, o[9], 4 * K, i32, (K, 4)),
-        "keys": view(binningBuffer, o[9], 2 * K, i64, (K, 2))[:, 0],
-        "point_list": view(binningBuffer, o[10], K, i32, (K,)),
-        "slot_emit": view(binningBuffer, o[11], K, i32, (K,)),
-    }
+        "pairs": view(binningBuffer, o[9], 2 * K, i32, (K, 2)),
+        "keys": view(binningBuffer, o[9], K, i64, (K,)),
+        "point_list": point_list,
+    })
```

Measured after the change: 1411 Msplats/s. Within noise of the previous version (-0.5%).
